# bonlime/sota_imagenet

Hardware: AMD Instinct MI355X
Metric: images/sec (whole node) ResNet-50 bs=256/GPU @224px (higher is better)
Workload: dtype bf16; 1 GPU; ResNet-50 v1.5 train step (fwd+CE+bwd+allreduce+SGD), bs=256/GPU, 224px, configs[2] bf16 activations / fp32 accumulate+master; global_batch=256, image_size=224, parallelism=dp1

## Files before the change

include/mi355rn.h:

```cpp
#ifndef MI355RN_H
#define MI355RN_H

#include <stddef.h>
#include <stdint.h>

#ifdef __cplusplus
extern "C" {
#endif

typedef enum mi355_status {
  MI355_OK = 0,
  MI355_E_ARG = -1,
  MI355_E_HIP = -2,
  MI355_E_STATE = -3,
  MI355_E_NOMEM = -4
} mi355_status;

typedef enum mi355_dtype { MI355_F32 = 0, MI355_BF16 = 1, MI355_FP8 = 2 } mi355_dtype;

const char* mi355_last_error(void);
int mi355_version(void);
int mi355_device_count(void);


size_t mi355_conv2d_workspace_bytes(int dtype, int N, int H, int W, int Cin, int Cout, int KH, int KW,
                                    int stride, int pad);

int mi355_conv2d_fwd(int dtype, const void* x, const void* w, void* y, int N, int H, int W, int Cin,
                     int Cout, int KH, int KW, int stride, int pad, void* stream);

int mi355_conv2d_fwd_stats(int dtype, const void* x, const void* w, void* y, float* partial, size_t partial_bytes, int* nblk,
                           int N, int H, int W, int Cin, int Cout, int KH, int KW, int stride, int pad, void* stream);
int mi355_conv2d_dgrad(int dtype, const void* dy, const void* w, void* dx, const void* addend, int N,
                       int H, int W, int Cin, int Cout, int KH, int KW, int stride, int pad, void* ws,
                       size_t ws_bytes, void* stream);
int mi355_conv2d_fwd_bn_in(int dtype, const void* y_in, const float* scale_shift, const void* w, void* y, void* a_out, uint8_t* a_bits,
                           float* partial, size_t partial_bytes, int* nblk, int N, int H, int W, int Cin, int Cout, int KH, int KW, int stride,
                           int pad, void* stream);
int mi355_conv2d_dgrad_bn(int dtype, const void* dy, const void* w, void* dx, const void* addend, const uint8_t* addend_bits, int addend_sub2,
                          const void* bn_y, const uint8_t* bn_bits, const float* bn_mean, const float* bn_invstd, float* partial,
                          size_t partial_bytes, int* nblk, int N, int H, int W, int Cin, int Cout, int KH, int KW, int stride, int pad,
                          void* ws, size_t ws_bytes, void* stream);
int mi355_conv2d_dgrad_bn_leaky(int dtype, const void* dy, const void* w, void* dx, const void* addend, const uint8_t* addend_bits, int addend_sub2,
                                const void* bn_y, const uint8_t* bn_bits, const float* bn_mean, const float* bn_invstd, float slope, float* partial,
                                size_t partial_bytes, int* nblk, int N, int H, int W, int Cin, int Cout, int KH, int KW, int stride, int pad,
                                void* ws, size_t ws_bytes, void* stream);

int mi355_conv2d_wgrad(int dtype, const void* dy, const void* x, float* dw, float beta, int N, int H,
                       int W, int Cin, int Cout, int KH, int KW, int stride, int pad, void* ws,
                       size_t ws_bytes, void* stream);

typedef struct mi355_crop {
  unsigned long long offset;
  int h, w, rh, rw, oy, ox, mirror, filter;
} mi355_crop;
typedef struct mi355_augment {
  float color[12];
  float blur_sigma;
  int gray, nbox, pad;
  int box[4][4];
} mi355_augment;
int mi355_ingest_u8(const unsigned char* packed, size_t packed_bytes, const mi355_crop* crops_host, const mi355_crop* crops_dev,
                    int N, int S, float mean, float std, float* out_nchw, void* stream);
int mi355_ingest_u8_aug(const unsigned char* packed, size_t packed_bytes, const mi355_crop* crops_host,
                        const mi355_crop* crops_dev, const mi355_augment* aug_host, const mi355_augment* aug_dev, int N, int S,
                        float mean, float std, float* scratch, float* out_nchw, void* stream);

int mi355_quantize_fp8(int src_dtype, const void* x, void* q, float scale, size_t n, void* stream);
int mi355_conv2d_fwd_fp8(const void* xq, const void* wq, void* y, float oscale, int N, int H, int W, int Cin, int Cout,
                         int KH, int KW, int stride, int pad, void* stream);
int mi355_conv2d_dgrad_fp8(const void* dyq, const void* wtq, void* dx, float oscale, int N, int H, int W, int Cin,
                           int Cout, int KH, int KW, int stride, int pad, void* stream);
int mi355_conv2d_wgrad_fp8(const void* dyq, const void* xq, float* dw, float beta, float oscale, int N, int H, int W, int Cin,
                           int Cout, int KH, int KW, int stride, int pad, void* ws, size_t ws_bytes, void* stream);

size_t mi355_stem_xpad_bytes(int dtype, int N, int H, int W);
int mi355_stem_ingest(int dtype, const float* x_nchw, void* xpad, int N, int H, int W, void* stream);
int mi355_stem_fwd(int dtype, const void* xpad, const float* w_krsc, void* y, int N, int H, int W,
                   void* ws, size_t ws_bytes, void* stream);
int mi355_stem_wgrad(int dtype, const void* dy, const void* xpad, float* dw, float beta, int N, int H,
                     int W, void* ws, size_t ws_bytes, void* stream);
size_t mi355_stem_workspace_bytes(int dtype, int N, int H, int W);

size_t mi355_bn_workspace_bytes(int C);
int mi355_bn_fwd_train(int dtype, const void* x, const void* residual, void* out, const float* gamma,
                       const float* beta, float* running_mean, float* running_var, float* save_mean,
                       float* save_invstd, int M, int C, float eps, float momentum, int relu, void* ws,
                       size_t ws_bytes, void* stream);
int mi355_bn_fwd_train_partial(int dtype, const void* x, const void* residual, void* out, const float* gamma,
                               const float* beta, float* running_mean, float* running_var, float* save_mean,
                               float* save_invstd, int M, int C, float eps, float momentum, int relu, const float* partial,
                               int nblk, void* ws, size_t ws_bytes, void* stream);
int mi355_bn_fwd_eval(int dtype, const void* x, const void* residual, void* out, const float* gamma,
                      const float* beta, const float* running_mean, const float* running_var, int M,
                      int C, float eps, int relu, void* ws, size_t ws_bytes, void* stream);
int mi355_bn_bwd(int dtype, const void* dout, const void* out, const void* x, const float* gamma,
                 const float* save_mean, const float* save_invstd, void* dx, void* dz_out,
                 float* dgamma, float* dbeta, float beta_acc, int M, int C, int relu, void* ws,
                 size_t ws_bytes, void* stream);

int mi355_maxpool_fwd(int dtype, const void* x, void* y, uint8_t* idx, int N, int H, int W, int C,
                      void* stream);
int mi355_maxpool_bwd(int dtype, const void* dy, const uint8_t* idx, void* dx, int N, int H, int W,
                      int C, void* stream);

int mi355_gap_fwd(int dtype, const void* x, float* pooled, int N, int HW, int C, void* stream);
int mi355_gap_bwd(int dtype, const float* dpooled, void* dx, int N, int HW, int C, void* stream);

int mi355_ce_loss(const float* logits, const float* target, float smoothing, float grad_scale,
                  float* loss, float* row_loss, float* dlogits, int N, int C, void* stream);

int mi355_sgd_step(float* p, const float* g, float* m, size_t n, float lr, float momentum,
                   float weight_decay, float grad_scale, void* stream);
int mi355_sgd_step_ema(float* p, const float* g, float* m, float* ema, size_t n, float lr, float momentum,
                       float weight_decay, float grad_scale, float ema_decay, void* stream);

int mi355_adam_step(float* p, const float* g, float* m, float* v, size_t n, double beta1, double beta2, float eps,
                    float step_size, float bc2_sqrt, double lr, double weight_decay, int decoupled, float grad_scale,
                    void* stream);
int mi355_adam_step_ema(float* p, const float* g, float* m, float* v, float* ema, size_t n, double beta1, double beta2,
                        float eps, float step_size, float bc2_sqrt, double lr, double weight_decay, int decoupled,
                        float grad_scale, float ema_decay, void* stream);

int mi355_madgrad_step(float* p, const float* g, float* grad_sum_sq, float* s, const float* x0, size_t n, double lr, double momentum,
                       double weight_decay, double eps, int k, float grad_scale, void* stream);
int mi355_madgrad_step_ema(float* p, const float* g, float* grad_sum_sq, float* s, const float* x0, float* ema, size_t n, double lr,
                           double momentum, double weight_decay, double eps, int k, float grad_scale, float ema_decay, void* stream);

size_t mi355_adais_workspace_bytes(size_t n);
int mi355_adais_moments(const float* g, float* v, size_t n, double beta2, int step, float grad_scale, void* workspace, void* stream);
int mi355_adais_mean(const void* workspace, size_t workspace_bytes, size_t param_size, float* mean, void* stream);
int mi355_adais_step(float* p, const float* g, float* m, const float* v, float* beta1_prod, const float* mean, size_t n, double lr,
                     double beta0, double beta2, double eps, double weight_decay, int step, float grad_scale, void* stream);
int mi355_adais_step_ema(float* p, const float* g, float* m, const float* v, float* beta1_prod, const float* mean, float* ema, size_t n,
                         double lr, double beta0, double beta2, double eps, double weight_decay, int step, float grad_scale,
                         float ema_decay, void* stream);

size_t mi355_lw_item_elems(void);
int mi355_lw_sumsq(const float* src, size_t n, const void* items, size_t n_items, int n_tensors, float scale, void* partial, void* stream);
int mi355_lw_coef(int rule, int flags, const void* partial, size_t n_partial, const void* tensors, size_t n_tensors, void* v, float* coef,
                  void* sums, double beta1, double beta2, double eps, double lr, double weight_decay, double mean, void* stream);
int mi355_lw_update(int rule, float* p, const float* g, float* m, size_t n, const void* items, size_t n_items, const float* coef, int n_tensors,
                    double lr, int soft_wd, double wd_eps, float grad_scale, void* stream);
int mi355_lw_update_ema(int rule, float* p, const float* g, float* m, float* ema, size_t n, const void* items, size_t n_items, const float* coef,
                        int n_tensors, double lr, int soft_wd, double wd_eps, float grad_scale, float ema_decay, void* stream);

int mi355_lw_unit_sumsq(const float* src, size_t n, const void* pieces, size_t n_pieces, int n_slots, float scale, void* partial, void* stream);
int mi355_lw_unit_coef(const void* partial, size_t n_partial, const void* slots, size_t n_slots, float* v, float* den, void* sums, double beta2,
                       double eps, void* stream);
int mi355_lw_unit_update(int rule, float* p, const float* g, float* m, size_t n, const void* items, size_t n_items, const void* tensors,
                         int n_tensors, const float* den, size_t n_slots, double beta1, double lr, double weight_decay, int soft_wd, double wd_eps,
                         float grad_scale, void* stream);
int mi355_lw_unit_update_ema(int rule, float* p, const float* g, float* m, float* ema, size_t n, const void* items, size_t n_items,
                             const void* tensors, int n_tensors, const float* den, size_t n_slots, double beta1, double lr, double weight_decay,
                             int soft_wd, double wd_eps, float grad_scale, float ema_decay, void* stream);

int mi355_adamp_unit_sums(const float* p, const float* g, const float* m, const float* v, size_t n, const void* pieces, size_t n_pieces,
                          int n_slots, double beta1, double beta2, double eps, int step, int nesterov, float grad_scale, void* partial,
                          void* stream);
int mi355_adamp_coef(const void* partial, size_t n_partial, const void* slots, size_t n_slots, const void* decide, size_t n_tensors, float* coef,
                     float* wdf, int* mode, double lr, double weight_decay, double eps, double delta, double wd_ratio, void* stream);
int mi355_adamp_update(float* p, const float* g, float* m, float* v, size_t n, const void* items, size_t n_items, const void* tensors,
                       int n_tensors, const float* coef, size_t n_slots, const float* wdf, double lr, double beta1, double beta2, double eps,
                       int step, int nesterov, float grad_scale, void* stream);
int mi355_adamp_update_ema(float* p, const float* g, float* m, float* v, float* ema, size_t n, const void* items, size_t n_items,
                           const void* tensors, int n_tensors, const float* coef, size_t n_slots, const float* wdf, double lr, double beta1,
                           double beta2, double eps, int step, int nesterov, float grad_scale, float ema_decay, void* stream);

int mi355_sam_sumsq(const float* p, const float* g, size_t n, const void* items, size_t n_items, const int* kind, int n_tensors, float eta,
                    float grad_scale, void* partial, void* stream);
int mi355_sam_scale(const void* partial, size_t n_partial, double rho, float* out, void* stream);
int mi355_sam_perturb(float* p, const float* g, float* eps, size_t n, const void* items, size_t n_items, const int* kind, int n_tensors,
                      const float* out, float eta, float grad_scale, void* stream);
int mi355_sam_restore(float* p, const float* eps, size_t n, const void* items, size_t n_items, int n_tensors, void* stream);

int mi355_sam_lw_sumsq(const float* p, const float* g, size_t n, const void* items, size_t n_items, int n_tensors, float grad_scale, void* partial,
                       void* stream);
int mi355_sam_unit_sumsq(const float* p, const float* g, size_t n, const void* pieces, size_t n_pieces, int n_slots, float grad_scale,
                         void* partial, int threads_per_piece, void* stream);
int mi355_sam_lw_coef(const void* partial, size_t n_partial, const void* slots, size_t n_slots, float* coef, float* norms, void* stream);
int mi355_sam_lw_perturb(float* p, const float* g, float* eps, size_t n, const void* items, size_t n_items, const void* tensors, int n_tensors,
                         const float* coef, size_t n_slots, double rho, float grad_scale, void* stream);
// ... 118 lines not shown
```

sota_imagenet_amd/csrc/bn.hip:

```cpp
#include <hip/hip_fp8.h>

#include <algorithm>

#include "common.h"
#include "vec.h"

namespace mi355 {
namespace {

constexpr int MAXBLK = 512;

__device__ __forceinline__ void quant8(const float (&v)[8], float scale, uint8_t* dst, float& amax) {
  float c[8];
#pragma unroll
  for (int e = 0; e < 8; ++e) {
    const float r = (float)(bf16_t)v[e];
    amax = fmaxf(amax, fabsf(r));
    c[e] = __builtin_amdgcn_fmed3f(r * scale, 448.f, -448.f);
  }
  int lo = 0, hi = 0;
  lo = __builtin_amdgcn_cvt_pk_fp8_f32(c[0], c[1], lo, false);
  lo = __builtin_amdgcn_cvt_pk_fp8_f32(c[2], c[3], lo, true);
  hi = __builtin_amdgcn_cvt_pk_fp8_f32(c[4], c[5], hi, false);
  hi = __builtin_amdgcn_cvt_pk_fp8_f32(c[6], c[7], hi, true);
// ... 326 lines not shown
      for (int e = 0; e < V; ++e) v[e] += fmaf(rv[e], sc2[e], sh2[e]);
    }
    if constexpr (RELU != 0) {
      if constexpr (RELU == 2 || RELU == 3) {
        unsigned b = 0;
#pragma unroll
        for (int e = 0; e < V; ++e) b |= (v[e] > 0.f ? 1u : 0u) << e;
        __builtin_nontemporal_store((uint8_t)b, p.bits + i);
      }
#pragma unroll
      for (int e = 0; e < V; ++e) v[e] = v[e] > 0.f ? v[e] : (RELU == 2 ? 0.f : v[e] * p.slope);
    }
    if constexpr (!QONLY) Vec16<T>::store(out + i * V, v);
    if constexpr (Q) quant8(v, qs, p.qo.q + i * V, amax);
  }
  if constexpr (Q) amax_flush(amax, p.qo.amax);
}

struct BwdApplyArgs {
  const void* g;
  const void* mask;
  const uint8_t* bits;
  const void* x;
  const float* mean;
  const float* invstd;
  const float* coef;
  void* dx;
  size_t nvec;
  int cvecs, C;
  float slope;
  EcaGrad eg;
  QuantOut qo;
};

template <typename T, int MASK, bool Q = false, bool QONLY = false>
__global__ __launch_bounds__(256) void bn_bwd_apply_kernel(const BwdApplyArgs p) {
  constexpr int V = Vec16<T>::N;
  static_assert(!Q || V == 8, "the quantised twin exists for bf16 tensors");
  float qs = 1.f, amax = 0.f;
  if constexpr (Q) qs = p.qo.scale[0];
  const T* g = reinterpret_cast<const T*>(p.g);
  const T* mk = reinterpret_cast<const T*>(p.mask);
  const T* x = reinterpret_cast<const T*>(p.x);
  T* dx = reinterpret_cast<T*>(p.dx);
  const size_t stride = (size_t)gridDim.x * 256;
  size_t i = (size_t)blockIdx.x * 256 + threadIdx.x;
  const int c0 = (int)(i % p.cvecs) * V;
  float mu[V], is[V], k0[V], k1[V], k2[V];
  load_consts<V>(p.mean, c0, mu);
  load_consts<V>(p.invstd, c0, is);
  load_consts<V>(p.coef, c0, k0);
  load_consts<V>(p.coef + p.C, c0, k1);
  load_consts<V>(p.coef + 2 * p.C, c0, k2);
#pragma unroll 2
  for (; i < p.nvec; i += stride) {
    float gv[V], xv[V];
    Vec16<T>::load_nt(g + i * V, gv);
    Vec16<T>::load_nt(x + i * V, xv);
    if constexpr (MASK == 2) {
      const unsigned b = p.bits[i];
#pragma unroll
      for (int e = 0; e < V; ++e) gv[e] = (b >> e) & 1u ? gv[e] : 0.f;
    } else if constexpr (MASK == 3) {
      const unsigned b = p.bits[i];
#pragma unroll
      for (int e = 0; e < V; ++e) gv[e] = (b >> e) & 1u ? gv[e] : gv[e] * p.slope;
    } else if constexpr (MASK == 4) {
      eca_grad<T, V>(p.eg, (int)((i / p.cvecs) / (size_t)p.eg.hw), p.C, c0, gv);
    } else if constexpr (MASK == 1) {
      float mv[V];
      Vec16<T>::load(mk + i * V, mv);
#pragma unroll
      for (int e = 0; e < V; ++e) gv[e] = mv[e] > 0.f ? gv[e] : gv[e] * p.slope;
    }
#pragma unroll
    for (int e = 0; e < V; ++e) {
      const float xh = (xv[e] - mu[e]) * is[e];
      gv[e] = k0[e] * (gv[e] - k1[e] - xh * k2[e]);
    }
    if constexpr (!QONLY) Vec16<T>::store(dx + i * V, gv);
    if constexpr (Q) quant8(gv, qs, p.qo.q + i * V, amax);
  }
  if constexpr (Q) amax_flush(amax, p.qo.amax);
}

constexpr int SC = 64;

__device__ __forceinline__ __amdgpu_buffer_rsrc_t rsrc_of(const void* p, size_t bytes) {
  return __builtin_amdgcn_make_buffer_rsrc(const_cast<void*>(p), 0, (int)(bytes > 0xfffffffcull ? 0xfffffffcull : bytes), 0x00020000);
}
__device__ __forceinline__ uint4 buf16(__amdgpu_buffer_rsrc_t r, unsigned voff, unsigned soff, bool nt = false) {
  return nt ? __builtin_bit_cast(uint4, __builtin_amdgcn_raw_buffer_load_b128(r, voff, soff, 2))
            : __builtin_bit_cast(uint4, __builtin_amdgcn_raw_buffer_load_b128(r, voff, soff, 0));
}

template <typename T>
struct PoolGather {
  static constexpr int V = Vec16<T>::N;
  uint4 g[4];
  uint32_t id[4][V / 4];
  __device__ __forceinline__ void load(__amdgpu_buffer_rsrc_t rg, __amdgpu_buffer_rsrc_t ri, unsigned t, unsigned cv, int a, int b, int Ho, int Wo) {
    const unsigned go = (t * SC + cv * V) * (unsigned)sizeof(T), io = t * SC + cv * V;
#pragma unroll
    for (int w = 0; w < 4; ++w) {
      const bool ok = a + (w >> 1) < Ho && b + (w & 1) < Wo;
      const unsigned srow = (w >> 1) ? (unsigned)Wo * SC : 0u;
      g[w] = buf16(rg, go + (w & 1) * SC * (unsigned)sizeof(T), srow * (unsigned)sizeof(T));
      if constexpr (V == 4) {
        const unsigned x = (unsigned)__builtin_amdgcn_raw_buffer_load_b32(ri, io + (w & 1) * SC, srow, 0);
        id[w][0] = ok ? x : 0xffffffffu;
      } else {
        typedef unsigned u32x2 __attribute__((ext_vector_type(2)));
        const u32x2 x = __builtin_bit_cast(u32x2, __builtin_amdgcn_raw_buffer_load_b64(ri, io + (w & 1) * SC, srow, 0));
        id[w][0] = ok ? x[0] : 0xffffffffu;
        id[w][1] = ok ? x[1] : 0xffffffffu;
      }
    }
  }
  template <int r, int c>
  __device__ __forceinline__ void pixel(unsigned bits, float (&out)[V]) const {
#pragma unroll
    for (int e = 0; e < V; ++e) out[e] = 0.f;
#pragma unroll
    for (int dr = 0; dr <= r; ++dr)
#pragma unroll
      for (int dc = 0; dc <= c; ++dc) {
        const unsigned pos = (r + 1 - 2 * dr) * 3 + (c + 1 - 2 * dc);
        float gw[V];
        Vec16<T>::unpack(g[2 * dr + dc], gw);
#pragma unroll
        for (int e = 0; e < V; ++e)
          if (((id[2 * dr + dc][e >> 2] >> (8 * (e & 3))) & 0xffu) == pos) out[e] += gw[e];
      }
#pragma unroll
    for (int e = 0; e < V; ++e) out[e] = (bits >> e) & 1u ? (float)(T)out[e] : 0.f;
  }
};

struct StemBwdArgs {
  const void* dp;
  const uint8_t* idx;
  const uint8_t* bits;
  const void* y;
  const float* mean;
  const float* invstd;
  const float* coef;
  float* partial;
  void* dx;
  int N, Ho, Wo;
};

template <typename T>
struct BlockIn {
  uint4 y[4];
  unsigned bt[4];
  unsigned pix00;
  __device__ __forceinline__ void load(__amdgpu_buffer_rsrc_t ry, __amdgpu_buffer_rsrc_t rb, int n, int a, int b, int Ho, int Wo, unsigned cv, bool nt) {
    constexpr int V = Vec16<T>::N;
    const unsigned W = 2 * Wo;
    pix00 = ((unsigned)n * 2 * Ho + 2 * a) * W + 2 * b;
#pragma unroll
    for (int k = 0; k < 4; ++k) {
      const unsigned srow = (k >> 1) ? W : 0u;
      y[k] = buf16(ry, (pix00 * SC + cv * V) * (unsigned)sizeof(T) + (k & 1) * SC * (unsigned)sizeof(T), srow * SC * (unsigned)sizeof(T), nt);
      bt[k] = (unsigned)__builtin_amdgcn_raw_buffer_load_b8(rb, pix00 * (SC / V) + cv + (k & 1) * (SC / V), srow * (SC / V), 0);
    }
// ... 329 lines not shown
  } else {
    MI355_BN_REDUCE(bf16_t)
  }
#undef MI355_BN_REDUCE
  MI355_LAUNCH_CHECK();
  return 0;
}

int launch_bn_bwd_finalize(const float* partial, int nblk, int M, int C, const float* gamma, const float* invstd,
                           float* dgamma, float* dbeta, float beta_acc, float* coef, hipStream_t s) {
  FinalizeArgs a{};
  a.partial = partial;
  a.nblk = nblk;
  a.M = M;
  a.C = C;
  a.gamma = gamma;
  a.invstd = invstd;
  a.dgamma = dgamma;
  a.dbeta = dbeta;
  a.beta_acc = beta_acc;
  a.coef = coef;
  if (fin_one_channel(C, nblk) && nblk > FIN_WIDE_ROWS) hipLaunchKernelGGL((bn_finalize_kernel<1, 1, 1024>), dim3(C), dim3(1024), 0, s, a);
  else if (fin_one_channel(C, nblk)) hipLaunchKernelGGL((bn_finalize_kernel<1, 1>), dim3(C), dim3(256), 0, s, a);
  else hipLaunchKernelGGL((bn_finalize_kernel<1, 4>), dim3(C / 4), dim3(256), 0, s, a);
  MI355_LAUNCH_CHECK();
  return 0;
}

int launch_bn_bwd_apply(int dtype, const void* g, const void* mask_src, const void* x, const float* mean,
                        const float* invstd, const float* coef, void* dx, int M, int C, hipStream_t s,
                        const uint8_t* relu_bits, float slope, QuantOut qo, const EcaGrad* eg) {
  MI355_TRY(check_c(dtype, C));
  const int V = 16 / (int)dtype_size(dtype);
  BwdApplyArgs a{};
  if (eg) a.eg = *eg;
  a.slope = slope;
  a.g = g;
  a.mask = mask_src;
  a.bits = relu_bits;
  a.x = x;
  a.mean = mean;
  a.invstd = invstd;
  a.coef = coef;
  a.dx = dx;
  a.nvec = (size_t)M * C / V;
  a.cvecs = C / V;
  a.C = C;
  const int blocks = elementwise_blocks(a.nvec, a.cvecs);
  const int mask = relu_bits ? (slope != 0.f ? 3 : 2) : mask_src ? 1 : 0;
  a.qo = qo;
  if (eg) {
    MI355_ARG(mask == 0 && !qo.q && eg->gate && eg->dpool && eg->hw > 0, "bn_bwd_apply: the ECA gradient source takes no mask / twin");
    if (dtype == MI355_F32) hipLaunchKernelGGL((bn_bwd_apply_kernel<float, 4>), dim3(blocks), dim3(256), 0, s, a);
    else hipLaunchKernelGGL((bn_bwd_apply_kernel<bf16_t, 4>), dim3(blocks), dim3(256), 0, s, a);
    MI355_LAUNCH_CHECK();
    return 0;
  }
  if (qo.q) {
    MI355_ARG(dtype == MI355_BF16 && mask != 1 && mask != 3 && qo.scale && qo.amax, "bn_bwd_apply: the e4m3 twin needs bf16 and a ReLU bit mask (or none)");
    if (mask == 2 && qo.only) hipLaunchKernelGGL((bn_bwd_apply_kernel<bf16_t, 2, true, true>), dim3(blocks), dim3(256), 0, s, a);
    else if (mask == 2) hipLaunchKernelGGL((bn_bwd_apply_kernel<bf16_t, 2, true>), dim3(blocks), dim3(256), 0, s, a);
    else if (qo.only) hipLaunchKernelGGL((bn_bwd_apply_kernel<bf16_t, 0, true, true>), dim3(blocks), dim3(256), 0, s, a);
    else hipLaunchKernelGGL((bn_bwd_apply_kernel<bf16_t, 0, true>), dim3(blocks), dim3(256), 0, s, a);
    MI355_LAUNCH_CHECK();
    return 0;
  }
#define MI355_BN_BWD_APPLY(TT)                                                                                  \
  switch (mask) {                                                                                               \
    case 0: hipLaunchKernelGGL((bn_bwd_apply_kernel<TT, 0>), dim3(blocks), dim3(256), 0, s, a); break;          \
    case 1: hipLaunchKernelGGL((bn_bwd_apply_kernel<TT, 1>), dim3(blocks), dim3(256), 0, s, a); break;          \
    case 2: hipLaunchKernelGGL((bn_bwd_apply_kernel<TT, 2>), dim3(blocks), dim3(256), 0, s, a); break;          \
    default: hipLaunchKernelGGL((bn_bwd_apply_kernel<TT, 3>), dim3(blocks), dim3(256), 0, s, a); break;         \
  }
  if (dtype == MI355_F32) {
    MI355_BN_BWD_APPLY(float)
  } else {
    MI355_BN_BWD_APPLY(bf16_t)
  }
#undef MI355_BN_BWD_APPLY
  MI355_LAUNCH_CHECK();
  return 0;
}

static int stem_bwd_args(StemBwdArgs& a, int dtype, const void* dp, const uint8_t* idx, const uint8_t* bits, const void* y, const float* mean,
                         const float* invstd, int N, int H, int W, int C) {
  MI355_TRY(check_c(dtype, C));
  const int V = 16 / (int)dtype_size(dtype);
  (void)V;
  MI355_ARG(dp && idx && bits && y && H % 2 == 0 && W % 2 == 0 && C == SC, "stem_bwd: N=%d H=%d W=%d C=%d (64 channels)", N, H, W, C);
  MI355_ARG((unsigned long long)N * H * W * C * dtype_size(dtype) < 0xfffffff0ull, "stem_bwd: tensor beyond 32-bit offsets");
  a = StemBwdArgs{};
  a.dp = dp; a.idx = idx; a.bits = bits; a.y = y; a.mean = mean; a.invstd = invstd;
  a.N = N; a.Ho = H / 2; a.Wo = W / 2;
  return 0;
}

int launch_stem_bwd_reduce(int dtype, const void* dp, const uint8_t* idx, const uint8_t* bits, const void* y, const float* mean,
                           const float* invstd, float* partial, int* nblk_out, int N, int H, int W, int C, hipStream_t s) {
  StemBwdArgs a;
  MI355_TRY(stem_bwd_args(a, dtype, dp, idx, bits, y, mean, invstd, N, H, W, C));
  a.partial = partial;
  const int V = 16 / (int)dtype_size(dtype);
  const int rpp = 256 / (C / V);
  int nblk = cdiv(N * a.Ho * a.Wo, rpp * 4);
  const int cap = std::min(2 * MAXBLK, 2 * device_cus());
  if (nblk > cap) nblk = cap;
  *nblk_out = nblk;
  if (dtype == MI355_F32) hipLaunchKernelGGL(stem_bwd_reduce_kernel<float>, dim3(nblk), dim3(256), 0, s, a);
  else hipLaunchKernelGGL(stem_bwd_reduce_kernel<bf16_t>, dim3(nblk), dim3(256), 0, s, a);
  MI355_LAUNCH_CHECK();
  return 0;
}

int launch_stem_bwd_apply(int dtype, const void* dp, const uint8_t* idx, const uint8_t* bits, const void* y, const float* mean,
                          const float* invstd, const float* coef, void* dx, int N, int H, int W, int C, hipStream_t s) {
  StemBwdArgs a;
  MI355_TRY(stem_bwd_args(a, dtype, dp, idx, bits, y, mean, invstd, N, H, W, C));
  a.coef = coef; a.dx = dx;
  const int V = 16 / (int)dtype_size(dtype);
  const int blocks = elementwise_blocks((size_t)N * a.Ho * a.Wo * (C / V), C / V);
  if (dtype == MI355_F32) hipLaunchKernelGGL(stem_bwd_apply_kernel<float>, dim3(blocks), dim3(256), 0, s, a);
  else hipLaunchKernelGGL(stem_bwd_apply_kernel<bf16_t>, dim3(blocks), dim3(256), 0, s, a);
  MI355_LAUNCH_CHECK();
  return 0;
}

}
```

sota_imagenet_amd/csrc/common.h:

```cpp
#pragma once
#include <hip/hip_runtime.h>
#include <cstdarg>
#include <cstdint>
#include <cstdio>
#include <cstring>

#include "../../include/mi355rn.h"

namespace mi355 {

typedef __bf16 bf16_t;

typedef float f32x4 __attribute__((ext_vector_type(4)));
typedef float f32x16 __attribute__((ext_vector_type(16)));
typedef __bf16 bf16x8 __attribute__((ext_vector_type(8)));
typedef __bf16 bf16x4 __attribute__((ext_vector_type(4)));
typedef short s16x4 __attribute__((ext_vector_type(4)));

void set_error(const char* fmt, ...);
int device_cus();
int probe_env(const char* name);

#define MI355_HIP(expr)                                                                         \
  do {                                                                                          \
    hipError_t e_ = (expr);                                                                     \
    if (e_ != hipSuccess) {                                                                     \
      ::mi355::set_error("%s:%d: %s -> %s", __FILE__, __LINE__, #expr, hipGetErrorString(e_));  \
      return MI355_E_HIP;                                                                       \
    }                                                                                           \
  } while (0)

#define MI355_LAUNCH_CHECK()                                                                    \
  do {                                                                                          \
    hipError_t e_ = hipGetLastError();                                                          \
    if (e_ != hipSuccess) {                                                                     \
      ::mi355::set_error("%s:%d: kernel launch -> %s", __FILE__, __LINE__, hipGetErrorString(e_)); \
      return MI355_E_HIP;                                                                       \
    }                                                                                           \
  } while (0)

#define MI355_ARG(cond, ...)                      \
  do {                                            \
    if (!(cond)) {                                \
      ::mi355::set_error(__VA_ARGS__);            \
      return MI355_E_ARG;                         \
    }                                             \
  } while (0)

#define MI355_TRY(expr)            \
  do {                             \
    int rc_ = (expr);              \
    if (rc_ != 0) return rc_;      \
  } while (0)

static inline size_t dtype_size(int dt) { return dt == MI355_BF16 ? 2 : 4; }
static inline size_t align_up(size_t x, size_t a) { return (x + a - 1) / a * a; }
static inline int cdiv(int a, int b) { return (a + b - 1) / b; }

struct Tap {
  int8_t dh, dw;
  int16_t wtap;
};
struct TapClass {
  int ph, pw, ntaps;
  Tap taps[9];
};
struct IgemmArgs {
  const void* in;
  const void* wt;
  void* out;
  const void* addend;
  const uint8_t* addend_bits = nullptr;
  int addend_sub2 = 0;
  int stat_rows_cap = 0;
  float* stat_partial;
  void* sk_ws = nullptr;
  const void* bn_y = nullptr;
  const uint8_t* bn_bits = nullptr;
  const float* bn_mean = nullptr;
  const float* bn_invstd = nullptr;
  float bn_slope = 0.f;
  const float* bn_in = nullptr;
  void* bn_in_a = nullptr;
  uint8_t* bn_in_bits = nullptr;
  const float* q_scale_in = nullptr;
  const float* q_scale_wt = nullptr;
  int N, Hin, Win, pix_stride;
  int Hsub, Wsub, IS;
  int Hout, Wout, OS;
  int Ck, Ncols, wtaps;
  int pair_delta;
  TapClass cls[4];
};

struct WgradArgs {
  const void* dy;
  const void* x;
  float* partial;
  int N, Ho, Wo, Cout;
  int Hin, Win, pix_stride, IS;
  int Ck, wtaps, ntaps;
  int chunks_per_split;
  int pair_delta;
  Tap taps[9];
};

int launch_igemm(int dtype, const IgemmArgs& a, int nclass, hipStream_t stream, int* stat_rows = nullptr);
bool igemm_leaky_sums_legal(int dtype, const IgemmArgs& a, int nclass);
bool igemm_sub2_legal(int dtype, const IgemmArgs& a, int nclass);
bool igemm_bn_in_legal(int dtype, const IgemmArgs& a, int nclass);
static constexpr size_t IGEMM_SK_FLAG_BYTES = 4096;
static constexpr int IGEMM_SK_ERR_WORD = 512;
size_t igemm_sk_ws_bytes();
bool igemm_fp8_legal(const IgemmArgs& a, int nclass);
int launch_igemm_fp8(const IgemmArgs& a, int nclass, float oscale, hipStream_t stream, int* stat_rows = nullptr);
int plan_wgrad_splits(int dtype, int M, int Cout, int ntaps, int Ck);
int plan_wgrad(int dtype, const WgradArgs& a);
int launch_wgrad(int dtype, const WgradArgs& a, int splits, hipStream_t stream);
struct Knobs {
  bool has_igemm8 = false;
  char igemm8[32] = {0};
  int igemm_big = -1;
  bool has_igemm_big = false;
  int stem_direct = 1;
  int stem_th = 0;
  bool stem_dbg = false;
  bool sk_mute = false;
  int dconv = 1;
  int wg3 = 1;
  int pw = 1;
  int pk = 1;
  int po = 1;
  int po64 = 1;
  int dconv_fp8 = 1;
  int pool_keys = 1;
  int po_bn = 1;
  int dconv_bn = 0;
  int dconv_s2 = 1;
  char error[160] = {0};
};
const Knobs& knobs();
inline int env_switch(const char* name, int def, int maxv, const char** bad) {
  const char* e = getenv(name);
  if (!e) return def;
  if (e[0] >= '0' && e[0] <= '0' + maxv && e[1] == 0) return e[0] - '0';
  if (bad && !*bad) *bad = name;
  return def;
}
void note_kernel(const char* fmt, ...);
int launch_splitk_reduce(const float* partial, int splits, size_t stride, float* dst, size_t n, float beta,
                         hipStream_t stream, const float* sa = nullptr, const float* sb = nullptr);
int launch_stem_unpack(float* partial, int splits, float* dw, float beta, hipStream_t stream);

int launch_weight_prep(int dtype, const float* w, void* w_cast, void* w_tr, int Cout, int taps, int Cin,
                       hipStream_t stream);
constexpr int PREP_TILE = 64;
struct PrepDesc {
  size_t w_off;
  void* w_cast;
  void* w_tr;
  void* w_q;
  void* w_trq;
  const float* q_scale;
  unsigned* q_amax;
  int Cout, taps, Cin;
  int tile_begin;
};
struct BPrepDesc {
  const float* w;
  float* w_hat;
  float* mean;
  float* invstd;
  void* wp;
  void* wtr;
  int Cout, taps, Cin, Coutp, Cinp;
  int row_begin;
  int tile_begin;
};
struct KeepBatch {
  float* keep[20];
  unsigned long long n[20];
  unsigned long long counter[20];
  float p[20];
  int count = 0;
};
int launch_keep_scale_batch(const KeepBatch& kb, unsigned long long seed, hipStream_t s);
int launch_bres_weight_prep(int dtype, const BPrepDesc* table, int nconv, int total_rows, int total_tiles, float eps, bool transposed, hipStream_t stream);
int launch_weight_prep_batch(int dtype, const PrepDesc* table, int nlayers, int total_tiles, const float* params,
                             hipStream_t stream);
int launch_transpose_any(int dtype, const void* w, void* wt, int Cout, int taps, int Cin, hipStream_t stream);
int launch_stem_pack(int dtype, const float* w, void* packed, hipStream_t stream);

void build_fwd_args(IgemmArgs& a, int N, int H, int W, int Cin, int Cout, int KH, int KW, int stride, int pad);
int build_dgrad_args(IgemmArgs& a, int N, int H, int W, int Cin, int Cout, int KH, int KW, int stride, int pad);
void build_wgrad_args(WgradArgs& a, int N, int H, int W, int Cin, int Cout, int KH, int KW, int stride, int pad);
void build_stem_fwd_args(IgemmArgs& a, int N, int H, int W);
void build_stem_wgrad_args(WgradArgs& a, int N, int H, int W);

static constexpr int STEM_PAD = 3, STEM_PS = 4, STEM_CK = 64, STEM_RPAD = 16;
static inline int stem_hp(int H) { return H + 2 * STEM_PAD; }
static inline int stem_wp(int W) { return W + STEM_RPAD; }

int launch_bn_stats(int dtype, const void* x, float* partial, float* pivot, int* nblk_out, int M, int C, hipStream_t s);
int launch_bn_finalize(const float* partial, const float* pivot, int nblk, int M, int C, const float* gamma, const float* beta,
                       float* running_mean, float* running_var, float* save_mean, float* save_invstd,
                       float* scale, float* shift, float eps, float momentum, hipStream_t s);
int launch_bn_eval_coeffs(const float* gamma, const float* beta, const float* rm, const float* rv, float* scale,
                          float* shift, int C, float eps, hipStream_t s);
struct QuantOut {
  uint8_t* q = nullptr;
  const float* scale = nullptr;
  unsigned* amax = nullptr;
  bool only = false;
};
int launch_bn_apply(int dtype, const void* x, const float* scale, const float* shift, const void* residual,
                    const void* x2, const float* scale2, const float* shift2, void* out, int M, int C, int relu,
                    hipStream_t s, uint8_t* relu_bits = nullptr, QuantOut qo = QuantOut());
struct EcaGrad {
  const float* keep = nullptr;
  const float* gate = nullptr;
  const float* dpool = nullptr;
  int hw = 0;
};
int launch_bn_bwd_reduce(int dtype, const void* g, const void* mask_src, const void* x, const float* mean,
                         const float* invstd, void* dz_out, float* partial, int* nblk_out, int M, int C,
                         hipStream_t s, const uint8_t* relu_bits = nullptr, float slope = 0.f, const EcaGrad* eg = nullptr);
int launch_bn_bwd_finalize(const float* partial, int nblk, int M, int C, const float* gamma, const float* invstd,
                           float* dgamma, float* dbeta, float beta_acc, float* coef , hipStream_t s);
int launch_bn_bwd_apply(int dtype, const void* g, const void* mask_src, const void* x, const float* mean,
                        const float* invstd, const float* coef, void* dx, int M, int C, hipStream_t s,
                        const uint8_t* relu_bits = nullptr, float slope = 0.f, QuantOut qo = QuantOut(), const EcaGrad* eg = nullptr);
int launch_stem_bwd_reduce(int dtype, const void* dp, const uint8_t* idx, const uint8_t* bits, const void* y, const float* mean,
                           const float* invstd, float* partial, int* nblk_out, int N, int H, int W, int C, hipStream_t s);
int launch_stem_bwd_apply(int dtype, const void* dp, const uint8_t* idx, const uint8_t* bits, const void* y, const float* mean,
                          const float* invstd, const float* coef, void* dx, int N, int H, int W, int C, hipStream_t s);
int bn_max_blocks();
int launch_nchw_pad64(int dtype, const float* x_nchw, void* h_nhwc64, int N, int HW, hipStream_t s);
int launch_weight_pad_cast(int dtype, const float* w, void* wp, int Cout, int taps, int Cin, int Coutp, int Cinp, hipStream_t s);
int launch_nchw_im2col3s2(int dtype, const float* x, void* h, int N, int H, int W, hipStream_t s);
int launch_weight_unpad(const float* dwp, float* dw, float beta, int Cout, int taps, int Cin, int Cinp, hipStream_t s);
int launch_axpby(const float* src, float* dst, float beta, size_t n, hipStream_t s);
int launch_eca_residual_fwd(int dtype, const void* x, const float* w, int k, const float* keep, const void* shortcut, void* out, float* pooled, float* gate,
                            int N, int HW, int C, int act, hipStream_t s, const float* xs = nullptr, const float* xh = nullptr, const float* ss = nullptr,
                            const float* sh2 = nullptr, uint8_t* out_bits = nullptr, float* raw_ws = nullptr );
int launch_eca_residual_bwd(int dtype, const void* dout, const void* out, const void* x, const float* keep, const float* w, int k, const float* pooled,
                            const float* gate, void* dshortcut, void* dx, float* dw, float beta, float* ws, int N, int HW, int C, int act, hipStream_t s,
                            const float* xs = nullptr, const float* xh = nullptr, float* bn_row = nullptr, const float* bn_mean = nullptr,
                            const float* bn_invstd = nullptr, const uint8_t* out_bits = nullptr, const void* ds_y = nullptr, float* ds_row = nullptr,
                            const float* ds_mean = nullptr, const float* ds_invstd = nullptr);
int launch_fp8_scale_update(float* scale, unsigned* amax, int n, float headroom, hipStream_t s);

int launch_maxpool_fwd(int dtype, const void* x, void* y, uint8_t* idx, int N, int H, int W, int C, hipStream_t s);
int launch_bn_relu_maxpool(int dtype, const void* y, const float* scale, const float* shift, void* p, uint8_t* idx,
                           uint8_t* bits, int N, int H, int W, int C, hipStream_t s);
int launch_maxpool_bwd(int dtype, const void* dy, const uint8_t* idx, void* dx, int N, int H, int W, int C,
                       hipStream_t s);
int launch_gap_fwd(int dtype, const void* x, float* pooled, int N, int HW, int C, hipStream_t s);
int launch_fc(const float* x, const float* w, float* out, int M, int N, int K, hipStream_t s);
int launch_gap_bwd(int dtype, const float* dpooled, void* dx, int N, int HW, int C, hipStream_t s);
int launch_ce(const float* logits, const float* target, float smoothing, float grad_scale, float* loss,
              float* row_loss, float* dlogits, int N, int C, hipStream_t s);
int launch_sgd(float* p, const float* g, float* m, size_t n, float lr, float mom, float wd, float gscale,
               hipStream_t s, float* ema = nullptr, float ema_decay = 0.f);
int launch_adam(float* p, const float* g, float* m, float* v, size_t n, double beta1, double beta2, float eps, float step_size,
                float bc2_sqrt, double lr, double wd, int decoupled, float gscale, hipStream_t s, float* ema = nullptr,
                float ema_decay = 0.f);
int launch_madgrad(float* p, const float* g, float* gss, float* s, const float* x0, size_t n, double lr, double momentum, double wd,
                   double eps, int k, float gscale, hipStream_t st, float* ema = nullptr, float ema_decay = 0.f);
size_t adais_partials(size_t n);
int launch_adais_moments(const float* g, float* v, size_t n, double beta2, int step, float gscale, double* partial, hipStream_t st);
int launch_adais_mean(const double* partial, size_t count, size_t param_size, float* mean, hipStream_t st);
int launch_adais_step(float* p, const float* g, float* m, const float* v, float* b1prod, const float* mean, size_t n, double lr, double beta0,
                      double beta2, double eps, double wd, int step, float gscale, hipStream_t st, float* ema = nullptr,
                      float ema_decay = 0.f);
size_t lw_item_elems();
int launch_lw_sumsq(const float* src, size_t n, const void* items, size_t n_items, int n_tensors, float scale, double* partial, hipStream_t st);
int launch_lw_coef(int rule, int flags, const double* partial, size_t n_partial, const void* tensors, size_t n_tensors, void* v, float* coef,
                   double* sums, double beta1, double beta2, double eps, double lr, double wd, double mean, hipStream_t st);
int launch_lw_update(int rule, float* p, const float* g, float* m, float* ema, size_t n, const void* items, size_t n_items, const float* coef,
                     int n_tensors, double lr, int soft_wd, double wd_eps, float gscale, float ema_decay, hipStream_t st);
int launch_lw_unit_sumsq(const float* src, size_t n, const void* pieces, size_t n_pieces, int n_slots, float scale, double* partial,
                         hipStream_t st);
int launch_lw_unit_coef(const double* partial, size_t n_partial, const void* slots, size_t n_slots, float* v, float* den, double* sums,
                        double beta2, double eps, hipStream_t st);
int launch_lw_unit_update(int rule, float* p, const float* g, float* m, float* ema, size_t n, const void* items, size_t n_items,
                          const void* tensors, int n_tensors, const float* den, size_t n_slots, double beta1, double lr, double wd, int soft_wd,
                          double wd_eps, float gscale, float ema_decay, hipStream_t st);
int launch_adamp_unit_sums(const float* p, const float* g, const float* m, const float* v, size_t n, const void* pieces, size_t n_pieces,
                           int n_slots, double beta1, double beta2, double eps, int step, int nesterov, float gscale, double* partial,
                           hipStream_t st);
int launch_adamp_coef(const double* partial, size_t n_partial, const void* slots, size_t n_slots, const void* tensors, size_t n_tensors,
                      float* coef, float* wdf, int* mode, double lr, double wd, double eps, double delta, double wd_ratio, hipStream_t st);
int launch_adamp_update(float* p, const float* g, float* m, float* v, float* ema, size_t n, const void* items, size_t n_items,
                        const void* tensors, int n_tensors, const float* coef, size_t n_slots, const float* wdf, double lr, double beta1,
                        double beta2, double eps, int step, int nesterov, float gscale, float ema_decay, hipStream_t st);
int launch_sam_sumsq(const float* p, const float* g, size_t n, const void* items, size_t n_items, const int* kind, int n_tensors, float eta,
                     float gscale, double* partial, hipStream_t st);
int launch_sam_scale(const double* partial, size_t n_partial, double rho, float* out, hipStream_t st);
int launch_sam_perturb(float* p, const float* g, float* eps, size_t n, const void* items, size_t n_items, const int* kind, int n_tensors,
                       const float* out, float eta, float gscale, hipStream_t st);
int launch_sam_restore(float* p, const float* eps, size_t n, const void* items, size_t n_items, int n_tensors, hipStream_t st);
int launch_sam_lw_sumsq(const float* p, const float* g, size_t n, const void* items, size_t n_items, int n_tensors, float gscale, double* partial,
                        hipStream_t st);
int launch_sam_unit_sumsq(const float* p, const float* g, size_t n, const void* pieces, size_t n_pieces, int n_slots, float gscale,
                          double* partial, int threads_per_piece, hipStream_t st);
int launch_sam_lw_coef(const double* partial, size_t n_partial, const void* slots, size_t n_slots, float* coef, float* norms, hipStream_t st);
int launch_sam_lw_perturb(float* p, const float* g, float* eps, size_t n, const void* items, size_t n_items, const void* tensors, int n_tensors,
                          const float* coef, size_t n_slots, double rho, float gscale, hipStream_t st);
int launch_ortho_init(float* w, size_t n, const void* mats, size_t n_mats, float gain, int* status, hipStream_t st);
int launch_stem_ingest(int dtype, const float* x, void* xpad, int N, int H, int W, hipStream_t s);
int launch_bias_slice(const float* tmp, int ld, const float* bias, float* out, int N, int O, hipStream_t s);
int launch_pad_dlogits(const float* src, float* dst, int ld, float* dbias, float beta, int N, int O, hipStream_t s);

}
// ... 1 lines not shown
```

sota_imagenet_amd/csrc/conv_api.cpp:

```cpp
#include <algorithm>
#include <atomic>
#include <cstdio>
#include <cstdlib>
#include <mutex>
#include <set>
#include <string>

#include "conv_kernels.h"

namespace mi355 {

static thread_local std::string g_err;

void set_error(const char* fmt, ...) {
  char buf[1024];
  va_list ap;
  va_start(ap, fmt);
  vsnprintf(buf, sizeof(buf), fmt, ap);
  va_end(ap);
  g_err = buf;
}
const char* get_error() { return g_err.c_str(); }

int probe_env(const char* name) {
// ... 282 lines not shown
  build_fwd_args(a, N, H, W, Cin, Cout, KH, KW, stride, pad);
  a.in = x; a.wt = w; a.out = y;
  return launch_igemm(dtype, a, 1, (hipStream_t)stream);
}

int mi355_conv2d_fwd_stats(int dtype, const void* x, const void* w, void* y, float* partial, size_t partial_bytes, int* nblk, int N,
                           int H, int W, int Cin, int Cout, int KH, int KW, int stride, int pad, void* stream) {
  MI355_TRY(check_conv(dtype, Cin, Cout, KH, KW, stride));
  MI355_ARG(partial && nblk && partial_bytes >= (size_t)768 * 2 * Cout * sizeof(float), "conv2d_fwd_stats: partial buffer needs 768 * 2 * Cout floats");
  IgemmArgs a;
  build_fwd_args(a, N, H, W, Cin, Cout, KH, KW, stride, pad);
  a.in = x; a.wt = w; a.out = y;
  a.stat_partial = partial;
  a.stat_rows_cap = (int)std::min<size_t>(partial_bytes / ((size_t)2 * Cout * sizeof(float)), 1u << 20);
  return launch_igemm(dtype, a, 1, (hipStream_t)stream, nblk);
}

int mi355_conv2d_fwd_bn_in(int dtype, const void* y_in, const float* scale_shift, const void* w, void* y, void* a_out, uint8_t* a_bits, float* partial,
                           size_t partial_bytes, int* nblk, int N, int H, int W, int Cin, int Cout, int KH, int KW, int stride, int pad, void* stream) {
  MI355_TRY(check_conv(dtype, Cin, Cout, KH, KW, stride));
  MI355_ARG(y_in && scale_shift && a_out && a_bits, "conv2d_fwd_bn_in: null pointer");
  MI355_ARG(partial && nblk && partial_bytes >= (size_t)768 * 2 * Cout * sizeof(float), "conv2d_fwd_bn_in: partial buffer needs 768 * 2 * Cout floats");
  IgemmArgs a;
  build_fwd_args(a, N, H, W, Cin, Cout, KH, KW, stride, pad);
  a.in = y_in; a.wt = w; a.out = y;
  a.bn_in = scale_shift; a.bn_in_a = a_out; a.bn_in_bits = a_bits;
  a.stat_partial = partial;
  a.stat_rows_cap = (int)std::min<size_t>(partial_bytes / ((size_t)2 * Cout * sizeof(float)), 1u << 20);
  MI355_ARG(igemm_bn_in_legal(dtype, a, 1), "conv2d_fwd_bn_in: no kernel applies the input's BatchNorm for this launch (bf16; 3x3 / stride 1 at a generated shape, or 1x1 with 64 / 128 / 256 input channels into a multiple of 256 columns over whole 64-pixel tiles)");
  return launch_igemm(dtype, a, 1, (hipStream_t)stream, nblk);
}

int mi355_conv2d_dgrad(int dtype, const void* dy, const void* w, void* dx, const void* addend, int N, int H, int W,
                       int Cin, int Cout, int KH, int KW, int stride, int pad, void* ws, size_t ws_bytes,
                       void* stream) {
  MI355_TRY(check_conv(dtype, Cin, Cout, KH, KW, stride));
  const size_t es = dtype_size(dtype);
  const size_t wbytes = (size_t)Cin * KH * KW * Cout * es;
  MI355_ARG(ws && ws_bytes >= wbytes, "dgrad: workspace too small (%zu < %zu)", ws_bytes, wbytes);
  hipStream_t s = (hipStream_t)stream;
  MI355_TRY(launch_transpose_any(dtype, w, ws, Cout, KH * KW, Cin, s));
  IgemmArgs a;
  const int nclass = build_dgrad_args(a, N, H, W, Cin, Cout, KH, KW, stride, pad);
  if (nclass < 0) return nclass;
  a.in = dy; a.wt = ws; a.out = dx; a.addend = addend;
  return launch_igemm(dtype, a, nclass, s);
}

int mi355_conv2d_dgrad_bn(int dtype, const void* dy, const void* w, void* dx, const void* addend, const uint8_t* addend_bits, int addend_sub2, const void* bn_y,
                          const uint8_t* bn_bits, const float* bn_mean, const float* bn_invstd, float* partial, size_t partial_bytes, int* nblk, int N,
                          int H, int W, int Cin, int Cout, int KH, int KW, int stride, int pad, void* ws, size_t ws_bytes, void* stream) {
  return mi355_conv2d_dgrad_bn_leaky(dtype, dy, w, dx, addend, addend_bits, addend_sub2, bn_y, bn_bits, bn_mean, bn_invstd, 0.f, partial, partial_bytes, nblk, N, H, W,
                                     Cin, Cout, KH, KW, stride, pad, ws, ws_bytes, stream);
}

int mi355_conv2d_dgrad_bn_leaky(int dtype, const void* dy, const void* w, void* dx, const void* addend, const uint8_t* addend_bits, int addend_sub2,
                                const void* bn_y, const uint8_t* bn_bits, const float* bn_mean, const float* bn_invstd, float slope, float* partial,
                                size_t partial_bytes, int* nblk, int N, int H, int W, int Cin, int Cout, int KH, int KW, int stride, int pad, void* ws,
                                size_t ws_bytes, void* stream) {
  MI355_TRY(check_conv(dtype, Cin, Cout, KH, KW, stride));
  MI355_ARG(slope == 0.f || partial, "dgrad_bn_leaky: a slope without the BN-backward sums");
  const size_t es = dtype_size(dtype);
  const size_t wbytes = (size_t)Cin * KH * KW * Cout * es;
  MI355_ARG(ws && ws_bytes >= wbytes, "dgrad_bn: workspace too small (%zu < %zu)", ws_bytes, wbytes);
  MI355_ARG(addend || !addend_bits, "dgrad_bn: addend_bits without an addend");
  MI355_ARG(!partial || (bn_y && bn_bits && bn_mean && bn_invstd && nblk), "dgrad_bn: the BN-backward sums need bn_y, bn_bits, bn_mean, bn_invstd and nblk");
  MI355_ARG(!partial || partial_bytes >= (size_t)768 * 2 * Cin * sizeof(float), "dgrad_bn: partial buffer needs 768 * 2 * Cin floats");
  hipStream_t s = (hipStream_t)stream;
  MI355_TRY(launch_transpose_any(dtype, w, ws, Cout, KH * KW, Cin, s));
  IgemmArgs a;
  const int nclass = build_dgrad_args(a, N, H, W, Cin, Cout, KH, KW, stride, pad);
  if (nclass < 0) return nclass;
  a.in = dy; a.wt = ws; a.out = dx; a.addend = addend; a.addend_bits = addend_bits; a.addend_sub2 = addend_sub2;
  MI355_ARG(!addend_sub2 || igemm_sub2_legal(dtype, a, nclass), "dgrad_bn: no kernel takes a half-resolution addend for this launch (bf16 1x1 / stride 1, even H and W)");
  if (partial) {
    a.stat_partial = partial;
    a.stat_rows_cap = (int)std::min<size_t>(partial_bytes / ((size_t)2 * Cin * sizeof(float)), 1u << 20);
    a.bn_y = bn_y; a.bn_bits = bn_bits; a.bn_mean = bn_mean; a.bn_invstd = bn_invstd; a.bn_slope = slope;
  }
  if (nblk) *nblk = 0;
  return launch_igemm(dtype, a, nclass, s, partial ? nblk : nullptr);
}

int mi355_conv2d_wgrad(int dtype, const void* dy, const void* x, float* dw, float beta, int N, int H, int W, int Cin,
                       int Cout, int KH, int KW, int stride, int pad, void* ws, size_t ws_bytes, void* stream) {
  MI355_TRY(check_conv(dtype, Cin, Cout, KH, KW, stride));
  WgradArgs a;
  build_wgrad_args(a, N, H, W, Cin, Cout, KH, KW, stride, pad);
  const int splits = plan_wgrad(dtype, a);
  const size_t n = (size_t)Cout * KH * KW * Cin;
  MI355_ARG(ws && ws_bytes >= (size_t)splits * n * 4, "wgrad: workspace too small (%zu < %zu)", ws_bytes,
            (size_t)splits * n * 4);
  a.dy = dy; a.x = x; a.partial = (float*)ws;
  hipStream_t s = (hipStream_t)stream;
  MI355_TRY(launch_wgrad(dtype, a, splits, s));
  return launch_splitk_reduce((const float*)ws, splits, n, dw, n, beta, s);
}

size_t mi355_stem_xpad_bytes(int dtype, int N, int H, int W) {
  return (size_t)N * stem_hp(H) * stem_wp(W) * STEM_PS * dtype_size(dtype);
}

size_t mi355_stem_workspace_bytes(int dtype, int N, int H, int W) {
  const int splits = plan_wgrad_splits(dtype, N * (H / 2) * (W / 2), 64, 4, STEM_CK);
  return align_up((size_t)64 * 4 * 64 * dtype_size(dtype), 256) + (size_t)splits * 64 * 4 * 64 * 4;
}

int mi355_stem_ingest(int dtype, const float* x_nchw, void* xpad, int N, int H, int W, void* stream) {
  MI355_ARG(x_nchw && xpad && H % 2 == 0 && W % 2 == 0, "stem_ingest: bad arguments");
  return launch_stem_ingest(dtype, x_nchw, xpad, N, H, W, (hipStream_t)stream);
}

int mi355_stem_fwd(int dtype, const void* xpad, const float* w_krsc, void* y, int N, int H, int W, void* ws,
                   size_t ws_bytes, void* stream) {
  const size_t pk = (size_t)64 * 4 * 64 * dtype_size(dtype);
  MI355_ARG(ws && ws_bytes >= pk, "stem_fwd: workspace too small");
  hipStream_t s = (hipStream_t)stream;
  MI355_TRY(launch_stem_pack(dtype, w_krsc, ws, s));
  IgemmArgs a;
  build_stem_fwd_args(a, N, H, W);
  a.in = xpad; a.wt = ws; a.out = y;
  return launch_igemm(dtype, a, 1, s);
}

int mi355_stem_wgrad(int dtype, const void* dy, const void* xpad, float* dw, float beta, int N, int H, int W, void* ws,
                     size_t ws_bytes, void* stream) {
  WgradArgs a;
  build_stem_wgrad_args(a, N, H, W);
  const int splits = plan_wgrad_splits(dtype, a.N * a.Ho * a.Wo, 64, 4, STEM_CK);
  MI355_ARG(ws && ws_bytes >= (size_t)splits * 64 * 4 * 64 * 4, "stem_wgrad: workspace too small");
  a.dy = dy; a.x = xpad; a.partial = (float*)ws;
  hipStream_t s = (hipStream_t)stream;
  MI355_TRY(launch_wgrad(dtype, a, splits, s));
  return launch_stem_unpack((float*)ws, splits, dw, beta, s);
}

size_t mi355_bn_workspace_bytes(int C) { return ((size_t)bn_max_blocks() * 2 * C + 8 * (size_t)C) * 4; }

int mi355_bn_fwd_train(int dtype, const void* x, const void* residual, void* out, const float* gamma,
                       const float* beta, float* running_mean, float* running_var, float* save_mean,
                       float* save_invstd, int M, int C, float eps, float momentum, int relu, void* ws,
                       size_t ws_bytes, void* stream) {
  MI355_ARG(ws && ws_bytes >= mi355_bn_workspace_bytes(C), "bn: workspace too small");
  hipStream_t s = (hipStream_t)stream;
  float* partial = (float*)ws;
  float* scale = partial + (size_t)bn_max_blocks() * 2 * C;
  float* shift = scale + C;
  float* pivot = shift + C;
  int nblk = 0;
  MI355_TRY(launch_bn_stats(dtype, x, partial, pivot, &nblk, M, C, s));
  MI355_TRY(launch_bn_finalize(partial, pivot, nblk, M, C, gamma, beta, running_mean, running_var, save_mean, save_invstd,
                               scale, shift, eps, momentum, s));
  return launch_bn_apply(dtype, x, scale, shift, residual, nullptr, nullptr, nullptr, out, M, C, relu, s);
}

int mi355_bn_fwd_train_partial(int dtype, const void* x, const void* residual, void* out, const float* gamma, const float* beta,
                               float* running_mean, float* running_var, float* save_mean, float* save_invstd, int M, int C, float eps,
                               float momentum, int relu, const float* partial, int nblk, void* ws, size_t ws_bytes, void* stream) {
  MI355_ARG(ws && ws_bytes >= (size_t)2 * C * 4 && partial && nblk >= 1, "bn_fwd_train_partial: nblk=%d, workspace of 2*C floats", nblk);
  hipStream_t s = (hipStream_t)stream;
  float* scale = (float*)ws;
  float* shift = scale + C;
  MI355_TRY(launch_bn_finalize(partial, nullptr, nblk, M, C, gamma, beta, running_mean, running_var, save_mean, save_invstd, scale,
                               shift, eps, momentum, s));
  return launch_bn_apply(dtype, x, scale, shift, residual, nullptr, nullptr, nullptr, out, M, C, relu, s);
}

int mi355_bn_fwd_eval(int dtype, const void* x, const void* residual, void* out, const float* gamma,
                      const float* beta, const float* running_mean, const float* running_var, int M, int C, float eps,
                      int relu, void* ws, size_t ws_bytes, void* stream) {
  MI355_ARG(ws && ws_bytes >= (size_t)2 * C * 4, "bn_eval: workspace too small");
  hipStream_t s = (hipStream_t)stream;
  float* scale = (float*)ws;
  float* shift = scale + C;
  MI355_TRY(launch_bn_eval_coeffs(gamma, beta, running_mean, running_var, scale, shift, C, eps, s));
  return launch_bn_apply(dtype, x, scale, shift, residual, nullptr, nullptr, nullptr, out, M, C, relu, s);
}

int mi355_bn_bwd(int dtype, const void* dout, const void* out, const void* x, const float* gamma,
                 const float* save_mean, const float* save_invstd, void* dx, void* dz_out, float* dgamma,
                 float* dbeta, float beta_acc, int M, int C, int relu, void* ws, size_t ws_bytes, void* stream) {
  MI355_ARG(ws && ws_bytes >= mi355_bn_workspace_bytes(C), "bn: workspace too small");
  hipStream_t s = (hipStream_t)stream;
  float* partial = (float*)ws;
  float* coef = partial + (size_t)bn_max_blocks() * 2 * C;
  int nblk = 0;
  const void* mask = relu ? out : nullptr;
  const float slope = relu == 2 ? 0.01f : 0.f;
  MI355_TRY(launch_bn_bwd_reduce(dtype, dout, mask, x, save_mean, save_invstd, dz_out, partial, &nblk, M, C, s, nullptr, slope));
  MI355_TRY(launch_bn_bwd_finalize(partial, nblk, M, C, gamma, save_invstd, dgamma, dbeta, beta_acc, coef, s));
  return launch_bn_bwd_apply(dtype, dout, mask, x, save_mean, save_invstd, coef, dx, M, C, s, nullptr, slope);
}

int mi355_maxpool_fwd(int dtype, const void* x, void* y, uint8_t* idx, int N, int H, int W, int C, void* stream) {
  return launch_maxpool_fwd(dtype, x, y, idx, N, H, W, C, (hipStream_t)stream);
}
int mi355_maxpool_bwd(int dtype, const void* dy, const uint8_t* idx, void* dx, int N, int H, int W, int C,
                      void* stream) {
  return launch_maxpool_bwd(dtype, dy, idx, dx, N, H, W, C, (hipStream_t)stream);
}
int mi355_gap_fwd(int dtype, const void* x, float* pooled, int N, int HW, int C, void* stream) {
  return launch_gap_fwd(dtype, x, pooled, N, HW, C, (hipStream_t)stream);
}
int mi355_gap_bwd(int dtype, const float* dpooled, void* dx, int N, int HW, int C, void* stream) {
  return launch_gap_bwd(dtype, dpooled, dx, N, HW, C, (hipStream_t)stream);
}
int mi355_ce_loss(const float* logits, const float* target, float smoothing, float grad_scale, float* loss,
                  float* row_loss, float* dlogits, int N, int C, void* stream) {
  return launch_ce(logits, target, smoothing, grad_scale, loss, row_loss, dlogits, N, C, (hipStream_t)stream);
}
int mi355_sgd_step(float* p, const float* g, float* m, size_t n, float lr, float momentum, float weight_decay,
                   float grad_scale, void* stream) {
  return launch_sgd(p, g, m, n, lr, momentum, weight_decay, grad_scale, (hipStream_t)stream);
}
int mi355_sgd_step_ema(float* p, const float* g, float* m, float* ema, size_t n, float lr, float momentum, float weight_decay,
                       float grad_scale, float ema_decay, void* stream) {
  MI355_ARG(ema, "sgd_step_ema: null ema");
  return launch_sgd(p, g, m, n, lr, momentum, weight_decay, grad_scale, (hipStream_t)stream, ema, ema_decay);
}
int mi355_adam_step(float* p, const float* g, float* m, float* v, size_t n, double beta1, double beta2, float eps,
                    float step_size, float bc2_sqrt, double lr, double weight_decay, int decoupled, float grad_scale,
                    void* stream) {
  return launch_adam(p, g, m, v, n, beta1, beta2, eps, step_size, bc2_sqrt, lr, weight_decay, decoupled, grad_scale,
                     (hipStream_t)stream);
}
int mi355_adam_step_ema(float* p, const float* g, float* m, float* v, float* ema, size_t n, double beta1, double beta2,
                        float eps, float step_size, float bc2_sqrt, double lr, double weight_decay, int decoupled,
                        float grad_scale, float ema_decay, void* stream) {
  MI355_ARG(ema, "adam_step_ema: null ema");
  return launch_adam(p, g, m, v, n, beta1, beta2, eps, step_size, bc2_sqrt, lr, weight_decay, decoupled, grad_scale,
                     (hipStream_t)stream, ema, ema_decay);
}
int mi355_madgrad_step(float* p, const float* g, float* grad_sum_sq, float* s, const float* x0, size_t n, double lr, double momentum,
                       double weight_decay, double eps, int k, float grad_scale, void* stream) {
  return launch_madgrad(p, g, grad_sum_sq, s, x0, n, lr, momentum, weight_decay, eps, k, grad_scale, (hipStream_t)stream);
}
int mi355_madgrad_step_ema(float* p, const float* g, float* grad_sum_sq, float* s, const float* x0, float* ema, size_t n, double lr,
                           double momentum, double weight_decay, double eps, int k, float grad_scale, float ema_decay, void* stream) {
  MI355_ARG(ema, "madgrad_step_ema: null ema");
  return launch_madgrad(p, g, grad_sum_sq, s, x0, n, lr, momentum, weight_decay, eps, k, grad_scale, (hipStream_t)stream, ema, ema_decay);
}
size_t mi355_adais_workspace_bytes(size_t n) { return adais_partials(n) * sizeof(double); }
int mi355_adais_moments(const float* g, float* v, size_t n, double beta2, int step, float grad_scale, void* workspace, void* stream) {
  return launch_adais_moments(g, v, n, beta2, step, grad_scale, (double*)workspace, (hipStream_t)stream);
}
int mi355_adais_mean(const void* workspace, size_t workspace_bytes, size_t param_size, float* mean, void* stream) {
  MI355_ARG(workspace_bytes % sizeof(double) == 0, "adais_mean: workspace_bytes=%zu is not a whole number of partial sums", workspace_bytes);
  return launch_adais_mean((const double*)workspace, workspace_bytes / sizeof(double), param_size, mean, (hipStream_t)stream);
}
int mi355_adais_step(float* p, const float* g, float* m, const float* v, float* beta1_prod, const float* mean, size_t n, double lr,
                     double beta0, double beta2, double eps, double weight_decay, int step, float grad_scale, void* stream) {
  return launch_adais_step(p, g, m, v, beta1_prod, mean, n, lr, beta0, beta2, eps, weight_decay, step, grad_scale, (hipStream_t)stream);
}
int mi355_adais_step_ema(float* p, const float* g, float* m, const float* v, float* beta1_prod, const float* mean, float* ema, size_t n,
                         double lr, double beta0, double beta2, double eps, double weight_decay, int step, float grad_scale,
                         float ema_decay, void* stream) {
  MI355_ARG(ema, "adais_step_ema: null ema");
  return launch_adais_step(p, g, m, v, beta1_prod, mean, n, lr, beta0, beta2, eps, weight_decay, step, grad_scale, (hipStream_t)stream, ema,
                           ema_decay);
}

size_t mi355_lw_item_elems(void) { return lw_item_elems(); }
int mi355_lw_sumsq(const float* src, size_t n, const void* items, size_t n_items, int n_tensors, float scale, void* partial, void* stream) {
  return launch_lw_sumsq(src, n, items, n_items, n_tensors, scale, (double*)partial, (hipStream_t)stream);
}
int mi355_lw_coef(int rule, int flags, const void* partial, size_t n_partial, const void* tensors, size_t n_tensors, void* v, float* coef,
                  void* sums, double beta1, double beta2, double eps, double lr, double weight_decay, double mean, void* stream) {
  return launch_lw_coef(rule, flags, (const double*)partial, n_partial, tensors, n_tensors, v, coef, (double*)sums, beta1, beta2, eps, lr,
                        weight_decay, mean, (hipStream_t)stream);
}
int mi355_lw_update(int rule, float* p, const float* g, float* m, size_t n, const void* items, size_t n_items, const float* coef, int n_tensors,
                    double lr, int soft_wd, double wd_eps, float grad_scale, void* stream) {
  return launch_lw_update(rule, p, g, m, nullptr, n, items, n_items, coef, n_tensors, lr, soft_wd, wd_eps, grad_scale, 0.f, (hipStream_t)stream);
}
int mi355_lw_update_ema(int rule, float* p, const float* g, float* m, float* ema, size_t n, const void* items, size_t n_items, const float* coef,
                        int n_tensors, double lr, int soft_wd, double wd_eps, float grad_scale, float ema_decay, void* stream) {
// ... 88 lines not shown
```

sota_imagenet_amd/csrc/conv_igemm.hip:

```cpp
#include <atomic>
#include <cstdio>
#include <cstdlib>
#include <type_traits>

#include "conv_kernels.h"
#include "lds_dma.h"
#include "vec.h"

namespace mi355 {

namespace {

constexpr int BKB = 128;

__device__ __attribute__((aligned(256))) unsigned char g_zero_page[256];
#ifdef MI355_STAMP
__device__ unsigned long long g_stamps[8 * 4096];
#define STAMP(slot)                                                                                   \
  do {                                                                                                \
    if (blockIdx.x == 0 && lane == 0 && wave < 4 && stamp_k < 1024) g_stamps[(wave * 1024 + stamp_k) * 8 + (slot)] = __builtin_readcyclecounter(); \
  } while (0)
#else
#define STAMP(slot)
#endif
__device__ __attribute__((aligned(256))) unsigned char g_trash[512 * 16];
#ifdef MI355_PROBES
#define MI355_PROBE(bit) ((kp.dbg & (bit)) != 0)
#else
#define MI355_PROBE(bit) false
#endif

struct IgemmKArgs {
  IgemmArgs a;
  int mtiles, ny, nclass, ngroups, ntpg, items;
  unsigned bytes_in, bytes_wt;
  int sk_rf, sk_tail, sk_nk, sk_gshift;
  int sk_tshift;
  unsigned sk_epoch;
  float* sk_partial;
  unsigned* sk_flags;
  unsigned sk_spin_limit;
  int sk_mute;
  int dbg;
  int xcd;
};

template <int N>
__device__ __forceinline__ void wait_vm() {
  asm volatile("s_waitcnt vmcnt(%0)" ::"n"(N) : "memory");
}

template <typename T, int BM, int BN, int WMW, int NSTG, int STATS>
__global__ __launch_bounds__(128 * WMW, (BM == 256 ? 1 : (BN == 64 && NSTG == 2 ? 3 : 2))) void igemm_kernel(const IgemmKArgs kp) {
  const IgemmArgs& p = kp.a;
  constexpr int ES = (int)sizeof(T);
  constexpr int BK = BKB / ES;
  constexpr int NW = 2 * WMW;
  constexpr int NT = 64 * NW;
  constexpr int MI = BM / (32 * WMW);
  constexpr int NI = BN / 64;
  constexpr int PA = BM / NW / 8;
  constexpr int PB = BN / NW / 8;
  constexpr int NPC = PA + PB;
  constexpr int A_BYTES = BM * BKB;
  constexpr int STAGE = (BM + BN) * BKB;
  constexpr int WN = BN / 2;
  constexpr int VEC = 16 / ES;
  constexpr int CPR = WN / VEC;
  constexpr int RPI = 64 / CPR;
  constexpr int NST = MI * (32 / RPI);
  constexpr int SCH = WN / 4;
  extern __shared__ __attribute__((aligned(16))) char smem[];
  constexpr int STG_WAVE = 32 * (BN / 2) * 4;
  constexpr int EPI_FIT = STAGE / STG_WAVE;
  constexpr int EPI_WAVES = NW <= EPI_FIT ? NW : (EPI_FIT >= 4 ? 4 : (EPI_FIT >= 2 ? 2 : 1));
  constexpr int EPI_TURNS = NW / EPI_WAVES;
  static_assert(NW % EPI_WAVES == 0, "epilogue turns");
  int* row_pix = reinterpret_cast<int*>(smem + NSTG * STAGE);
  float* stat_acc = reinterpret_cast<float*>(smem + NSTG * STAGE + BM * sizeof(int));

  const int tid = threadIdx.x;
  const int lane = tid & 63;
  const int wave = __builtin_amdgcn_readfirstlane(tid >> 6);
  const int wm = wave >> 1, wn = wave & 1;
  const int G = gridDim.x;
  const int Msub = p.N * p.Hsub * p.Wsub;
  const int kc_per_tap = p.Ck / BK;

  const int prow = lane >> 3;
  const int pch = lane & 7;
  int L_seq = 0, L_item = 0, L_nt = 0, L_kt = 0, L_kend = 0, L_cls = 0, L_grp = 0;
  bool L_valid = true;
  constexpr bool SKC = BM == 128 && BN == 128 && ES == 4;
  int sk_bg = 0, sk_n = 0, sk_item0 = 0, sk_k00 = 0, sk_k10 = 0, sk_k11 = 0;
  if constexpr (SKC) {
    if (kp.sk_tail != 0) {
      sk_bg = (int)blockIdx.x / kp.ngroups;
      const int g = (int)blockIdx.x - sk_bg * kp.ngroups;
      const unsigned TK = (unsigned)(kp.sk_tail * kp.sk_nk);
      const unsigned lo = ((unsigned)sk_bg * TK) >> kp.sk_tshift, hi = ((unsigned)(sk_bg + 1) * TK) >> kp.sk_tshift;
      if (lo < hi && sk_bg < (1 << kp.sk_tshift)) {
        const int t0 = (int)(lo / (unsigned)kp.sk_nk);
        sk_item0 = ((kp.sk_rf << kp.sk_gshift) + t0) * kp.ngroups + g;
        sk_k00 = (int)lo - t0 * kp.sk_nk;
        const int e = sk_k00 + (int)(hi - lo);
        sk_k10 = e < kp.sk_nk ? e : kp.sk_nk;
        sk_k11 = (int)hi - (t0 + 1) * kp.sk_nk;
        sk_n = sk_k11 > 0 ? 2 : 1;
      }
      sk_bg = __builtin_amdgcn_readfirstlane(sk_bg);
      sk_n = __builtin_amdgcn_readfirstlane(sk_n);
      sk_item0 = __builtin_amdgcn_readfirstlane(sk_item0);
      sk_k00 = __builtin_amdgcn_readfirstlane(sk_k00);
      sk_k10 = __builtin_amdgcn_readfirstlane(sk_k10);
      sk_k11 = __builtin_amdgcn_readfirstlane(sk_k11);
    }
  }
  const int bx = __builtin_amdgcn_readfirstlane(kp.xcd ? (int)(blockIdx.x & 7u) * (G >> 3) + (int)(blockIdx.x >> 3) : (int)blockIdx.x);
  auto unit_at = [&](int seq, int& item, int& k0, int& k1) -> bool {
    if (!SKC || kp.sk_tail == 0) {
      item = bx + seq * G;
      k0 = 0;
      k1 = -1;
      return item < kp.items;
    }
    const int u = seq - kp.sk_rf;
    if (u < 0) {
      item = (int)blockIdx.x + seq * G;
      k0 = 0;
      k1 = -1;
      return true;
    }
    if (u >= sk_n) return false;
    item = sk_item0 + u * kp.ngroups;
    k0 = u == 0 ? sk_k00 : 0;
    k1 = u == 0 ? sk_k10 : sk_k11;
    return true;
  };
  const i32x4 srdA = make_srd(p.in, kp.bytes_in);
  const i32x4 srdB = make_srd(p.wt, kp.bytes_wt);
  unsigned a_off[PA];
  int a_h[PA], a_w[PA];
  unsigned b_off[PB];
#pragma unroll
  for (int i = 0; i < PB; ++i) {
    const int r = PB * 8 * wave + 8 * i + prow;
    b_off[i] = (unsigned)r * p.wtaps * p.Ck * ES + (unsigned)((pch ^ ((r >> 1) & 7)) * 16);
  }
  auto L_setup = [&]() {
    int uk0, uk1;
    while ((L_valid = unit_at(L_seq, L_item, uk0, uk1))) {
      const int rowtile = L_item / kp.ngroups;
      L_grp = L_item - rowtile * kp.ngroups;
      L_cls = rowtile / kp.mtiles;
      const int mt = rowtile - L_cls * kp.mtiles;
      const int nk_all = p.cls[L_cls].ntaps * kc_per_tap;
      if (nk_all == 0) {
        ++L_seq;
        continue;
      }
#pragma unroll
      for (int i = 0; i < PA; ++i) {
        const int r = (BM / NW) * wave + 8 * i + prow;
        const int m = mt * BM + r;
        if (m < Msub) {
          const int j = m % p.Wsub;
          const int t = m / p.Wsub;
          const int ii = t % p.Hsub;
          const int n = t / p.Hsub;
          a_h[i] = ii * p.IS;
          a_w[i] = j * p.IS;
          const int chunk = pch ^ ((r >> 1) & 7);
          a_off[i] = (unsigned)((n * p.Hin + a_h[i]) * p.Win + a_w[i]) * (unsigned)(p.pix_stride * ES) +
                     (unsigned)(chunk * 16);
          if (ES == 2 && chunk >= 4) a_off[i] += (unsigned)(p.pair_delta * ES);
        } else {
          a_h[i] = -(1 << 20);
          a_w[i] = 0;
          a_off[i] = 0;
        }
      }
      L_nt = 0;
      L_kt = uk0;
      L_kend = uk1 < 0 ? nk_all : uk1;
      return;
    }
  };
  int S_dh = 0, S_dw = 0, S_dA = 0;
  unsigned S_dB = 0, S_As = 0;
  auto L_begin = [&](int stage) {
    const int kt_u = __builtin_amdgcn_readfirstlane(L_kt);
    const int cls_u = __builtin_amdgcn_readfirstlane(L_cls);
    const int t = kt_u / kc_per_tap;
    const int c0 = (kt_u - t * kc_per_tap) * BK;
    const Tap tp = p.cls[cls_u].taps[t];
    S_dh = tp.dh;
    S_dw = tp.dw;
    S_dA = ((tp.dh * p.Win + tp.dw) * p.pix_stride + c0 + (ES == 4 && c0 >= 32 ? p.pair_delta : 0)) * ES;
    const int n0 = __builtin_amdgcn_readfirstlane((L_grp * kp.ntpg + L_nt) * BN);
    S_dB = ((unsigned)n0 * p.wtaps + tp.wtap) * (unsigned)(p.Ck * ES) + (unsigned)(c0 * ES);
    S_As = __builtin_amdgcn_readfirstlane(lds_addr(smem) + stage * STAGE);
  };
  auto L_piece = [&](int j) {
    if (j < PA) {
      const int ih = a_h[j] + S_dh;
      const int iw = a_w[j] + S_dw;
      const bool ok = ((unsigned)ih < (unsigned)p.Hin) && ((unsigned)iw < (unsigned)p.Win);
      blds16(srdA, ok ? a_off[j] + (unsigned)S_dA : 0x80000000u, S_As + ((BM / NW) * wave + 8 * j) * BKB);
    } else {
      const int i = j - PA;
      blds16(srdB, b_off[i] + S_dB, S_As + A_BYTES + (PB * 8 * wave + 8 * i) * BKB);
    }
  };
  auto L_advance = [&]() {
    if (++L_kt < L_kend) return;
    if (++L_nt < kp.ntpg) {
      L_kt = 0;
      return;
    }
    ++L_seq;
    L_setup();
  };

  const int hh = lane >> 5;
  int a_row[MI], a_sw[MI], b_row[NI], b_sw[NI];
#pragma unroll
  for (int mi = 0; mi < MI; ++mi) {
    const int r = wm * (BM / WMW) + mi * 32 + (lane & 31);
    a_row[mi] = r * BKB;
    a_sw[mi] = (r >> 1) & 7;
  }
#pragma unroll
  for (int ni = 0; ni < NI; ++ni) {
    const int r = wn * WN + ni * 32 + (lane & 31);
    b_row[ni] = A_BYTES + r * BKB;
    b_sw[ni] = (r >> 1) & 7;
  }

  if constexpr (STATS != 0) {
    for (int i = tid; i < WMW * kp.ntpg * BN * 2; i += NT) stat_acc[i] = 0.f;
  }
  L_setup();
  int stage = 0;
  int L_stage = 0;
  int inflight = 0;
#pragma unroll
  for (int pre = 0; pre < NSTG - 1; ++pre)
    if (L_valid) {
      L_begin(L_stage);
#pragma unroll
      for (int j = 0; j < NPC; ++j) L_piece(j);
      L_advance();
      L_stage = L_stage + 1 == NSTG ? 0 : L_stage + 1;
      ++inflight;
    }
  int pending_st = 0;
#ifdef MI355_STAMP
  int stamp_k = 0;
#endif

  T* out = reinterpret_cast<T*>(p.out);
  const T* addend = reinterpret_cast<const T*>(p.addend);

  int item, uk0, uk1;
  for (int seq = 0; unit_at(seq, item, uk0, uk1); ++seq) {
    const int rowtile = item / kp.ngroups;
    const int grp = item - rowtile * kp.ngroups;
    const int ci = rowtile / kp.mtiles;
    const int mt = rowtile - ci * kp.mtiles;
    const TapClass& cls = p.cls[ci];
    const int nk = cls.ntaps * kc_per_tap;
    const int m0 = mt * BM;
    for (int nti = 0; nti < kp.ntpg; ++nti) {
      const int n0 = (grp * kp.ntpg + nti) * BN;
      f32x16 acc[MI][NI];
#pragma unroll
      for (int mi = 0; mi < MI; ++mi)
#pragma unroll
        for (int ni = 0; ni < NI; ++ni)
#pragma unroll
          for (int r = 0; r < 16; ++r) acc[mi][ni][r] = 0.f;

      const int kbeg = uk0, kend = uk1 < 0 ? nk : uk1;
      for (int kt = kbeg; kt < kend; ++kt) {
        STAMP(0);
        if constexpr (NSTG == 2) {
          if (pending_st == NST) {
            wait_vm<NST>();
          } else {
            wait_vm<0>();
          }
        } else {
          const bool younger = inflight >= 2;
          if (younger && pending_st == NST) wait_vm<NPC + NST>();
          else if (younger) wait_vm<NPC>();
          else if (pending_st == NST) wait_vm<NST>();
          else wait_vm<0>();
        }
        pending_st = 0;
        STAMP(1);
        MI355_LDS_BARRIER();
        STAMP(2);
        const bool lv = L_valid;
        if (lv) L_begin(L_stage);
        const char* base = smem + stage * STAGE;
        typedef typename std::conditional<ES == 4, f32x4, bf16x8>::type frag_t;
        frag_t av[2][MI], bv[2][NI];
        auto read_frags = [&](int g, int set) {
#pragma unroll
          for (int mi = 0; mi < MI; ++mi)
            av[set][mi] = *reinterpret_cast<const frag_t*>(base + a_row[mi] + (((2 * g + hh) ^ a_sw[mi]) << 4));
#pragma unroll
          for (int ni = 0; ni < NI; ++ni)
            bv[set][ni] = *reinterpret_cast<const frag_t*>(base + b_row[ni] + (((2 * g + hh) ^ b_sw[ni]) << 4));
        };
        read_frags(0, 0);
#pragma unroll
        for (int g = 0; g < 4; ++g) {
          if (g + 1 < 4) read_frags(g + 1, (g + 1) & 1);
          if (lv) {
#pragma unroll
            for (int j = g * NPC / 4; j < (g + 1) * NPC / 4; ++j) L_piece(j);
          }
// ... 32 lines not shown
        if (kbeg > 0) {
          const i32x4 srdP = make_srd(kp.sk_partial, (unsigned)((size_t)G * SLOT * 4));
          const unsigned base = ((unsigned)blockIdx.x * SLOT + tid * 4) * 4u;
#pragma unroll
          for (int mi = 0; mi < MI; ++mi)
#pragma unroll
            for (int ni = 0; ni < NI; ++ni)
#pragma unroll
              for (int g = 0; g < 4; ++g) {
                const f32x4 v = {acc[mi][ni][4 * g], acc[mi][ni][4 * g + 1], acc[mi][ni][4 * g + 2], acc[mi][ni][4 * g + 3]};
                const unsigned off = base + (unsigned)(((mi * NI + ni) * 4 + g) * 256 * 16);
                asm volatile("buffer_store_dwordx4 %0, %1, %2, 0 offen sc1" ::"v"(v), "v"(off), "s"(srdP) : "memory");
              }
          asm volatile("s_waitcnt vmcnt(0)" ::: "memory");
          __builtin_amdgcn_s_barrier();
          if (tid == 0 && !kp.sk_mute)
            __hip_atomic_store(kp.sk_flags + blockIdx.x, kp.sk_epoch, __ATOMIC_RELAXED, __HIP_MEMORY_SCOPE_AGENT);
          pending_st = 0;
          continue;
        }
        const unsigned TK = (unsigned)(kp.sk_tail * kp.sk_nk);
        const int tt = rowtile - (kp.sk_rf << kp.sk_gshift);
        const unsigned tile_end = (unsigned)((tt + 1) * kp.sk_nk);
        int bgj = sk_bg + 1;
        int covered = kend;
        while (covered < nk && bgj < (1 << kp.sk_tshift)) {
          const unsigned lo_j = ((unsigned)bgj * TK) >> kp.sk_tshift, hi_j = ((unsigned)(bgj + 1) * TK) >> kp.sk_tshift;
          const int cnt = (int)((hi_j < tile_end ? hi_j : tile_end) - lo_j);
          if (cnt > 0) {
            const int j = bgj * kp.ngroups + grp;
            if (tid == 0) {
              unsigned spins = 0;
              while (__hip_atomic_load(kp.sk_flags + j, __ATOMIC_RELAXED, __HIP_MEMORY_SCOPE_AGENT) != kp.sk_epoch) {
                __builtin_amdgcn_s_sleep(2);
                if (++spins > kp.sk_spin_limit) {
                  __hip_atomic_store(kp.sk_flags + IGEMM_SK_ERR_WORD, 1u, __ATOMIC_RELAXED, __HIP_MEMORY_SCOPE_AGENT);
                  break;
                }
              }
              __builtin_amdgcn_fence(__ATOMIC_ACQUIRE, "agent");
            }
            asm volatile("s_waitcnt vmcnt(0)" ::: "memory");
            __builtin_amdgcn_s_barrier();
            const float* slot = kp.sk_partial + (size_t)j * SLOT + tid * 4;
#pragma unroll
            for (int mi = 0; mi < MI; ++mi)
#pragma unroll
              for (int ni = 0; ni < NI; ++ni)
#pragma unroll
                for (int g = 0; g < 4; ++g) {
                  const f32x4 v = *reinterpret_cast<const f32x4*>(slot + ((mi * NI + ni) * 4 + g) * 256 * 4);
#pragma unroll
                  for (int e = 0; e < 4; ++e) acc[mi][ni][4 * g + e] += v[e];
                }
            covered += cnt;
            pending_st = 0;
          }
          ++bgj;
        }
      }

      const int done_stage = stage == 0 ? NSTG - 1 : stage - 1;
      char* stg = smem + done_stage * STAGE + (wave % EPI_WAVES) * STG_WAVE;
      MI355_LDS_BARRIER();
      if (MI355_PROBE(1)) continue;
      if (tid < BM) {
        const int m = m0 + tid;
        int pix = -1;
        if (m < Msub) {
          const int j = m % p.Wsub;
          const int t = m / p.Wsub;
          const int ii = t % p.Hsub;
          const int n = t / p.Hsub;
          pix = (n * p.Hout + ii * p.OS + cls.ph) * p.Wout + j * p.OS + cls.pw;
        }
        row_pix[tid] = pix;
      }
      if constexpr (EPI_TURNS > 1) MI355_LDS_BARRIER();
#pragma unroll
      for (int turn = 0; turn < EPI_TURNS; ++turn) {
        if (EPI_TURNS == 1 || wave / EPI_WAVES == turn) {
        const int prw = lane & 31;
        const int rr = lane / CPR, ch = lane % CPR;
        float s1[VEC], s2[VEC];
        float bmu[VEC], bis[VEC];
        if constexpr (STATS == 2) {
          const int c0 = n0 + wn * WN + ch * VEC;
  #pragma unroll
          for (int q = 0; q < VEC / 4; ++q) {
            const f32x4 a = *reinterpret_cast<const f32x4*>(p.bn_mean + c0 + 4 * q);
            const f32x4 b = *reinterpret_cast<const f32x4*>(p.bn_invstd + c0 + 4 * q);
  #pragma unroll
            for (int e = 0; e < 4; ++e) {
              bmu[4 * q + e] = a[e];
              bis[4 * q + e] = b[e];
            }
          }
        }
  #pragma unroll
        for (int e = 0; e < VEC; ++e) {
          s1[e] = 0.f;
          s2[e] = 0.f;
        }
  #pragma unroll
        for (int mi = 0; mi < MI; ++mi) {
  #pragma unroll
          for (int ni = 0; ni < NI; ++ni)
  #pragma unroll
            for (int g = 0; g < 4; ++g) {
              const f32x4 v = {acc[mi][ni][4 * g], acc[mi][ni][4 * g + 1], acc[mi][ni][4 * g + 2], acc[mi][ni][4 * g + 3]};
              const int sc = (ni * 8 + 2 * g + hh) ^ (prw & (SCH - 1));
              *reinterpret_cast<f32x4*>(stg + prw * (WN * 4) + sc * 16) = v;
            }
          if (mi == 0 && EPI_TURNS == 1) {
            MI355_LDS_BARRIER();
          } else {
            asm volatile("s_waitcnt lgkmcnt(0)" ::: "memory");
          }
          constexpr int NP = 32 / RPI;
          int pixs[NP];
          uint4 araw[NP];
          unsigned abits[NP];
          uint4 yraw[NP];
          unsigned ybits[NP];
  #pragma unroll
          for (int ps = 0; ps < NP; ++ps) {
            pixs[ps] = row_pix[wm * (BM / WMW) + mi * 32 + ps * RPI + rr];
            if (addend) {
              const size_t o = (size_t)(pixs[ps] < 0 ? 0 : pixs[ps]) * p.Ncols + n0 + wn * WN + ch * VEC;
              araw[ps] = *reinterpret_cast<const uint4*>((pixs[ps] < 0 || MI355_PROBE(4)) ? reinterpret_cast<const T*>(g_zero_page) : addend + o);
              abits[ps] = p.addend_bits ? (unsigned)p.addend_bits[pixs[ps] < 0 ? 0 : o / VEC] : 0xffu;
            }
            if constexpr (STATS == 2) {
              const size_t o = (size_t)(pixs[ps] < 0 ? 0 : pixs[ps]) * p.Ncols + n0 + wn * WN + ch * VEC;
              yraw[ps] = *reinterpret_cast<const uint4*>(reinterpret_cast<const T*>(p.bn_y) + o);
              ybits[ps] = (unsigned)p.bn_bits[o / VEC];
            }
          }
  #pragma unroll
          for (int ps = 0; ps < NP; ++ps) {
            const int row = ps * RPI + rr;
            const int pix = pixs[ps];
            float v[VEC];
  #pragma unroll
            for (int q = 0; q < VEC / 4; ++q) {
              const int sc = (ch * (VEC / 4) + q) ^ (row & (SCH - 1));
              const f32x4 t = *reinterpret_cast<const f32x4*>(stg + row * (WN * 4) + sc * 16);
              v[4 * q] = t[0]; v[4 * q + 1] = t[1]; v[4 * q + 2] = t[2]; v[4 * q + 3] = t[3];
            }
            const size_t o = (size_t)(pix < 0 ? 0 : pix) * p.Ncols + n0 + wn * WN + ch * VEC;
            if (addend) {
              float a[VEC];
              Vec16<T>::unpack(araw[ps], a);
  #pragma unroll
              for (int e = 0; e < VEC; ++e) v[e] += (abits[ps] >> e) & 1u ? a[e] : 0.f;
            }
            T* dst = (pix < 0 || MI355_PROBE(2)) ? reinterpret_cast<T*>(g_trash + tid * 16) : out + o;
            Vec16<T>::store(dst, v);
            if constexpr (STATS == 1) {
              if (pix >= 0) {
  #pragma unroll
                for (int e = 0; e < VEC; ++e) {
                  const float xr = (float)(T)v[e];
                  s1[e] += xr;
                  s2[e] += xr * xr;
                }
              }
            }
            if constexpr (STATS == 2) {
              if (pix >= 0) {
                float yv[VEC];
                Vec16<T>::unpack(yraw[ps], yv);
  #pragma unroll
                for (int e = 0; e < VEC; ++e) {
                  const float dz = (ybits[ps] >> e) & 1u ? (float)(T)v[e] : 0.f;
                  s1[e] += dz;
                  s2[e] += dz * ((yv[e] - bmu[e]) * bis[e]);
                }
              }
            }
          }
          asm volatile("" ::: "memory");
        }
        if constexpr (STATS != 0) {
          float* scr = reinterpret_cast<float*>(stg);
          asm volatile("s_waitcnt lgkmcnt(0)" ::: "memory");
  #pragma unroll
          for (int q = 0; q < VEC / 4; ++q) {
            const f32x4 a = {s1[4 * q], s1[4 * q + 1], s1[4 * q + 2], s1[4 * q + 3]};
            const f32x4 b = {s2[4 * q], s2[4 * q + 1], s2[4 * q + 2], s2[4 * q + 3]};
            *reinterpret_cast<f32x4*>(scr + rr * WN + ch * VEC + 4 * q) = a;
            *reinterpret_cast<f32x4*>(scr + (RPI + rr) * WN + ch * VEC + 4 * q) = b;
          }
          asm volatile("s_waitcnt lgkmcnt(0)" ::: "memory");
  #pragma unroll
          for (int cc = lane; cc < WN; cc += 64) {
            float a = 0.f, b = 0.f;
  #pragma unroll
            for (int r = 0; r < RPI; ++r) {
              a += scr[r * WN + cc];
              b += scr[(RPI + r) * WN + cc];
            }
            float* slot = stat_acc + ((wm * kp.ntpg + nti) * BN + wn * WN + cc) * 2;
            slot[0] += a;
            slot[1] += b;
          }
          asm volatile("s_waitcnt lgkmcnt(0)" ::: "memory");
        }
        }
        if constexpr (EPI_TURNS > 1) MI355_LDS_BARRIER();
      }
      pending_st += NST;
    }
  }
  if constexpr (STATS != 0) {
    MI355_LDS_BARRIER();
    const int chan = kp.ntpg * BN;
    const int grp = bx % kp.ngroups;
    float* row = p.stat_partial + (size_t)(bx / kp.ngroups) * 2 * p.Ncols + grp * chan;
    for (int c = tid; c < chan; c += NT) {
      float a = 0.f, b = 0.f;
#pragma unroll
      for (int w = 0; w < WMW; ++w) {
        a += stat_acc[(w * chan + c) * 2];
        b += stat_acc[(w * chan + c) * 2 + 1];
      }
      row[c] = a;
      row[p.Ncols + c] = b;
    }
  }
}

template <typename T, int BM, int BN, int WMW = 2, int NSTG = 2>
int launch_t(const IgemmArgs& a, int nclass, hipStream_t stream, int* stat_rows) {
  constexpr int NT = 128 * WMW;
  const int MAX_WG = device_cus() * (BM == 256 ? 1 : (BN == 64 && NSTG == 2 ? 3 : 2));
  IgemmKArgs k;
  k.a = a;
  const int Msub = a.N * a.Hsub * a.Wsub;
  k.mtiles = cdiv(Msub, BM);
  k.ny = a.Ncols / BN;
  k.nclass = nclass;
  const int R = nclass * k.mtiles;
  int ng = k.ny;
  if (sizeof(T) == 4) {
    long best_rounds = -1;
    for (int d = 1; d <= k.ny; ++d) {
      if (k.ny % d != 0) continue;
      const long rounds = (long)cdiv(R * d, MAX_WG) * (k.ny / d);
      if (best_rounds < 0 || rounds < best_rounds) {
        best_rounds = rounds;
        ng = d;
      }
    }
  } else {
    for (int d = 1; d <= k.ny; ++d)
      if (k.ny % d == 0 && R * d >= MAX_WG) {
        ng = d;
        break;
      }
  }
  k.sk_rf = k.sk_tail = k.sk_nk = k.sk_gshift = k.sk_tshift = 0;
  k.sk_epoch = 0;
  k.sk_partial = nullptr;
  k.sk_flags = nullptr;
  k.sk_mute = knobs().sk_mute ? 1 : 0;
#ifdef MI355_PROBES
  k.dbg = probe_env("MI355_IGEMM_DBG");
#else
  k.dbg = 0;
#endif
  k.sk_spin_limit = k.sk_mute ? (1u << 8) : (1u << 24);
  bool sk = false;
  if (BM == 128 && BN == 128 && sizeof(T) == 4 && a.sk_ws && nclass == 1 && MAX_WG % k.ny == 0) {
    const int Gg = MAX_WG / k.ny;
    const int rf = R / Gg, rt = R - rf * Gg;
    const int nk = a.cls[0].ntaps * (a.Ck / (BKB / (int)sizeof(T)));
    if (rt > 0 && rt * 100 <= Gg * 85 && nk >= 8 && (Gg & (Gg - 1)) == 0 && (long)rt * nk * MAX_WG < (1l << 31)) {
      sk = true;
      ng = k.ny;
      k.sk_rf = rf;
      k.sk_tail = rt;
      k.sk_nk = nk;
      k.sk_gshift = 0;
      while ((1 << k.sk_gshift) < Gg) ++k.sk_gshift;
      k.sk_tshift = 0;
      while ((2 << k.sk_tshift) <= Gg && (2 << k.sk_tshift) <= 4 * rt) ++k.sk_tshift;
      static std::atomic<unsigned> epoch{0};
      k.sk_epoch = ++epoch;
      if (k.sk_epoch == 0) k.sk_epoch = ++epoch;
      k.sk_flags = reinterpret_cast<unsigned*>(a.sk_ws);
      k.sk_partial = reinterpret_cast<float*>(reinterpret_cast<char*>(a.sk_ws) + IGEMM_SK_FLAG_BYTES);
    }
  }
  k.xcd = 0;
  if (sizeof(T) == 2 && !sk && BM == 128 && MAX_WG % 8 == 0 && (MAX_WG / 8) % k.ny == 0 && R * k.ny >= MAX_WG && k.ny >= 2 &&
      (a.addend_bits != nullptr || a.bn_bits != nullptr) && a.Ncols >= 512) {
    ng = k.ny;
    k.xcd = 1;
  }
  k.ngroups = ng;
  k.ntpg = k.ny / ng;
  k.items = R * ng;
  const size_t bytes_in = (size_t)a.N * a.Hin * a.Win * a.pix_stride * sizeof(T);
  const size_t bytes_wt = (size_t)a.Ncols * a.wtaps * a.Ck * sizeof(T);
  MI355_ARG(bytes_in < 0x80000000ull && bytes_wt < 0x80000000ull, "igemm: tensor exceeds the 2 GiB buffer-offset range");
  k.bytes_in = (unsigned)bytes_in;
  k.bytes_wt = (unsigned)bytes_wt;
  const int grid = sk ? MAX_WG : (k.items < MAX_WG ? k.items : MAX_WG);
  size_t lds = (size_t)NSTG * (BM + BN) * BKB + BM * sizeof(int);
  const int chan = k.ntpg * BN;
  const bool stats = a.stat_partial != nullptr && chan <= 512 && grid % ng == 0 &&
                     lds + (size_t)WMW * chan * 2 * sizeof(float) <= 160 * 1024;
  if (stat_rows) *stat_rows = stats ? grid / ng : 0;
  if (stats) {
    lds += (size_t)WMW * chan * 2 * sizeof(float);
    lds_opt_in((const void*)igemm_kernel<T, BM, BN, WMW, NSTG, 1>, lds);
    lds_opt_in((const void*)igemm_kernel<T, BM, BN, WMW, NSTG, 2>, lds);
    if (a.bn_y)
      hipLaunchKernelGGL((igemm_kernel<T, BM, BN, WMW, NSTG, 2>), dim3(grid), dim3(NT), lds, stream, k);
    else
      hipLaunchKernelGGL((igemm_kernel<T, BM, BN, WMW, NSTG, 1>), dim3(grid), dim3(NT), lds, stream, k);
  } else {
    lds_opt_in((const void*)igemm_kernel<T, BM, BN, WMW, NSTG, 0>, lds);
    hipLaunchKernelGGL((igemm_kernel<T, BM, BN, WMW, NSTG, 0>), dim3(grid), dim3(NT), lds, stream, k);
  }
  MI355_LAUNCH_CHECK();
  note_kernel("igemm<%s,%d,%d,%d>", sizeof(T) == 2 ? "bf16" : "f32", BM, BN, NSTG);
  return 0;
}

}

size_t igemm_sk_ws_bytes() { return IGEMM_SK_FLAG_BYTES + (size_t)512 * 128 * 128 * sizeof(float); }

int launch_igemm_tile(int dtype, const IgemmArgs& a, int nclass, int bm, int bn, hipStream_t stream, int* stat_rows) {
  if (dtype == MI355_F32 && bm == 128 && bn == 128) return launch_t<float, 128, 128>(a, nclass, stream, stat_rows);
  if (dtype == MI355_F32 && bm == 128 && bn == 64) return launch_t<float, 128, 64>(a, nclass, stream, stat_rows);
  if (dtype == MI355_BF16 && bm == 256 && bn == 256) return launch_t<bf16_t, 256, 256>(a, nclass, stream, stat_rows);
  if (dtype == MI355_BF16 && bm == 256 && bn == 128) return launch_t<bf16_t, 256, 128, 4, 3>(a, nclass, stream, stat_rows);
  if (dtype == MI355_BF16 && bm == 128 && bn == 128) return launch_t<bf16_t, 128, 128>(a, nclass, stream, stat_rows);
  if (dtype == MI355_BF16 && bm == 128 && bn == 64) return launch_t<bf16_t, 128, 64>(a, nclass, stream, stat_rows);
  set_error("igemm: no %dx%d tile for dtype %d", bm, bn, dtype);
  return MI355_E_ARG;
}

}

#ifdef MI355_STAMP
extern "C" int mi355_debug_stamps(unsigned long long* host_out, int n) {
  return (int)hipMemcpyFromSymbol(host_out, HIP_SYMBOL(mi355::g_stamps), (size_t)n * sizeof(unsigned long long), 0,
                                  hipMemcpyDeviceToHost);
}
extern "C" int mi355_debug_stamps_clear(void) {
  static unsigned long long z[8 * 4096];
  return (int)hipMemcpyToSymbol(HIP_SYMBOL(mi355::g_stamps), z, sizeof(z), 0, hipMemcpyHostToDevice);
}
#endif
```

sota_imagenet_amd/csrc/conv_select.cpp:

```cpp
#include <cstdio>

#include "conv_kernels.h"

namespace mi355 {

namespace {

constexpr int BKB = 128;

int max_taps(const IgemmArgs& a, int nclass) {
  int m = 0;
  for (int ci = 0; ci < nclass; ++ci) m = a.cls[ci].ntaps > m ? a.cls[ci].ntaps : m;
  return m;
}

bool choose_igemm8(const IgemmArgs& a, int nclass, ConvPick* p) {
  const char* env = knobs().has_igemm8 ? knobs().igemm8 : nullptr;
  if (env && env[0] == '0') return false;
  if (env && env[0]) {
    int m = 0, n = 0;
    char k1 = 0, k2 = 0;
    if (sscanf(env, "%dx%d%c%c", &m, &n, &k1, &k2) >= 2 && (m == 256 || m == 224) && (n == 256 || n == 128) && igemm8_legal(a, nclass, n)) {
      p->bm = m; p->bn = n; p->korder = k1 == 'k' || k2 == 'k'; p->fat = k1 == 'f' || k2 == 'f';
      return true;
    }
    return false;
  }
  const int mt = max_taps(a, nclass);
  const long K = (long)mt * a.Ck;
  const long M = (long)a.N * a.Hsub * a.Wsub;
  const bool heavy_epilogue = (a.addend != nullptr && K < 1024);
  const int ko = (mt > 1 && a.Ck > 64) ? 1 : 0;
  if (a.Ncols % 256 == 0 && K >= 256 && !heavy_epilogue && igemm8_legal(a, nclass, 256)) {
    const long tiles = ((M + 223) / 224) * nclass * (a.Ncols / 256);
    const int cus = device_cus();
    if (tiles * 10 >= 7L * cus && !(nclass > 1 && tiles > 2L * cus && mt > 1)) {
      p->bm = 224; p->bn = 256; p->korder = ko; p->fat = 0;
      return true;
    }
  }
  if (a.Ncols % 128 == 0 && K >= 4096 && igemm8_legal(a, nclass, 128)) {
    const long tiles = ((M + 255) / 256) * nclass * (a.Ncols / 128);
    if (tiles * 10 >= 7L * device_cus() && tiles <= device_cus()) {
      p->bm = 256; p->bn = 128; p->korder = ko; p->fat = 1;
      return true;
    }
  }
  return false;
}

bool select_generated(const IgemmArgs& a, int nclass, ConvPick* p) {
  return dconv_pick(a, nclass, 0, p) || po_pick(a, nclass, p) || pw_pick(a, nclass, p) || pk_pick(a, nclass, p);
}

ConvPick select_bf16(const IgemmArgs& a, int nclass, bool wide) {
  ConvPick p;
  if (select_generated(a, nclass, &p)) return p;
  if (knobs().stem_direct && stem_direct_legal(a, nclass)) {
    p.family = CONV_STEM;
    return p;
  }
  if (choose_igemm8(a, nclass, &p)) {
    p.family = CONV_IGEMM8;
    return p;
  }
  const int big_mode = knobs().has_igemm_big ? knobs().igemm_big : -1;
  const long items256 = (long)cdiv(a.N * a.Hsub * a.Wsub, 256) * nclass * (a.Ncols / 256);
  const int mt = max_taps(a, nclass);
  const int cus = device_cus();
  const bool big = a.Ncols % 256 == 0 && (big_mode < 0 ? (items256 * 4 >= 3L * cus && mt * a.Ck >= 256 && !a.bn_y) : big_mode == 1);
  const long items3 = (long)cdiv(a.N * a.Hsub * a.Wsub, 256) * nclass * (a.Ncols / 128);
  const bool tall = a.Ncols % 128 == 0 &&
                    (big_mode < 0 ? ((items3 <= cus && items3 * 2 >= cus && mt * a.Ck >= 512) || (items3 <= 2L * cus && mt == 1 && a.Ck >= 1024)) : big_mode == 3);
  p.bm = big || tall ? 256 : 128;
  p.bn = big ? 256 : (tall || wide ? 128 : 64);
  return p;
}

bool leaky_sums_args(int dtype, const IgemmArgs& a) { return dtype == MI355_BF16 && a.bn_y && a.stat_partial && a.bn_slope == 0.01f && !knobs().error[0]; }
bool takes_leaky_sums(const ConvPick& p) { return p.family == CONV_DCONV || p.family == CONV_PO || p.family == CONV_PK; }
bool takes_bn_in(const ConvPick& p) { return p.family == CONV_DCONV || p.family == CONV_PO; }
bool takes_sub2(const ConvPick& p) { return p.family == CONV_PO; }

}

bool igemm_leaky_sums_legal(int dtype, const IgemmArgs& a, int nclass) {
  ConvPick p;
  return leaky_sums_args(dtype, a) && select_generated(a, nclass, &p) && takes_leaky_sums(p);
}

bool igemm_sub2_legal(int dtype, const IgemmArgs& a, int nclass) {
  ConvPick p;
  return dtype == MI355_BF16 && a.addend_sub2 && select_generated(a, nclass, &p) && takes_sub2(p);
}

bool igemm_bn_in_legal(int dtype, const IgemmArgs& a, int nclass) {
  ConvPick p;
  return dtype == MI355_BF16 && a.bn_in != nullptr && select_generated(a, nclass, &p) && takes_bn_in(p);
}

int launch_igemm(int dtype, const IgemmArgs& a, int nclass, hipStream_t stream, int* stat_rows) {
  const int bk = BKB / (int)dtype_size(dtype);
  MI355_ARG(a.in && a.wt && a.out, "igemm: null pointer");
  MI355_ARG(a.Ck % bk == 0, "igemm: Ck=%d not a multiple of %d", a.Ck, bk);
  MI355_ARG(a.Ncols % 64 == 0, "igemm: Ncols=%d not a multiple of 64", a.Ncols);
  MI355_ARG(nclass >= 1 && nclass <= 4, "igemm: nclass=%d", nclass);
  MI355_ARG(((size_t)a.pix_stride * dtype_size(dtype)) % 8 == 0, "igemm: pixel stride not 8-byte aligned");
  MI355_ARG(a.N > 0 && a.Hsub > 0 && a.Wsub > 0, "igemm: empty problem");
  MI355_ARG(!knobs().error[0], "%s", knobs().error);
  const long tiles128 = (long)cdiv(a.N * a.Hsub * a.Wsub, 128) * nclass * (a.Ncols / 128);
  const bool wide = (a.Ncols % 128 == 0) && tiles128 * 2 >= device_cus();
  MI355_ARG(dtype == MI355_BF16 || !a.addend_sub2, "igemm: a half-resolution addend needs the generated pointwise kernel (igemm_sub2_legal)");
  ConvPick p;
  p.bm = 128;
  p.bn = wide ? 128 : 64;
  if (dtype == MI355_BF16) p = select_bf16(a, nclass, wide);
  MI355_ARG(a.bn_slope == 0.f || (leaky_sums_args(dtype, a) && takes_leaky_sums(p)), "igemm: BN-backward sums under a leaky mask need a generated kernel with that epilogue and slope 0.01 (igemm_leaky_sums_legal)");
  MI355_ARG(a.bn_in == nullptr || takes_bn_in(p), "igemm: the input's BatchNorm in the operand path needs a generated kernel with that form (igemm_bn_in_legal)");
  if (dtype != MI355_F32 && dtype != MI355_BF16) {
    set_error("igemm: bad dtype %d", dtype);
    return MI355_E_ARG;
  }
  MI355_ARG(!a.addend_sub2 || p.family == CONV_DCONV || p.family == CONV_PO, "igemm: a half-resolution addend needs the generated pointwise kernel (igemm_sub2_legal)");
  switch (p.family) {
    case CONV_STEM: return launch_stem_direct(a, stream, stat_rows);
    case CONV_IGEMM8: return launch_igemm8(a, nclass, p.bm, p.bn, p.korder, p.fat, stream, stat_rows);
    case CONV_TILE: return launch_igemm_tile(dtype, a, nclass, p.bm, p.bn, stream, stat_rows);
    default: return launch_gen(p, a, nclass, 1.f, stream, stat_rows);
  }
}

bool igemm_fp8_legal(const IgemmArgs& a, int nclass) { return igemm8_fp8_legal(a, nclass, 128); }

int launch_igemm_fp8(const IgemmArgs& a, int nclass, float oscale, hipStream_t stream, int* stat_rows) {
  ConvPick p;
  if (dconv_pick(a, nclass, 1, &p)) return launch_gen(p, a, nclass, oscale, stream, stat_rows);
  const long long M = (long long)a.N * a.Hsub * a.Wsub;
  const bool wide8 = a.Ncols % 256 == 0 && ((M + 223) / 224) * nclass * (a.Ncols / 256) * 10 >= 7LL * device_cus();
  MI355_ARG(wide8 || a.Ncols % 128 == 0, "conv fp8: %d output columns (a multiple of 128 is needed)", a.Ncols);
  const int bm = wide8 ? 224 : 256, bn = wide8 ? 256 : 128;
  return launch_igemm8_fp8(a, nclass, bm, bn, max_taps(a, nclass) > 1 ? 1 : 0, oscale, stream, stat_rows);
}

}
```

sota_imagenet_amd/csrc/resnet_exec.cpp:

```cpp
#include <cstdlib>
#include <string>
#include <vector>

#include "flat_model.h"

namespace mi355 {

namespace {

constexpr float BN_EPS = 1e-5f;
constexpr float FP8_HEADROOM = 2.f;
constexpr size_t PARAM_ALIGN = 64;
constexpr int MAX_EVENTS = 8192;

struct ConvBN {
  std::string conv_name, bn_name;
  int Cin, Cout, K, stride, pad;
  int Hin, Win, Hout, Wout;
  size_t w_off = 0, gamma_off = 0, beta_off = 0;
  size_t rm_off = 0, rv_off = 0;
  void* y = nullptr;
  void* w_cast = nullptr;
  void* w_tr = nullptr;
  float* stat = nullptr;
  int splits = 1;
  int splits8 = 1;
  int stat_rows = 0;
  int bwd_rows = 0;
  bool is_stem = false;
  bool fp8_fwd = false, fp8_dgrad = false, fp8_wgrad = false;
  void* w_q = nullptr;
  void* w_trq = nullptr;
  const void* in_q = nullptr;
  int qid_w = -1, qid_in = -1, qid_dy = -1;
  char k_fwd[48] = "", k_dgrad[48] = "", k_wgrad[48] = "";
};

struct Block {
  ConvBN c1, c2, c3, ds;
  bool has_ds = false;
  const void* in = nullptr;
  void* a1 = nullptr;
  void* a2 = nullptr;
  void* out = nullptr;
  uint8_t *a1_bits = nullptr, *a2_bits = nullptr, *out_bits = nullptr;
  uint8_t *a1_q = nullptr, *a2_q = nullptr, *out_q = nullptr;
  int qid_a1 = -1, qid_a2 = -1, qid_out = -1;
  int Hin, Win, Hout, Wout, Cin, Cout;
};

}
}

using namespace mi355;

constexpr int MAX_GSETS = 4;

struct mi355_ctx : FlatModel {
  int fc_pad = 0;
  size_t es = 4;
  ConvBN stem;
  std::vector<Block> blocks;
  size_t fc_w_off = 0, fc_b_off = 0;

  void *xpad = nullptr, *stem_pack = nullptr, *p0 = nullptr;
  uint8_t* pool_idx = nullptr;
  uint8_t* a0_bits = nullptr;
  float *pooled = nullptr, *fc_tmp = nullptr, *dlogits_pad = nullptr, *dpooled = nullptr, *fc_wtr = nullptr;
  float *bn_partial = nullptr, *bn_coef = nullptr, *wg_partial = nullptr;
  float *bn_partial2 = nullptr, *bn_coef2 = nullptr;
  void* sk_ws[2] = {nullptr, nullptr};
  bool stream_k = true;
  bool fp8 = false;
  int q_n = 0;
  float* q_scale = nullptr;
  unsigned* q_amax = nullptr;
  void* gq[MAX_GSETS][4] = {};
  bool fp8_fwd_cal = false, fp8_bwd_cal = false;
  bool fp8_fwd_on = false, fp8_bwd_on = false;
  bool fp8_use_fwd = true, fp8_use_bwd = true;
  bool fp8_use_wgrad = true;
  bool fp8_keep_bf16 = false;
  bool fp8_lean = false;
  unsigned* sk_err_host = nullptr;
  PrepDesc* prep_table[2] = {nullptr, nullptr};
  int prep_layers = 0, prep_tiles = 0;
  void* gG[2] = {nullptr, nullptr};
  void* gsub = nullptr;
  bool ds_compact = true;
  void* gset[MAX_GSETS][4] = {};
  size_t max_c = 64;
  int nsets = 2;
  bool fuse_bn_bwd = false;
  bool fuse_bn_in = true;
  bool stem_fused_bwd = true;
  hipEvent_t w_done[MAX_GSETS] = {};
  hipEvent_t ds_done = nullptr;
  bool w_pending[MAX_GSETS] = {};
  int bwd_parity = 0;
  bool fwd_training_done = false;
  int next_seg = 0;
  void* cur_dout = nullptr;
  double fwd_flops = 0, train_flops = 0;

  unsigned prof_mask = 0;
  std::vector<hipEvent_t> ev;
  struct Rec {
    int cls;
    int tag;
    double flops, bytes;
  };
  std::vector<Rec> recs;
};

namespace {

size_t act_bytes(const mi355_ctx* c, int H, int W, int C) { return (size_t)c->N * H * W * C * c->es; }

void add_param(mi355_ctx* c, std::vector<TensorInfo>& rev, const std::string& name, size_t* off, int ndim, int s0,
               int s1 = 0, int s2 = 0, int s3 = 0, size_t extra_pad = 0) {
  size_t n = (size_t)s0 * (ndim > 1 ? s1 : 1) * (ndim > 2 ? s2 : 1) * (ndim > 3 ? s3 : 1);
  *off = c->param_elems;
  c->param_elems += align_up(n + extra_pad, PARAM_ALIGN);
  TensorInfo t{name, 0, *off, ndim, {s0, s1, s2, s3}};
  rev.push_back(t);
}
void add_buffer(mi355_ctx* c, std::vector<TensorInfo>& rev, const std::string& name, size_t* off, int n) {
  *off = c->buffer_elems;
  c->buffer_elems += align_up((size_t)n, PARAM_ALIGN);
  TensorInfo t{name, 1, *off, 1, {n, 0, 0, 0}};
  rev.push_back(t);
}

void init_conv(ConvBN& l, const std::string& conv_name, const std::string& bn_name, int Cin, int Cout, int K,
               int stride, int Hin, int Win) {
  l.conv_name = conv_name;
  l.bn_name = bn_name;
  l.Cin = Cin; l.Cout = Cout; l.K = K; l.stride = stride; l.pad = K / 2;
  l.Hin = Hin; l.Win = Win;
  l.Hout = (Hin + 2 * l.pad - K) / stride + 1;
  l.Wout = (Win + 2 * l.pad - K) / stride + 1;
}

void register_convbn(mi355_ctx* c, std::vector<TensorInfo>& rev, ConvBN& l) {
  add_param(c, rev, l.bn_name + ".bias", &l.beta_off, 1, l.Cout);
  add_param(c, rev, l.bn_name + ".weight", &l.gamma_off, 1, l.Cout);
  add_param(c, rev, l.conv_name + ".weight", &l.w_off, 4, l.Cout, l.Cin, l.K, l.K);
  add_buffer(c, rev, l.bn_name + ".running_var", &l.rv_off, l.Cout);
  add_buffer(c, rev, l.bn_name + ".running_mean", &l.rm_off, l.Cout);
}

struct Prof {
  mi355_ctx* c;
  hipStream_t stream;
  int idx = -1;
  Prof(mi355_ctx* ctx, int cls, double flops, double bytes, hipStream_t s, int tag = 0) : c(ctx), stream(s) {
    if (!(c->prof_mask & (1u << cls))) return;
    if ((c->recs.size() + 1) * 2 > c->ev.size()) return;
    idx = (int)c->recs.size();
    c->recs.push_back({cls, tag, flops, bytes});
    (void)hipEventRecord(c->ev[2 * idx], stream);
  }
  ~Prof() {
    if (idx >= 0) (void)hipEventRecord(c->ev[2 * idx + 1], stream);
  }
};

enum { PC_IGEMM128 = 0, PC_IGEMM64 = 1, PC_WGRAD128 = 2, PC_WGRAD64 = 3, PC_BN_REDUCE = 4, PC_BN_APPLY = 5, PC_OTHER = 6,
       PC_BN_BWD_APPLY = 7 };
inline int igemm_class(int ncols) { return ncols % 128 == 0 ? PC_IGEMM128 : PC_IGEMM64; }
inline int wgrad_class(int cout) { return cout % 128 == 0 ? PC_WGRAD128 : PC_WGRAD64; }

inline float* bn_partial_of(mi355_ctx* c, hipStream_t s) { return (c->wstream && s == c->wstream) ? c->bn_partial2 : c->bn_partial; }
inline void* sk_ws_of(mi355_ctx* c, hipStream_t s) {
  return c->stream_k ? c->sk_ws[(c->wstream && s == c->wstream) ? 1 : 0] : nullptr;
}
inline float* bn_coef_of(mi355_ctx* c, hipStream_t s) { return (c->wstream && s == c->wstream) ? c->bn_coef2 : c->bn_coef; }
double conv_flops(const mi355_ctx* c, const ConvBN& l) {
  return 2.0 * c->N * l.Hout * l.Wout * (double)l.Cout * l.Cin * l.K * l.K;
}

int conv_forward(mi355_ctx* c, ConvBN& l, const void* in, int training, float momentum, hipStream_t s, const ConvBN* bn_in = nullptr,
                 void* a_out = nullptr, uint8_t* a_bits = nullptr) {
  IgemmArgs a;
  build_fwd_args(a, c->N, l.Hin, l.Win, l.Cin, l.Cout, l.K, l.K, l.stride, l.pad);
  a.in = in;
  if (bn_in) {
    a.bn_in = bn_in->stat + 2 * bn_in->Cout;
    a.bn_in_a = a_out;
    a.bn_in_bits = a_bits;
  }
  a.stat_partial = training ? bn_partial_of(c, s) : nullptr;
  a.stat_rows_cap = (int)((size_t)bn_max_blocks() * c->max_c / l.Cout);
  a.sk_ws = sk_ws_of(c, s);
  a.wt = c->dtype == MI355_F32 ? (const void*)(c->params + l.w_off) : (const void*)l.w_cast;
  a.out = l.y;
  const double fl = conv_flops(c, l);
  const bool q = training && c->fp8_fwd_on && l.fp8_fwd;
  const double by = (double)c->N * l.Hin * l.Win * l.Cin * (q ? 1 : c->es) * (bn_in ? 2.0 + 1.0 / 16 : 1.0) + (double)c->N * l.Hout * l.Wout * l.Cout * c->es;
  Prof p(c, igemm_class(l.Cout), fl, by, s, (l.K == 3 ? 1 : 0) | (q ? 2 : 0));
  if (q) {
    a.in = l.in_q; a.wt = l.w_q;
    a.q_scale_in = c->q_scale + l.qid_in; a.q_scale_wt = c->q_scale + l.qid_w;
    MI355_TRY(launch_igemm_fp8(a, 1, 1.f, s, &l.stat_rows));
  } else {
    MI355_TRY(launch_igemm(c->dtype, a, 1, s, &l.stat_rows));
  }
  snprintf(l.k_fwd, sizeof(l.k_fwd), "%s", mi355_last_conv_kernel());
  return 0;
}

bool conv_bn_in_legal(mi355_ctx* c, const ConvBN& prev, const ConvBN& l, int training) {
  if (!training || c->dtype != MI355_BF16 || c->fp8 || !c->fuse_bn_in) return false;
  IgemmArgs a;
  build_fwd_args(a, c->N, l.Hin, l.Win, l.Cin, l.Cout, l.K, l.K, l.stride, l.pad);
  a.in = prev.y; a.wt = l.w_cast; a.out = l.y;
  a.stat_partial = c->bn_partial;
  a.stat_rows_cap = (int)((size_t)bn_max_blocks() * c->max_c / l.Cout);
  a.bn_in = prev.stat; a.bn_in_a = prev.y; a.bn_in_bits = (uint8_t*)prev.y;
  return igemm_bn_in_legal(c->dtype, a, 1);
}

int bn_prepare(mi355_ctx* c, ConvBN& l, int training, float momentum, hipStream_t s) {
  const int M = c->N * l.Hout * l.Wout, C = l.Cout;
  float* save_mean = l.stat;
  float* save_invstd = l.stat + C;
  float* scale = l.stat + 2 * C;
  float* shift = l.stat + 3 * C;
  const float* gamma = c->params + l.gamma_off;
  const float* beta = c->params + l.beta_off;
  if (training) {
    int nblk = l.stat_rows;
    const float* pivot = nullptr;
    if (nblk == 0) {
      Prof p(c, PC_BN_REDUCE, 0, (double)M * C * c->es, s);
      MI355_TRY(launch_bn_stats(c->dtype, l.y, bn_partial_of(c, s), bn_coef_of(c, s), &nblk, M, C, s));
      pivot = bn_coef_of(c, s);
    }
    return launch_bn_finalize(bn_partial_of(c, s), pivot, nblk, M, C, gamma, beta, c->buffers + l.rm_off, c->buffers + l.rv_off,
                              save_mean, save_invstd, scale, shift, BN_EPS, momentum, s);
  }
  return launch_bn_eval_coeffs(gamma, beta, c->buffers + l.rm_off, c->buffers + l.rv_off, scale, shift, C, BN_EPS, s);
}

int bn_apply(mi355_ctx* c, ConvBN& l, const void* residual, ConvBN* l2, void* out, int relu, hipStream_t s,
             uint8_t* bits, uint8_t* q = nullptr, int qid = -1, bool q_only = false) {
  const int M = c->N * l.Hout * l.Wout, C = l.Cout;
  const int nin = 1 + (residual ? 1 : 0) + (l2 ? 1 : 0);
  QuantOut qo;
  if (q && bits && qid >= 0) {
    qo.q = q; qo.scale = c->q_scale + qid; qo.amax = c->q_amax + qid;
    qo.only = q_only && !residual && !l2;
  }
  Prof p(c, PC_BN_APPLY, 0, (double)M * C * (c->es * (nin + (qo.only ? 0 : 1)) + (qo.q ? 1 : 0)), s);
  return launch_bn_apply(c->dtype, l.y, l.stat + 2 * C, l.stat + 3 * C, residual, l2 ? l2->y : nullptr,
                         l2 ? l2->stat + 2 * C : nullptr, l2 ? l2->stat + 3 * C : nullptr, out, M, C, relu, s, bits, qo);
}

void* grad_twin(const mi355_ctx* c, const void* g) {
  for (int p = 0; p < c->nsets; ++p)
    for (int i = 0; i < 4; ++i)
      if (c->gset[p][i] == g) return c->gq[p][i];
  return nullptr;
}

int bn_backward(mi355_ctx* c, ConvBN& l, const void* g, const uint8_t* bits, void* dz_out, void* dx, float beta_acc,
                hipStream_t s) {
  const int M = c->N * l.Hout * l.Wout, C = l.Cout;
  int nblk = l.bwd_rows;
  l.bwd_rows = 0;
  const double mask_bytes = bits ? (double)M * C * c->es / 16 : 0.0;
  if (nblk == 0 || dz_out) {
    Prof p(c, PC_BN_REDUCE, 0, (double)M * C * c->es * (2 + (dz_out ? 1 : 0)) + mask_bytes, s);
    MI355_TRY(launch_bn_bwd_reduce(c->dtype, g, nullptr, l.y, l.stat, l.stat + C, dz_out, bn_partial_of(c, s), &nblk, M, C, s,
                                   bits, 0.f));
  }
  MI355_TRY(launch_bn_bwd_finalize(bn_partial_of(c, s), nblk, M, C, c->params + l.gamma_off, l.stat + C,
                                     c->grads + l.gamma_off, c->grads + l.beta_off, beta_acc, bn_coef_of(c, s), s));
  const uint8_t* bits2 = dz_out ? nullptr : bits;
  const void* g2 = dz_out ? dz_out : g;
  QuantOut qo;
  if (c->fp8 && l.qid_dy >= 0) {
    qo.q = (uint8_t*)grad_twin(c, dx); qo.scale = c->q_scale + l.qid_dy; qo.amax = c->q_amax + l.qid_dy;
    qo.only = c->fp8_lean && c->fp8_bwd_on && l.fp8_dgrad && l.fp8_wgrad && qo.q;
  }
  Prof p(c, PC_BN_BWD_APPLY, 0, (double)M * C * (c->es * (qo.only ? 2 : 3) + (qo.q ? 1 : 0)) + (bits2 ? mask_bytes : 0.0), s);
  return launch_bn_bwd_apply(c->dtype, g2, nullptr, l.y, l.stat, l.stat + C, bn_coef_of(c, s), dx, M, C, s, bits2, 0.f, qo);
}

int conv_wgrad(mi355_ctx* c, ConvBN& l, const void* dy, const void* x, float beta_acc, hipStream_t s) {
  WgradArgs a;
  build_wgrad_args(a, c->N, l.Hin, l.Win, l.Cin, l.Cout, l.K, l.K, l.stride, l.pad);
  a.dy = dy; a.x = x; a.partial = c->wg_partial;
  const size_t n = (size_t)l.Cout * l.K * l.K * l.Cin;
  void* dyq = c->fp8_bwd_on && l.fp8_wgrad ? grad_twin(c, dy) : nullptr;
  const double by = ((double)c->N * l.Hin * l.Win * l.Cin + (double)c->N * l.Hout * l.Wout * l.Cout) * (dyq ? 1 : c->es);
  if (dyq) {
    a.dy = dyq; a.x = l.in_q;
    {
      Prof p(c, wgrad_class(l.Cout), conv_flops(c, l), by, s, 2);
      MI355_TRY(launch_wgrad(MI355_FP8, a, l.splits8, s));
    }
    snprintf(l.k_wgrad, sizeof(l.k_wgrad), "%s", mi355_last_conv_kernel());
    return launch_splitk_reduce(c->wg_partial, l.splits8, n, c->grads + l.w_off, n, beta_acc, s, c->q_scale + l.qid_dy, c->q_scale + l.qid_in);
  }
  {
    Prof p(c, wgrad_class(l.Cout), conv_flops(c, l), by, s);
    MI355_TRY(launch_wgrad(c->dtype, a, l.splits, s));
  }
  snprintf(l.k_wgrad, sizeof(l.k_wgrad), "%s", mi355_last_conv_kernel());
  return launch_splitk_reduce(c->wg_partial, l.splits, n, c->grads + l.w_off, n, beta_acc, s);
}

int conv_dgrad(mi355_ctx* c, ConvBN& l, const void* dy, void* dx, const void* addend, hipStream_t s,
               const uint8_t* addend_bits = nullptr, ConvBN* bn = nullptr, const uint8_t* bn_bits = nullptr, float beta_acc = 0.f, bool sub2 = false) {
  IgemmArgs a;
  const int nclass = build_dgrad_args(a, c->N, l.Hin, l.Win, l.Cin, l.Cout, l.K, l.K, l.stride, l.pad);
  if (nclass < 0) return nclass;
  a.in = dy; a.wt = l.w_tr; a.out = dx; a.addend = addend; a.addend_bits = addend_bits; a.addend_sub2 = sub2 ? 1 : 0;
  a.sk_ws = sk_ws_of(c, s);
  if (bn && c->fuse_bn_bwd) {
    a.stat_partial = bn_partial_of(c, s);
    a.stat_rows_cap = (int)((size_t)bn_max_blocks() * c->max_c / bn->Cout);
    a.bn_y = bn->y; a.bn_bits = bn_bits; a.bn_mean = bn->stat; a.bn_invstd = bn->stat + bn->Cout;
  }
  const double dx_elems = (double)c->N * l.Hin * l.Win * l.Cin;
  void* dyq = c->fp8_bwd_on && l.fp8_dgrad ? grad_twin(c, dy) : nullptr;
  const double by = dx_elems * (1 + (addend ? (sub2 ? 0.25 : 1) : 0) + (a.bn_y ? 1 : 0)) * c->es + (double)c->N * l.Hout * l.Wout * l.Cout * (dyq ? 1 : c->es) +
                    dx_elems * c->es / 16 * ((addend_bits ? 1 : 0) + (a.bn_y ? 1 : 0));
  Prof p(c, igemm_class(l.Cin), conv_flops(c, l), by, s, (l.K == 3 ? 1 : 0) | (dyq ? 2 : 0));
  int* rows = bn && c->fuse_bn_bwd ? &bn->bwd_rows : nullptr;
  if (dyq) {
    a.in = dyq; a.wt = l.w_trq;
    a.q_scale_in = c->q_scale + l.qid_dy; a.q_scale_wt = c->q_scale + l.qid_w;
    MI355_TRY(launch_igemm_fp8(a, nclass, 1.f, s, rows));
  } else {
    MI355_TRY(launch_igemm(c->dtype, a, nclass, s, rows));
  }
  snprintf(l.k_dgrad, sizeof(l.k_dgrad), "%s", mi355_last_conv_kernel());
  return 0;
}

int conv_dgrad_compact(mi355_ctx* c, ConvBN& l, const void* dy, void* dxs, hipStream_t s) {
  IgemmArgs a;
  const int nclass = build_dgrad_args(a, c->N, l.Hout, l.Wout, l.Cin, l.Cout, 1, 1, 1, 0);
  if (nclass < 0) return nclass;
  a.in = dy; a.wt = l.w_tr; a.out = dxs;
  const double px = (double)c->N * l.Hout * l.Wout;
  Prof p(c, igemm_class(l.Cin), 2.0 * px * l.Cin * l.Cout, px * (l.Cin + l.Cout) * c->es, s, 0);
  MI355_TRY(launch_igemm(c->dtype, a, nclass, s, nullptr));
  snprintf(l.k_dgrad, sizeof(l.k_dgrad), "%s", mi355_last_conv_kernel());
  return 0;
}

bool sub2_ok(mi355_ctx* c, Block& b, Block* prev) {
  if (!c->ds_compact || c->dtype != MI355_BF16 || !b.has_ds || b.ds.stride != 2 || b.ds.K != 1) return false;
  if (c->fp8 && b.ds.fp8_dgrad) return false;
  IgemmArgs a;
  ConvBN& l = b.c1;
  const int nclass = build_dgrad_args(a, c->N, l.Hin, l.Win, l.Cin, l.Cout, l.K, l.K, l.stride, l.pad);
  if (nclass < 0) return false;
  a.in = a.wt = a.addend = (const void*)1;
  a.out = (void*)1;
  a.addend_sub2 = 1;
  if (prev && c->fuse_bn_bwd) {
    a.stat_partial = (float*)1; a.bn_y = (const void*)1; a.bn_bits = (const uint8_t*)1; a.bn_mean = a.bn_invstd = (const float*)1;
    a.stat_rows_cap = (int)((size_t)bn_max_blocks() * c->max_c / prev->c3.Cout);
  }
  return igemm_sub2_legal(c->dtype, a, nclass);
}

int plan_arena(mi355_ctx* c, Arena& ar) {
  const int N = c->N;
  size_t max_act = 0, max_wg = 0, max_c = 64;
  auto conv_ws = [&](ConvBN& l) {
    ar.add(&l.y, act_bytes(c, l.Hout, l.Wout, l.Cout));
    ar.add((void**)&l.stat, (size_t)4 * l.Cout * 4);
    max_act = std::max(max_act, act_bytes(c, l.Hout, l.Wout, l.Cout));
    max_act = std::max(max_act, act_bytes(c, l.Hin, l.Win, l.Cin));
    max_c = std::max<size_t>(max_c, l.Cout);
    if (!l.is_stem) {
      const size_t wn = (size_t)l.Cout * l.K * l.K * l.Cin;
      if (c->dtype != MI355_F32) ar.add(&l.w_cast, wn * c->es);
      ar.add(&l.w_tr, wn * c->es);
      if (l.qid_w >= 0) {
        ar.add(&l.w_q, wn);
        ar.add(&l.w_trq, wn);
      }
      WgradArgs wa;
      build_wgrad_args(wa, N, l.Hin, l.Win, l.Cin, l.Cout, l.K, l.K, l.stride, l.pad);
      l.splits = plan_wgrad(c->dtype, wa);
      l.splits8 = c->fp8 ? plan_wgrad_splits(c->dtype, N * l.Hout * l.Wout, l.Cout, l.K * l.K, l.Cin) : l.splits;
      max_wg = std::max(max_wg, (size_t)std::max(l.splits, l.splits8) * wn * 4);
    } else {
      l.splits = plan_wgrad_splits(c->dtype, N * l.Hout * l.Wout, 64, 4, STEM_CK);
      max_wg = std::max(max_wg, (size_t)l.splits * 64 * 4 * 64 * 4);
    }
  };
  ar.add(&c->xpad, mi355_stem_xpad_bytes(c->dtype, N, c->H, c->W));
  ar.add(&c->stem_pack, (size_t)64 * 4 * 64 * c->es);
  conv_ws(c->stem);
  ar.add((void**)&c->a0_bits, act_bytes(c, c->stem.Hout, c->stem.Wout, 64) / 16);
  ar.add(&c->p0, act_bytes(c, c->stem.Hout / 2, c->stem.Wout / 2, 64));
  ar.add((void**)&c->pool_idx, (size_t)N * (c->stem.Hout / 2) * (c->stem.Wout / 2) * 64);
  for (auto& b : c->blocks) {
    conv_ws(b.c1);
    ar.add(&b.a1, act_bytes(c, b.c1.Hout, b.c1.Wout, b.c1.Cout));
    ar.add((void**)&b.a1_bits, act_bytes(c, b.c1.Hout, b.c1.Wout, b.c1.Cout) / 16);
    conv_ws(b.c2);
    ar.add(&b.a2, act_bytes(c, b.c2.Hout, b.c2.Wout, b.c2.Cout));
    ar.add((void**)&b.a2_bits, act_bytes(c, b.c2.Hout, b.c2.Wout, b.c2.Cout) / 16);
    conv_ws(b.c3);
    if (b.has_ds) conv_ws(b.ds);
    ar.add(&b.out, act_bytes(c, b.Hout, b.Wout, b.Cout));
    ar.add((void**)&b.out_bits, act_bytes(c, b.Hout, b.Wout, b.Cout) / 16);
    if (b.qid_a1 >= 0) ar.add((void**)&b.a1_q, act_bytes(c, b.c1.Hout, b.c1.Wout, b.c1.Cout) / c->es);
    if (b.qid_a2 >= 0) ar.add((void**)&b.a2_q, act_bytes(c, b.c2.Hout, b.c2.Wout, b.c2.Cout) / c->es);
    if (b.qid_out >= 0) ar.add((void**)&b.out_q, act_bytes(c, b.Hout, b.Wout, b.Cout) / c->es);
  }
  const int fcp = c->fc_pad;
  ar.add((void**)&c->pooled, (size_t)N * 2048 * 4);
// ... 67 lines not shown
      l.fp8_wgrad = c->fp8_use_wgrad && l.fp8_fwd && l.qid_in >= 0 && l.Cin % 128 == 0 && l.Cout % 128 == 0;
      if (!plan_all) {
        if (l.K == 3 && l.stride == 1) l.fp8_wgrad = false;
        if (l.K == 1 && l.stride == 1 && l.Cin * l.Cout == 2048 * 512) l.fp8_wgrad = false;
      }
      if (l.fp8_wgrad && l.qid_dy < 0) l.qid_dy = n++;
    };
    wg_plan(b.c1); wg_plan(b.c2); wg_plan(b.c3);
    if (b.has_ds) wg_plan(b.ds);
  }
  c->q_n = (int)align_up((size_t)n, 64);
}

int weight_prep_all(mi355_ctx* c, bool need_tr, hipStream_t s) {
  Prof p(c, PC_OTHER, 0, 0, s);
  MI355_TRY(launch_stem_pack(c->dtype, c->params + c->stem.w_off, c->stem_pack, s));
  if (need_tr || c->dtype != MI355_F32)
    MI355_TRY(launch_weight_prep_batch(c->dtype, c->prep_table[need_tr ? 1 : 0], c->prep_layers, c->prep_tiles, c->params, s));
  if (need_tr)
    MI355_TRY(launch_weight_prep(MI355_F32, c->params + c->fc_w_off, nullptr, c->fc_wtr, c->fc_pad, 1, 2048, s));
  return 0;
}

int acquire_set(mi355_ctx* c, int p, hipStream_t s) {
  if (c->overlap && c->w_pending[p]) {
    MI355_HIP(hipStreamWaitEvent(s, c->w_done[p], 0));
    c->w_pending[p] = false;
  }
  return 0;
}
int release_set(mi355_ctx* c, int p) {
  if (c->overlap) {
    MI355_HIP(hipEventRecord(c->w_done[p], c->wstream));
    c->w_pending[p] = true;
  }
  return 0;
}
int sk_check(mi355_ctx* c) {
  if (c->sk_err_host && (c->sk_err_host[0] | c->sk_err_host[1])) {
    set_error("a stream-K hand-off of an earlier convolution launch timed out (partial tile lost): the results of that "
              "step are invalid; recreate the context (MI355_STREAM_K=0 disables the tile cutting)");
    return MI355_E_STATE;
  }
  return 0;
}
int sk_snapshot(mi355_ctx* c, hipStream_t s) {
  if (!c->sk_err_host || !c->stream_k) return 0;
  for (int i = 0; i < 2; ++i)
    if (c->sk_ws[i])
      MI355_HIP(hipMemcpyAsync(c->sk_err_host + i, reinterpret_cast<unsigned*>(c->sk_ws[i]) + IGEMM_SK_ERR_WORD, sizeof(unsigned),
                               hipMemcpyDeviceToHost, s));
  return 0;
}

int backward_fc(mi355_ctx* c, const float* dlogits, float beta_acc, hipStream_t s) {
  const int N = c->N, O = c->num_classes, P = c->fc_pad;
  MI355_TRY(launch_pad_dlogits(dlogits, c->dlogits_pad, P, c->grads + c->fc_b_off, beta_acc, N, O, s));
  WgradArgs w;
  build_wgrad_args(w, N, 1, 1, 2048, P, 1, 1, 1, 0);
  w.dy = c->dlogits_pad; w.x = c->pooled; w.partial = c->wg_partial;
  const int splits = plan_wgrad_splits(MI355_F32, N, P, 1, 2048);
  hipStream_t ws;
  MI355_TRY(c->fork(s, &ws));
  MI355_TRY(launch_wgrad(MI355_F32, w, splits, ws));
  MI355_TRY(launch_splitk_reduce(c->wg_partial, splits, (size_t)P * 2048, c->grads + c->fc_w_off, (size_t)O * 2048,
                                 beta_acc, ws));
  MI355_TRY(launch_fc(c->dlogits_pad, c->fc_wtr, c->dpooled, N, 2048, P, s));
  const Block& last = c->blocks.back();
  c->cur_dout = c->gG[0];
  c->bwd_parity = 0;
  return launch_gap_bwd(c->dtype, c->dpooled, c->cur_dout, N, last.Hout * last.Wout, last.Cout, s);
}

int backward_block(mi355_ctx* c, Block& b, Block* prev, float beta_acc, hipStream_t s) {
  void* G = c->cur_dout;
  void* Gn = G == c->gG[0] ? c->gG[1] : c->gG[0];
  const int par = c->bwd_parity;
  c->bwd_parity = (par + 1) % c->nsets;
  void** S = c->gset[par];
  void *B1 = S[0], *B2 = S[1], *B3 = S[2], *B4 = S[3];
  hipStream_t ws;
  const bool sub2 = sub2_ok(c, b, prev);
  MI355_TRY(acquire_set(c, par, s));
  MI355_TRY(bn_backward(c, b.c3, G, b.out_bits, nullptr, B1, beta_acc, s));
  MI355_TRY(c->fork(s, &ws));
  MI355_TRY(conv_wgrad(c, b.c3, B1, b.a2, beta_acc, ws));
  if (b.has_ds) {
    MI355_TRY(bn_backward(c, b.ds, G, b.out_bits, nullptr, B2, beta_acc, ws));
    if (sub2) MI355_TRY(conv_dgrad_compact(c, b.ds, B2, c->gsub, ws));
    else MI355_TRY(conv_dgrad(c, b.ds, B2, Gn, nullptr, ws));
    if (c->overlap) MI355_HIP(hipEventRecord(c->ds_done, ws));
    MI355_TRY(conv_wgrad(c, b.ds, B2, b.in, beta_acc, ws));
  }
  MI355_TRY(conv_dgrad(c, b.c3, B1, B3, nullptr, s, nullptr, &b.c2, b.a2_bits, beta_acc));
  MI355_TRY(bn_backward(c, b.c2, B3, b.a2_bits, nullptr, B3, beta_acc, s));
  MI355_TRY(c->fork(s, &ws));
  MI355_TRY(conv_wgrad(c, b.c2, B3, b.a1, beta_acc, ws));
  MI355_TRY(conv_dgrad(c, b.c2, B3, B4, nullptr, s, nullptr, &b.c1, b.a1_bits, beta_acc));
  MI355_TRY(bn_backward(c, b.c1, B4, b.a1_bits, nullptr, B4, beta_acc, s));
  MI355_TRY(c->fork(s, &ws));
  MI355_TRY(conv_wgrad(c, b.c1, B4, b.in, beta_acc, ws));
  if (b.has_ds) {
    if (c->overlap) MI355_HIP(hipStreamWaitEvent(s, c->ds_done, 0));
    MI355_TRY(conv_dgrad(c, b.c1, B4, Gn, sub2 ? c->gsub : Gn, s, nullptr, prev ? &prev->c3 : nullptr, prev ? prev->out_bits : nullptr, beta_acc, sub2));
    c->cur_dout = Gn;
  } else {
    MI355_TRY(conv_dgrad(c, b.c1, B4, G, G, s, b.out_bits, prev ? &prev->c3 : nullptr, prev ? prev->out_bits : nullptr, beta_acc));
    c->cur_dout = G;
  }
  return release_set(c, par);
}

int backward_stem(mi355_ctx* c, float beta_acc, hipStream_t s) {
  void* G = c->cur_dout;
  const int par = c->bwd_parity;
  c->bwd_parity = (par + 1) % c->nsets;
  void* B1 = c->gset[par][0];
  ConvBN& l = c->stem;
  MI355_TRY(acquire_set(c, par, s));
  if (c->stem_fused_bwd) {
    const int M = c->N * l.Hout * l.Wout, C = l.Cout;
    const double full = (double)M * C * c->es, pooled = full / 4 + (double)M * C / 4, mask = full / 16;
    int nblk = 0;
    {
      Prof p(c, PC_BN_REDUCE, 0, full + pooled + mask, s);
      MI355_TRY(launch_stem_bwd_reduce(c->dtype, G, c->pool_idx, c->a0_bits, l.y, l.stat, l.stat + C, bn_partial_of(c, s), &nblk, c->N, l.Hout,
                                       l.Wout, C, s));
    }
    MI355_TRY(launch_bn_bwd_finalize(bn_partial_of(c, s), nblk, M, C, c->params + l.gamma_off, l.stat + C, c->grads + l.gamma_off,
                                     c->grads + l.beta_off, beta_acc, bn_coef_of(c, s), s));
    Prof p(c, PC_BN_BWD_APPLY, 0, 2 * full + pooled + mask, s);
    MI355_TRY(launch_stem_bwd_apply(c->dtype, G, c->pool_idx, c->a0_bits, l.y, l.stat, l.stat + C, bn_coef_of(c, s), B1, c->N, l.Hout, l.Wout, C, s));
  } else {
    {
      Prof p(c, PC_OTHER, 0, 0, s);
      MI355_TRY(launch_maxpool_bwd(c->dtype, G, c->pool_idx, B1, c->N, l.Hout, l.Wout, 64, s));
    }
    MI355_TRY(bn_backward(c, l, B1, c->a0_bits, nullptr, B1, beta_acc, s));
  }
  WgradArgs a;
  build_stem_wgrad_args(a, c->N, c->H, c->W);
  a.dy = B1; a.x = c->xpad; a.partial = c->wg_partial;
  hipStream_t ws;
  MI355_TRY(c->fork(s, &ws));
  {
    Prof p(c, PC_WGRAD64, conv_flops(c, l), 0, ws);
    MI355_TRY(launch_wgrad(c->dtype, a, l.splits, ws));
    snprintf(l.k_wgrad, sizeof(l.k_wgrad), "%s", mi355_last_conv_kernel());
  }
  MI355_TRY(launch_stem_unpack(c->wg_partial, l.splits, c->grads + l.w_off, beta_acc, ws));
  return release_set(c, par);
}

}

extern "C" {

int mi355_resnet50_create(mi355_ctx** out, int device, int dtype, int N, int H, int W, int num_classes) {
  MI355_ARG(out, "create: null out");
  MI355_ARG(dtype == MI355_F32 || dtype == MI355_BF16 || dtype == MI355_FP8, "create: bad dtype %d", dtype);
  const bool fp8 = dtype == MI355_FP8;
  if (fp8) dtype = MI355_BF16;
  MI355_ARG(N >= 1 && H >= 32 && W >= 32 && H % 32 == 0 && W % 32 == 0, "create: N=%d H=%d W=%d (H,W multiples of 32)",
            N, H, W);
  MI355_ARG(num_classes >= 1 && num_classes <= 65536, "create: num_classes=%d", num_classes);
  if (device >= 0) MI355_HIP(hipSetDevice(device));
  mi355_ctx* c = new mi355_ctx();
  c->device = device; c->dtype = dtype; c->N = N; c->H = H; c->W = W; c->num_classes = num_classes;
  c->fc_pad = (int)align_up((size_t)num_classes, 128);
  c->es = dtype_size(dtype);
  c->fp8 = fp8;

  init_conv(c->stem, "conv1", "bn1", 3, 64, 7, 2, H, W);
  c->stem.is_stem = true;
  int h = c->stem.Hout / 2, w = c->stem.Wout / 2, cin = 64;
  const int nblk[4] = {3, 4, 6, 3};
  const int planes[4] = {64, 128, 256, 512};
  for (int st = 0; st < 4; ++st) {
    for (int i = 0; i < nblk[st]; ++i) {
      Block b;
      const int p = planes[st];
      const int stride = (i == 0 && st > 0) ? 2 : 1;
      const std::string pre = "layer" + std::to_string(st + 1) + "." + std::to_string(i) + ".";
      b.Hin = h; b.Win = w; b.Cin = cin; b.Cout = 4 * p;
      init_conv(b.c1, pre + "conv1", pre + "bn1", cin, p, 1, 1, h, w);
      init_conv(b.c2, pre + "conv2", pre + "bn2", p, p, 3, stride, h, w);
      init_conv(b.c3, pre + "conv3", pre + "bn3", p, 4 * p, 1, 1, b.c2.Hout, b.c2.Wout);
      b.has_ds = (i == 0);
      if (b.has_ds) init_conv(b.ds, pre + "downsample.0", pre + "downsample.1", cin, 4 * p, 1, stride, h, w);
      b.Hout = b.c2.Hout; b.Wout = b.c2.Wout;
      h = b.Hout; w = b.Wout; cin = 4 * p;
      c->blocks.push_back(b);
    }
  }
  std::vector<TensorInfo> rev;
  size_t seg_begin = c->param_elems;
  auto end_segment = [&] {
    c->segs.push_back({seg_begin, c->param_elems});
    seg_begin = c->param_elems;
  };
  add_param(c, rev, "fc.bias", &c->fc_b_off, 1, num_classes);
  add_param(c, rev, "fc.weight", &c->fc_w_off, 2, num_classes, 2048, 0, 0,
            (size_t)(c->fc_pad - num_classes) * 2048);
  end_segment();
  for (int i = (int)c->blocks.size() - 1; i >= 0; --i) {
    Block& b = c->blocks[i];
    if (b.has_ds) register_convbn(c, rev, b.ds);
    register_convbn(c, rev, b.c3);
    register_convbn(c, rev, b.c2);
    register_convbn(c, rev, b.c1);
    end_segment();
  }
  register_convbn(c, rev, c->stem);
  end_segment();
  c->tensors.assign(rev.rbegin(), rev.rend());

  double f = conv_flops(c, c->stem), bw = 2 * conv_flops(c, c->stem) - conv_flops(c, c->stem);
  double tr = 2 * conv_flops(c, c->stem);
  (void)bw;
  for (auto& b : c->blocks) {
    const double fb = conv_flops(c, b.c1) + conv_flops(c, b.c2) + conv_flops(c, b.c3) + (b.has_ds ? conv_flops(c, b.ds) : 0);
    f += fb;
    tr += 3 * fb;
  }
  const double ffc = 2.0 * N * 2048 * num_classes;
  c->fwd_flops = f + ffc;
  c->train_flops = tr + 3 * ffc;

  const char* bad = nullptr;
  if (c->fp8) {
    plan_fp8(c, &bad);
    c->fp8_use_fwd = env_switch("MI355_FP8_FWD", 1, 1, &bad) != 0;
    c->fp8_use_bwd = env_switch("MI355_FP8_BWD", 1, 1, &bad) != 0;
  }
  c->stream_k = env_switch("MI355_STREAM_K", 1, 1, &bad) != 0;
  c->fuse_bn_bwd = env_switch("MI355_FUSE_BN_BWD", dtype == MI355_BF16 ? 1 : 0, 1, &bad) != 0;
  c->stem_fused_bwd = env_switch("MI355_STEM_FUSED", 1, 1, &bad) != 0;
  c->overlap = env_switch("MI355_WGRAD_STREAM", 1, 1, &bad) != 0;
  c->ds_compact = env_switch("MI355_DS_COMPACT", 1, 1, &bad) != 0;
  if (bad) {
    set_error("create: %s=%s is outside the switch's domain", bad, getenv(bad));
    mi355_resnet50_destroy(c);
    return MI355_E_ARG;
  }
  Arena ar;
  plan_arena(c, ar);
  c->arena_bytes = ar.size;
  if (device < 0) {
    *out = c;
    return 0;
  }
  hipError_t e = hipMalloc((void**)&c->arena, ar.size);
  if (e != hipSuccess) {
    set_error("create: hipMalloc(%zu bytes) -> %s", ar.size, hipGetErrorString(e));
    delete c;
    return MI355_E_NOMEM;
  }
  for (auto& sl : ar.slots) *sl.first = c->arena + sl.second;
  e = hipMemset(c->arena, 0, ar.size);
  if (e != hipSuccess) {
    set_error("create: hipMemset -> %s", hipGetErrorString(e));
    delete c;
    return MI355_E_HIP;
  }
  if (c->fp8) {
    for (size_t i = 0; i < c->blocks.size(); ++i) {
      Block& b = c->blocks[i];
      if (i > 0) b.c1.in_q = b.ds.in_q = c->blocks[i - 1].out_q;
      b.c2.in_q = b.a1_q;
      b.c3.in_q = b.a2_q;
    }
    std::vector<float> ones(c->q_n, 1.f);
    if (hipMemcpy(c->q_scale, ones.data(), ones.size() * 4, hipMemcpyHostToDevice) != hipSuccess) {
      set_error("create: fp8 scale table upload failed");
      mi355_resnet50_destroy(c);
      return MI355_E_HIP;
    }
  }
  {
    std::vector<PrepDesc> tab[2];
    int tiles = 0;
    auto add = [&](ConvBN& l) {
      PrepDesc d;
      d.w_off = l.w_off; d.w_cast = l.w_cast; d.w_tr = nullptr;
      d.w_q = d.w_trq = nullptr; d.q_scale = nullptr; d.q_amax = nullptr;
      d.Cout = l.Cout; d.taps = l.K * l.K; d.Cin = l.Cin; d.tile_begin = tiles;
      tab[0].push_back(d);
      d.w_tr = l.w_tr;
      if (l.qid_w >= 0) {
        d.w_q = l.w_q; d.w_trq = l.w_trq;
        d.q_scale = c->q_scale + l.qid_w; d.q_amax = c->q_amax + l.qid_w;
      }
      tab[1].push_back(d);
      tiles += (l.Cout / PREP_TILE) * (l.Cin / PREP_TILE) * l.K * l.K;
    };
    for (auto& b : c->blocks) {
      add(b.c1); add(b.c2); add(b.c3);
      if (b.has_ds) add(b.ds);
    }
    c->prep_layers = (int)tab[0].size();
    c->prep_tiles = tiles;
    bool ok = c->prep_layers <= 64;
    for (int i = 0; i < 2 && ok; ++i)
      ok = hipMemcpy(c->prep_table[i], tab[i].data(), tab[i].size() * sizeof(PrepDesc), hipMemcpyHostToDevice) == hipSuccess;
    if (!ok) {
      set_error("create: weight-prep table upload failed");
      mi355_resnet50_destroy(c);
      return MI355_E_HIP;
    }
  }
  if (c->stream_k && dtype == MI355_F32) {
    if (hipHostMalloc((void**)&c->sk_err_host, 2 * sizeof(unsigned), hipHostMallocDefault) != hipSuccess) {
      set_error("create: hipHostMalloc -> %s", hipGetErrorString(hipGetLastError()));
      mi355_resnet50_destroy(c);
      return MI355_E_HIP;
    }
    c->sk_err_host[0] = c->sk_err_host[1] = 0;
  }
  if (c->overlap) {
    bool ok = c->create_side_stream(true, 16);
    for (auto& ev : c->w_done) ok = ok && hipEventCreateWithFlags(&ev, hipEventDisableTiming) == hipSuccess;
    ok = ok && hipEventCreateWithFlags(&c->ds_done, hipEventDisableTiming) == hipSuccess;
// ... 166 lines not shown
  }
  return sk_snapshot(c, s);
}

int mi355_resnet50_debug_tensor(const mi355_ctx* c, const char* name, void** ptr, int* dtype, int* ndim,
                                int shape[4]) {
  MI355_ARG(c && name && ptr && dtype && ndim && shape, "debug_tensor: null argument");
  const std::string n(name);
  auto set4 = [&](void* p, int dt, int h, int w, int ch) {
    *ptr = p; *dtype = dt; *ndim = 4;
    shape[0] = c->N; shape[1] = h; shape[2] = w; shape[3] = ch;
    return 0;
  };
  auto set1 = [&](void* p, int len) {
    *ptr = p; *dtype = MI355_F32; *ndim = 1;
    shape[0] = len; shape[1] = shape[2] = shape[3] = 0;
    return 0;
  };
  auto setq = [&](const void* p, int d0, int d1, int d2, int d3) {
    if (!p) return 1;
    *ptr = const_cast<void*>(p); *dtype = MI355_FP8; *ndim = 4;
    shape[0] = d0; shape[1] = d1; shape[2] = d2; shape[3] = d3;
    return 0;
  };
  auto conv_match = [&](const ConvBN& l) -> int {
    if (c->fp8 && l.qid_w >= 0) {
      if (n == l.conv_name + ".xq" && l.fp8_fwd) return setq(l.in_q, c->N, l.Hin, l.Win, l.Cin);
      if (n == l.conv_name + ".wq") return setq(l.w_q, l.Cout, l.K, l.K, l.Cin);
      if (n == l.conv_name + ".wtq") return setq(l.w_trq, l.Cin, l.K, l.K, l.Cout);
      if (n == l.conv_name + ".sx" && l.fp8_fwd) return set1(c->q_scale + l.qid_in, 1);
      if (n == l.conv_name + ".sw") return set1(c->q_scale + l.qid_w, 1);
      if (n == l.conv_name + ".sdy" && l.fp8_dgrad) return set1(c->q_scale + l.qid_dy, 1);
      if (n == l.conv_name + ".amax_w") return set1(reinterpret_cast<float*>(c->q_amax + l.qid_w), 1);
    }
    if (n == l.conv_name + ".y") return set4(l.y, c->dtype, l.Hout, l.Wout, l.Cout);
    if (n == l.bn_name + ".save_mean") return set1(l.stat, l.Cout);
    if (n == l.bn_name + ".save_invstd") return set1(l.stat + l.Cout, l.Cout);
    return 1;
  };
  if (conv_match(c->stem) == 0) return 0;
  if (n == "stem.p0") return set4(c->p0, c->dtype, c->stem.Hout / 2, c->stem.Wout / 2, 64);
  for (const auto& b : c->blocks) {
    if (conv_match(b.c1) == 0 || conv_match(b.c2) == 0 || conv_match(b.c3) == 0) return 0;
    if (b.has_ds && conv_match(b.ds) == 0) return 0;
    const std::string pre = b.c1.conv_name.substr(0, b.c1.conv_name.size() - 5);
    if (n == pre + "a1") return set4(b.a1, c->dtype, b.c1.Hout, b.c1.Wout, b.c1.Cout);
    if (n == pre + "a2") return set4(b.a2, c->dtype, b.c2.Hout, b.c2.Wout, b.c2.Cout);
    if (n == pre + "out") return set4(b.out, c->dtype, b.Hout, b.Wout, b.Cout);
  }
  const Block& last = c->blocks.back();
  if (n == "pooled" || n == "dpooled") {
    *ptr = n == "pooled" ? c->pooled : c->dpooled; *dtype = MI355_F32; *ndim = 2;
    shape[0] = c->N; shape[1] = 2048; shape[2] = shape[3] = 0;
    return 0;
  }
  for (int i = 0; i < 2; ++i)
    if (n == "gG" + std::to_string(i)) return set4(c->gG[i], c->dtype, last.Hout, last.Wout, last.Cout);
  if (n == "grad.cur") {
    const int nb = (int)c->blocks.size();
    if (c->next_seg >= 1 && c->next_seg <= nb) {
      const Block& b = c->blocks[nb - c->next_seg];
      return set4(c->cur_dout, c->dtype, b.Hout, b.Wout, b.Cout);
    }
    if (c->next_seg == nb + 1) return set4(c->cur_dout, c->dtype, c->stem.Hout / 2, c->stem.Wout / 2, 64);
    set_error("debug_tensor: 'grad.cur' exists between backward segments only (next segment %d)", c->next_seg);
    return MI355_E_STATE;
  }
  set_error("debug_tensor: unknown tensor '%s'", name);
  return MI355_E_ARG;
}

int mi355_resnet50_force_grad(mi355_ctx* c, const void* g, size_t bytes, void* stream) {
  MI355_ARG(c && g, "force_grad: null argument");
  const int nb = (int)c->blocks.size();
  if (!c->fwd_training_done || c->next_seg < 1 || c->next_seg > nb + 1) {
    set_error("force_grad: only between two backward segments (next segment %d)", c->next_seg);
    return MI355_E_STATE;
  }
  size_t want;
  if (c->next_seg <= nb) {
    Block& b = c->blocks[nb - c->next_seg];
    want = (size_t)c->N * b.Hout * b.Wout * b.Cout * c->es;
    b.c3.bwd_rows = 0;
  } else {
    want = (size_t)c->N * (c->stem.Hout / 2) * (c->stem.Wout / 2) * 64 * c->es;
  }
  MI355_ARG(bytes == want, "force_grad: %zu bytes given, the pending gradient has %zu", bytes, want);
  MI355_HIP(hipMemcpyAsync(c->cur_dout, g, bytes, hipMemcpyDeviceToDevice, (hipStream_t)stream));
  return 0;
}

int mi355_resnet50_fp8_state(const mi355_ctx* c, int* fwd_on, int* bwd_on, int* n_fwd_layers, int* n_dgrad_layers) {
  MI355_ARG(c, "fp8_state: null ctx");
  int nf = 0, nd = 0;
  auto count = [&](const ConvBN& l) {
    nf += l.fp8_fwd ? 1 : 0;
    nd += l.fp8_dgrad ? 1 : 0;
  };
  for (const auto& b : c->blocks) {
    count(b.c1); count(b.c2); count(b.c3);
    if (b.has_ds) count(b.ds);
  }
  if (fwd_on) *fwd_on = c->fp8 && c->fp8_fwd_on;
  if (bwd_on) *bwd_on = c->fp8 && c->fp8_bwd_on;
  if (n_fwd_layers) *n_fwd_layers = nf;
  if (n_dgrad_layers) *n_dgrad_layers = nd;
  return 0;
}

int mi355_resnet50_flops(const mi355_ctx* c, double* fwd, double* train) {
  MI355_ARG(c, "flops: null ctx");
  if (fwd) *fwd = c->fwd_flops;
  if (train) *train = c->train_flops;
  return 0;
}

int mi355_resnet50_kernel_table(const mi355_ctx* c, char* out, size_t cap, size_t* needed) {
  MI355_ARG(c && (out || cap == 0), "kernel_table: bad arguments");
  std::string t;
  auto line = [&](const ConvBN& l) {
    t += l.conv_name + " fwd=" + (l.k_fwd[0] ? l.k_fwd : "-") + " dgrad=" + (l.k_dgrad[0] ? l.k_dgrad : "-") + " wgrad=" + (l.k_wgrad[0] ? l.k_wgrad : "-") + "\n";
  };
  line(c->stem);
  for (const Block& b : c->blocks) {
    line(b.c1); line(b.c2); line(b.c3);
    if (b.has_ds) line(b.ds);
  }
  if (needed) *needed = t.size() + 1;
  if (cap > 0) {
    const size_t n = std::min(cap - 1, t.size());
    memcpy(out, t.data(), n);
    out[n] = 0;
  }
  return 0;
}

int mi355_resnet50_profile(mi355_ctx* c, int class_mask) {
  MI355_ARG(c, "profile: null ctx");
  MI355_HIP(hipSetDevice(c->device));
  if (class_mask && c->ev.empty()) {
    c->ev.resize(MAX_EVENTS);
    for (auto& e : c->ev) MI355_HIP(hipEventCreate(&e));
  }
  c->prof_mask = (unsigned)class_mask;
  c->recs.clear();
  return 0;
}

int mi355_resnet50_profile_read(mi355_ctx* c, int kind, double* total_ms, int* launches, double* alg_flops,
                                double* alg_bytes) {
  MI355_ARG(c && kind >= 0 && kind < 32, "profile_read: bad arguments");
  double ms = 0, fl = 0, by = 0;
  int n = 0;
  for (size_t i = 0; i < c->recs.size(); ++i) {
    const bool match = kind == 8 ? ((c->recs[i].tag & 1) && c->recs[i].cls <= 1) : kind == 9 ? (c->recs[i].tag & 2) != 0 : c->recs[i].cls == kind;
    if (!match) continue;
    float t = 0;
    MI355_HIP(hipEventSynchronize(c->ev[2 * i + 1]));
    MI355_HIP(hipEventElapsedTime(&t, c->ev[2 * i], c->ev[2 * i + 1]));
    ms += t; fl += c->recs[i].flops; by += c->recs[i].bytes;
    ++n;
  }
  MI355_TRY(sk_check(c));
  if (total_ms) *total_ms = ms;
  if (launches) *launches = n;
  if (alg_flops) *alg_flops = fl;
// ... 6 lines not shown
```

sota_imagenet_amd/ops.py:

```python
import ctypes

import torch

from . import native
from .native import check, cur_stream, dtype_code, ptr


def _L():
    return native.lib()


def _need_cuda(*ts):
    for t in ts:
        if t is not None and not (t.is_cuda and t.is_contiguous()):
            raise ValueError("tensors must be contiguous CUDA (ROCm) tensors")


def _out_dim(h, k, s, p):
    return (h + 2 * p - k) // s + 1


def conv2d_fwd(x, w, stride=1, pad=0, stats=False):
    _need_cuda(x, w)
    N, H, W, Cin = x.shape
# ... 42 lines not shown
    return y


def conv2d_dgrad_fp8(dyq, wq, x_shape, stride=1, pad=0, oscale=1.0, wt=None):
    _need_cuda(dyq, wq)
    N, H, W, Cin = x_shape
    Cout, KH, KW, _ = wq.shape
    if wt is None:
        wt = wq.view(torch.uint8).permute(3, 1, 2, 0).contiguous()
    dx = torch.empty((N, H, W, Cin), dtype=torch.bfloat16, device=dyq.device)
    check(_L().mi355_conv2d_dgrad_fp8(ptr(dyq), ptr(wt), ptr(dx), float(oscale), N, H, W, Cin, Cout, KH, KW, stride, pad, cur_stream()))
    return dx


_WGRAD_WS = {}


def conv2d_wgrad_fp8(dyq, xq, KH, KW, stride=1, pad=0, oscale=1.0):
    _need_cuda(dyq, xq)
    N, H, W, Cin = xq.shape
    Cout = dyq.shape[-1]
    n = _L().mi355_conv2d_workspace_bytes(native.BF16, N, H, W, Cin, Cout, KH, KW, stride, pad)
    key = (dyq.device, torch.cuda.current_stream(dyq.device).cuda_stream, n)
    ws = _WGRAD_WS.get(key)
    if ws is None:
        while len(_WGRAD_WS) >= 8:
            _WGRAD_WS.pop(next(iter(_WGRAD_WS)))
        ws = _WGRAD_WS[key] = torch.empty(n + 256, dtype=torch.uint8, device=dyq.device)
    dw = torch.empty((Cout, KH, KW, Cin), dtype=torch.float32, device=dyq.device)
    check(_L().mi355_conv2d_wgrad_fp8(ptr(dyq), ptr(xq), ptr(dw), 0.0, float(oscale), N, H, W, Cin, Cout, KH, KW, stride, pad, ptr(ws), n + 256, cur_stream()))
    return dw


def ingest_u8(packed, table_host, table_dev, S, mean=127.5, std=51.0, aug_host=None, aug_dev=None):
    _need_cuda(packed, table_dev, aug_dev)
    N = int(table_host.shape[0])
    if table_host.dtype.itemsize != 40 or table_dev.numel() * table_dev.element_size() != 40 * N or not table_host.flags["C_CONTIGUOUS"]:
        raise ValueError("ingest_u8: the descriptor table must be N contiguous 40-byte mi355_crop records on both sides")
    out = torch.empty((N, 3, S, S), dtype=torch.float32, device=packed.device)
    if aug_host is None:
        check(_L().mi355_ingest_u8(ptr(packed), packed.numel(), table_host.ctypes.data, ptr(table_dev), N, int(S), float(mean), float(std), ptr(out), cur_stream()))
        return out
    if aug_host.dtype.itemsize != 128 or aug_host.shape[0] != N or aug_dev is None or aug_dev.numel() * aug_dev.element_size() != 128 * N or not aug_host.flags["C_CONTIGUOUS"]:
        raise ValueError("ingest_u8: the augment table must be N contiguous 128-byte mi355_augment records on both sides")
    scratch = torch.empty((N, 3, S, S), dtype=torch.float32, device=packed.device) if bool((aug_host["blur_sigma"] > 0).any()) else None
    check(_L().mi355_ingest_u8_aug(ptr(packed), packed.numel(), table_host.ctypes.data, ptr(table_dev), aug_host.ctypes.data, ptr(aug_dev), N, int(S),
                                   float(mean), float(std), ptr(scratch), ptr(out), cur_stream()))
    return out


def _conv_ws(dt, N, H, W, Cin, Cout, KH, KW, stride, pad, device):
    n = _L().mi355_conv2d_workspace_bytes(dt, N, H, W, Cin, Cout, KH, KW, stride, pad)
    return torch.empty(n, dtype=torch.uint8, device=device), n


def conv2d_dgrad(dy, w, x_shape, stride=1, pad=0, addend=None):
    _need_cuda(dy, w, addend)
    N, H, W, Cin = x_shape
    Cout, KH, KW, _ = w.shape
    dt = dtype_code(dy.dtype)
    ws, n = _conv_ws(dt, N, H, W, Cin, Cout, KH, KW, stride, pad, dy.device)
    dx = torch.empty((N, H, W, Cin), dtype=dy.dtype, device=dy.device)
    check(_L().mi355_conv2d_dgrad(dt, ptr(dy), ptr(w), ptr(dx), ptr(addend), N, H, W, Cin, Cout, KH, KW, stride, pad, ptr(ws), n, cur_stream()))
    return dx


def conv2d_dgrad_bn(dy, w, x_shape, stride=1, pad=0, addend=None, addend_bits=None, bn_y=None, bn_bits=None, bn_mean=None, bn_invstd=None, addend_sub2=False, slope=0.0):
    _need_cuda(dy, w, addend, addend_bits, bn_y, bn_bits, bn_mean, bn_invstd)
    N, H, W, Cin = x_shape
    Cout, KH, KW, _ = w.shape
    dt = dtype_code(dy.dtype)
    ws, n = _conv_ws(dt, N, H, W, Cin, Cout, KH, KW, stride, pad, dy.device)
    dx = torch.empty((N, H, W, Cin), dtype=dy.dtype, device=dy.device)
    part = None
    nblk = ctypes.c_int(0)
    if bn_y is not None:
        part = torch.empty((4096, 2, Cin), dtype=torch.float32, device=dy.device)
    check(_L().mi355_conv2d_dgrad_bn_leaky(dt, ptr(dy), ptr(w), ptr(dx), ptr(addend), ptr(addend_bits), int(addend_sub2), ptr(bn_y), ptr(bn_bits), ptr(bn_mean),
                                           ptr(bn_invstd), float(slope), ptr(part), 0 if part is None else part.numel() * 4, ctypes.byref(nblk), N, H, W, Cin, Cout,
                                           KH, KW, stride, pad, ptr(ws), n, cur_stream()))
    if part is not None:
        part = part[:nblk.value] if nblk.value > 0 else None
    return dx, part


def last_conv_kernel():
    return _L().mi355_last_conv_kernel().decode()


def conv2d_wgrad(dy, x, KH, KW, stride=1, pad=0, dw=None, beta=0.0):
    _need_cuda(dy, x, dw)
    N, H, W, Cin = x.shape
    Cout = dy.shape[-1]
    dt = dtype_code(dy.dtype)
    ws, n = _conv_ws(dt, N, H, W, Cin, Cout, KH, KW, stride, pad, dy.device)
    if dw is None:
        dw = torch.empty((Cout, KH, KW, Cin), dtype=torch.float32, device=dy.device)
    check(_L().mi355_conv2d_wgrad(dt, ptr(dy), ptr(x), ptr(dw), beta, N, H, W, Cin, Cout, KH, KW, stride, pad, ptr(ws), n, cur_stream()))
    return dw


def stem_ingest(x_nchw, dtype):
    _need_cuda(x_nchw)
    N, _, H, W = x_nchw.shape
    dt = dtype_code(dtype)
    nbytes = _L().mi355_stem_xpad_bytes(dt, N, H, W)
    xpad = torch.zeros(nbytes, dtype=torch.uint8, device=x_nchw.device)
    check(_L().mi355_stem_ingest(dt, ptr(x_nchw), ptr(xpad), N, H, W, cur_stream()))
    return xpad


def stem_fwd(xpad, w, N, H, W, dtype):
    _need_cuda(xpad, w)
    dt = dtype_code(dtype)
    n = _L().mi355_stem_workspace_bytes(dt, N, H, W)
    ws = torch.empty(n, dtype=torch.uint8, device=w.device)
    y = torch.empty((N, H // 2, W // 2, 64), dtype=dtype, device=w.device)
    check(_L().mi355_stem_fwd(dt, ptr(xpad), ptr(w), ptr(y), N, H, W, ptr(ws), n, cur_stream()))
    return y


def stem_wgrad(dy, xpad, N, H, W):
    _need_cuda(dy, xpad)
    dt = dtype_code(dy.dtype)
    n = _L().mi355_stem_workspace_bytes(dt, N, H, W)
    ws = torch.empty(n, dtype=torch.uint8, device=dy.device)
    dw = torch.empty((64, 7, 7, 3), dtype=torch.float32, device=dy.device)
    check(_L().mi355_stem_wgrad(dt, ptr(dy), ptr(xpad), ptr(dw), 0.0, N, H, W, ptr(ws), n, cur_stream()))
    return dw


def _bn_ws(C, device):
    n = _L().mi355_bn_workspace_bytes(C)
    return torch.empty(n, dtype=torch.uint8, device=device), n


def bn_fwd_train(x, gamma, beta, running_mean, running_var, residual=None, relu=True, eps=1e-5, momentum=0.1, stats=None):
    _need_cuda(x, gamma, beta, running_mean, running_var, residual)
    C = x.shape[-1]
    M = x.numel() // C
    out = torch.empty_like(x)
    sm = torch.empty(C, dtype=torch.float32, device=x.device)
    si = torch.empty(C, dtype=torch.float32, device=x.device)
    if stats is not None:
        _need_cuda(stats)
        if stats.dim() != 3 or stats.shape[1:] != (2, C) or stats.dtype != torch.float32:
            raise ValueError(f"bn_fwd_train: stats must be the fp32 [nblk, 2, {C}] rows conv2d_fwd(stats=True) returned for this tensor")
        ws = torch.empty(2 * C, dtype=torch.float32, device=x.device)
        check(_L().mi355_bn_fwd_train_partial(dtype_code(x.dtype), ptr(x), ptr(residual), ptr(out), ptr(gamma), ptr(beta), ptr(running_mean),
                                              ptr(running_var), ptr(sm), ptr(si), M, C, eps, momentum, int(relu), ptr(stats), stats.shape[0], ptr(ws),
                                              ws.numel() * 4, cur_stream()))
        return out, sm, si
    ws, n = _bn_ws(C, x.device)
    check(_L().mi355_bn_fwd_train(dtype_code(x.dtype), ptr(x), ptr(residual), ptr(out), ptr(gamma), ptr(beta), ptr(running_mean),
                                  ptr(running_var), ptr(sm), ptr(si), M, C, eps, momentum, int(relu), ptr(ws), n, cur_stream()))
    return out, sm, si


def bn_fwd_eval(x, gamma, beta, running_mean, running_var, residual=None, relu=True, eps=1e-5):
    _need_cuda(x, gamma, beta, running_mean, running_var, residual)
    C = x.shape[-1]
    M = x.numel() // C
    out = torch.empty_like(x)
    ws, n = _bn_ws(C, x.device)
    check(_L().mi355_bn_fwd_eval(dtype_code(x.dtype), ptr(x), ptr(residual), ptr(out), ptr(gamma), ptr(beta), ptr(running_mean),
                                 ptr(running_var), M, C, eps, int(relu), ptr(ws), n, cur_stream()))
# ... 517 lines not shown
```

Before: 14490 images/sec.

## Fuse downsample BN backward stats into dgrad epilogue and joint apply kernel

At blocks with a downsample branch, the BN backward reductions for the main c3 BN and the downsample BN share one incoming gradient. The dgrad epilogue of the next block's c1 now also accumulates the second BN's dz·xhat sum. A new kernel then applies both BN backward transforms in one pass, reading the gradient and bit mask once. This removes a separate reduce pass and a duplicate gradient read. In exchange it uses more LDS and registers in the STATS==3 igemm variant (occupancy is lowered to 2) and puts both BN applies on the main stream instead of splitting them across streams.

```diff
diff --git a/include/mi355rn.h b/include/mi355rn.h
--- a/include/mi355rn.h
+++ b/include/mi355rn.h
@@ -45,6 +45,10 @@
                                 const void* bn_y, const uint8_t* bn_bits, const float* bn_mean, const float* bn_invstd, float slope, float* partial,
                                 size_t partial_bytes, int* nblk, int N, int H, int W, int Cin, int Cout, int KH, int KW, int stride, int pad,
                                 void* ws, size_t ws_bytes, void* stream);
+int mi355_conv2d_dgrad_bn2(int dtype, const void* dy, const void* w, void* dx, const void* addend, const uint8_t* addend_bits, const void* bn_y,
+                           const uint8_t* bn_bits, const float* bn_mean, const float* bn_invstd, float* partial, const void* bn2_y,
+                           const float* bn2_mean, const float* bn2_invstd, float* partial2, size_t partial_bytes, int* nblk, int N, int H, int W,
+                           int Cin, int Cout, int KH, int KW, int stride, int pad, void* ws, size_t ws_bytes, void* stream);
 
 int mi355_conv2d_wgrad(int dtype, const void* dy, const void* x, float* dw, float beta, int N, int H,
                        int W, int Cin, int Cout, int KH, int KW, int stride, int pad, void* ws,
@@ -98,6 +102,11 @@
                  const float* save_mean, const float* save_invstd, void* dx, void* dz_out,
                  float* dgamma, float* dbeta, float beta_acc, int M, int C, int relu, void* ws,
                  size_t ws_bytes, void* stream);
+int mi355_bn_bwd_apply_bits(int dtype, const void* dout, const uint8_t* bits, const void* x, const float* save_mean, const float* save_invstd,
+                            const float* coef, void* dx, int M, int C, void* stream);
+int mi355_bn_bwd_apply2(int dtype, const void* dout, const uint8_t* bits, const void* xa, const float* mean_a, const float* invstd_a,
+                        const float* coef_a, void* dxa, const void* xb, const float* mean_b, const float* invstd_b, const float* coef_b, void* dxb,
+                        int M, int C, void* stream);
 
 int mi355_maxpool_fwd(int dtype, const void* x, void* y, uint8_t* idx, int N, int H, int W, int C,
                       void* stream);
diff --git a/sota_imagenet_amd/csrc/bn.hip b/sota_imagenet_amd/csrc/bn.hip
--- a/sota_imagenet_amd/csrc/bn.hip
+++ b/sota_imagenet_amd/csrc/bn.hip
@@ -432,6 +432,63 @@
     if constexpr (Q) quant8(gv, qs, p.qo.q + i * V, amax);
   }
   if constexpr (Q) amax_flush(amax, p.qo.amax);
+}
+
+struct BwdApply2Args {
+  const void* g;
+  const uint8_t* bits;
+  const void *xa, *xb;
+  const float *mean_a, *invstd_a, *coef_a;
+  const float *mean_b, *invstd_b, *coef_b;
+  void *dxa, *dxb;
+  size_t nvec;
+  int cvecs, C;
+};
+
+template <typename T, int MASK>
+__global__ __launch_bounds__(256) void bn_bwd_apply2_kernel(const BwdApply2Args p) {
+  static_assert(MASK == 0 || MASK == 2, "no mask or the ReLU bit mask");
+  constexpr int V = Vec16<T>::N;
+  const T* g = reinterpret_cast<const T*>(p.g);
+  const T* xa = reinterpret_cast<const T*>(p.xa);
+  const T* xb = reinterpret_cast<const T*>(p.xb);
+  T* dxa = reinterpret_cast<T*>(p.dxa);
+  T* dxb = reinterpret_cast<T*>(p.dxb);
+  const size_t stride = (size_t)gridDim.x * 256;
+  size_t i = (size_t)blockIdx.x * 256 + threadIdx.x;
+  const int c0 = (int)(i % p.cvecs) * V;
+  float mua[V], isa[V], a0[V], a1[V], a2[V];
+  float mub[V], isb[V], b0[V], b1[V], b2[V];
+  load_consts<V>(p.mean_a, c0, mua);
+  load_consts<V>(p.invstd_a, c0, isa);
+  load_consts<V>(p.coef_a, c0, a0);
+  load_consts<V>(p.coef_a + p.C, c0, a1);
+  load_consts<V>(p.coef_a + 2 * p.C, c0, a2);
+  load_consts<V>(p.mean_b, c0, mub);
+  load_consts<V>(p.invstd_b, c0, isb);
+  load_consts<V>(p.coef_b, c0, b0);
+  load_consts<V>(p.coef_b + p.C, c0, b1);
+  load_consts<V>(p.coef_b + 2 * p.C, c0, b2);
+  for (; i < p.nvec; i += stride) {
+    float gv[V], xv[V], yv[V], ra[V], rb[V];
+    Vec16<T>::load_nt(g + i * V, gv);
+    Vec16<T>::load_nt(xa + i * V, xv);
+    Vec16<T>::load_nt(xb + i * V, yv);
+    if constexpr (MASK == 2) {
+      const unsigned b = p.bits[i];
+#pragma unroll
+      for (int e = 0; e < V; ++e) gv[e] = (b >> e) & 1u ? gv[e] : 0.f;
+    }
+#pragma unroll
+    for (int e = 0; e < V; ++e) {
+      const float xh = (xv[e] - mua[e]) * isa[e];
+      ra[e] = a0[e] * (gv[e] - a1[e] - xh * a2[e]);
+      const float yh = (yv[e] - mub[e]) * isb[e];
+      rb[e] = b0[e] * (gv[e] - b1[e] - yh * b2[e]);
+    }
+    Vec16<T>::store(dxa + i * V, ra);
+    Vec16<T>::store(dxb + i * V, rb);
+  }
 }
 
 constexpr int SC = 64;
@@ -927,6 +984,31 @@
   return 0;
 }
 
+int launch_bn_bwd_apply2(int dtype, const void* g, const uint8_t* relu_bits, const void* xa, const float* mean_a, const float* invstd_a,
+                         const float* coef_a, void* dxa, const void* xb, const float* mean_b, const float* invstd_b, const float* coef_b,
+                         void* dxb, int M, int C, hipStream_t s) {
+  MI355_TRY(check_c(dtype, C));
+  const int V = 16 / (int)dtype_size(dtype);
+  BwdApply2Args a{};
+  a.g = g;
+  a.bits = relu_bits;
+  a.xa = xa; a.mean_a = mean_a; a.invstd_a = invstd_a; a.coef_a = coef_a; a.dxa = dxa;
+  a.xb = xb; a.mean_b = mean_b; a.invstd_b = invstd_b; a.coef_b = coef_b; a.dxb = dxb;
+  a.nvec = (size_t)M * C / V;
+  a.cvecs = C / V;
+  a.C = C;
+  const int blocks = elementwise_blocks(a.nvec, a.cvecs);
+  if (dtype == MI355_F32) {
+    if (relu_bits) hipLaunchKernelGGL((bn_bwd_apply2_kernel<float, 2>), dim3(blocks), dim3(256), 0, s, a);
+    else hipLaunchKernelGGL((bn_bwd_apply2_kernel<float, 0>), dim3(blocks), dim3(256), 0, s, a);
+  } else {
+    if (relu_bits) hipLaunchKernelGGL((bn_bwd_apply2_kernel<bf16_t, 2>), dim3(blocks), dim3(256), 0, s, a);
+    else hipLaunchKernelGGL((bn_bwd_apply2_kernel<bf16_t, 0>), dim3(blocks), dim3(256), 0, s, a);
+  }
+  MI355_LAUNCH_CHECK();
+  return 0;
+}
+
 static int stem_bwd_args(StemBwdArgs& a, int dtype, const void* dp, const uint8_t* idx, const uint8_t* bits, const void* y, const float* mean,
                          const float* invstd, int N, int H, int W, int C) {
   MI355_TRY(check_c(dtype, C));
diff --git a/sota_imagenet_amd/csrc/common.h b/sota_imagenet_amd/csrc/common.h
--- a/sota_imagenet_amd/csrc/common.h
+++ b/sota_imagenet_amd/csrc/common.h
@@ -79,6 +79,10 @@
   const uint8_t* bn_bits = nullptr;
   const float* bn_mean = nullptr;
   const float* bn_invstd = nullptr;
+  const void* bn2_y = nullptr;
+  const float* bn2_mean = nullptr;
+  const float* bn2_invstd = nullptr;
+  float* stat2_partial = nullptr;
   float bn_slope = 0.f;
   const float* bn_in = nullptr;
   void* bn_in_a = nullptr;
@@ -230,6 +234,9 @@
 int launch_bn_bwd_apply(int dtype, const void* g, const void* mask_src, const void* x, const float* mean,
                         const float* invstd, const float* coef, void* dx, int M, int C, hipStream_t s,
                         const uint8_t* relu_bits = nullptr, float slope = 0.f, QuantOut qo = QuantOut(), const EcaGrad* eg = nullptr);
+int launch_bn_bwd_apply2(int dtype, const void* g, const uint8_t* relu_bits, const void* xa, const float* mean_a, const float* invstd_a,
+                         const float* coef_a, void* dxa, const void* xb, const float* mean_b, const float* invstd_b, const float* coef_b,
+                         void* dxb, int M, int C, hipStream_t s);
 int launch_stem_bwd_reduce(int dtype, const void* dp, const uint8_t* idx, const uint8_t* bits, const void* y, const float* mean,
                            const float* invstd, float* partial, int* nblk_out, int N, int H, int W, int C, hipStream_t s);
 int launch_stem_bwd_apply(int dtype, const void* dp, const uint8_t* idx, const uint8_t* bits, const void* y, const float* mean,
diff --git a/sota_imagenet_amd/csrc/conv_api.cpp b/sota_imagenet_amd/csrc/conv_api.cpp
--- a/sota_imagenet_amd/csrc/conv_api.cpp
+++ b/sota_imagenet_amd/csrc/conv_api.cpp
@@ -388,6 +388,31 @@
   return launch_igemm(dtype, a, nclass, s, partial ? nblk : nullptr);
 }
 
+int mi355_conv2d_dgrad_bn2(int dtype, const void* dy, const void* w, void* dx, const void* addend, const uint8_t* addend_bits, const void* bn_y,
+                           const uint8_t* bn_bits, const float* bn_mean, const float* bn_invstd, float* partial, const void* bn2_y, const float* bn2_mean,
+                           const float* bn2_invstd, float* partial2, size_t partial_bytes, int* nblk, int N, int H, int W, int Cin, int Cout, int KH, int KW,
+                           int stride, int pad, void* ws, size_t ws_bytes, void* stream) {
+  MI355_TRY(check_conv(dtype, Cin, Cout, KH, KW, stride));
+  const size_t es = dtype_size(dtype);
+  const size_t wbytes = (size_t)Cin * KH * KW * Cout * es;
+  MI355_ARG(ws && ws_bytes >= wbytes, "dgrad_bn2: workspace too small (%zu < %zu)", ws_bytes, wbytes);
+  MI355_ARG(addend || !addend_bits, "dgrad_bn2: addend_bits without an addend");
+  MI355_ARG(partial && partial2 && bn_y && bn_bits && bn_mean && bn_invstd && bn2_y && bn2_mean && bn2_invstd && nblk, "dgrad_bn2: null pointer");
+  MI355_ARG(partial_bytes >= (size_t)768 * 2 * Cin * sizeof(float), "dgrad_bn2: each partial buffer needs 768 * 2 * Cin floats");
+  hipStream_t s = (hipStream_t)stream;
+  MI355_TRY(launch_transpose_any(dtype, w, ws, Cout, KH * KW, Cin, s));
+  IgemmArgs a;
+  const int nclass = build_dgrad_args(a, N, H, W, Cin, Cout, KH, KW, stride, pad);
+  if (nclass < 0) return nclass;
+  a.in = dy; a.wt = ws; a.out = dx; a.addend = addend; a.addend_bits = addend_bits;
+  a.stat_partial = partial;
+  a.stat_rows_cap = (int)std::min<size_t>(partial_bytes / ((size_t)2 * Cin * sizeof(float)), 1u << 20);
+  a.bn_y = bn_y; a.bn_bits = bn_bits; a.bn_mean = bn_mean; a.bn_invstd = bn_invstd;
+  a.bn2_y = bn2_y; a.bn2_mean = bn2_mean; a.bn2_invstd = bn2_invstd; a.stat2_partial = partial2;
+  *nblk = 0;
+  return launch_igemm(dtype, a, nclass, s, nblk);
+}
+
 int mi355_conv2d_wgrad(int dtype, const void* dy, const void* x, float* dw, float beta, int N, int H, int W, int Cin,
                        int Cout, int KH, int KW, int stride, int pad, void* ws, size_t ws_bytes, void* stream) {
   MI355_TRY(check_conv(dtype, Cin, Cout, KH, KW, stride));
@@ -498,6 +523,18 @@
   return launch_bn_bwd_apply(dtype, dout, mask, x, save_mean, save_invstd, coef, dx, M, C, s, nullptr, slope);
 }
 
+int mi355_bn_bwd_apply_bits(int dtype, const void* dout, const uint8_t* bits, const void* x, const float* save_mean, const float* save_invstd,
+                            const float* coef, void* dx, int M, int C, void* stream) {
+  MI355_ARG(dout && x && save_mean && save_invstd && coef && dx && M >= 1, "bn_bwd_apply_bits: null pointer");
+  return launch_bn_bwd_apply(dtype, dout, nullptr, x, save_mean, save_invstd, coef, dx, M, C, (hipStream_t)stream, bits, 0.f);
+}
+
+int mi355_bn_bwd_apply2(int dtype, const void* dout, const uint8_t* bits, const void* xa, const float* mean_a, const float* invstd_a, const float* coef_a,
+                        void* dxa, const void* xb, const float* mean_b, const float* invstd_b, const float* coef_b, void* dxb, int M, int C, void* stream) {
+  MI355_ARG(dout && xa && mean_a && invstd_a && coef_a && dxa && xb && mean_b && invstd_b && coef_b && dxb && M >= 1, "bn_bwd_apply2: null pointer");
+  return launch_bn_bwd_apply2(dtype, dout, bits, xa, mean_a, invstd_a, coef_a, dxa, xb, mean_b, invstd_b, coef_b, dxb, M, C, (hipStream_t)stream);
+}
+
 int mi355_maxpool_fwd(int dtype, const void* x, void* y, uint8_t* idx, int N, int H, int W, int C, void* stream) {
   return launch_maxpool_fwd(dtype, x, y, idx, N, H, W, C, (hipStream_t)stream);
 }
diff --git a/sota_imagenet_amd/csrc/conv_igemm.hip b/sota_imagenet_amd/csrc/conv_igemm.hip
--- a/sota_imagenet_amd/csrc/conv_igemm.hip
+++ b/sota_imagenet_amd/csrc/conv_igemm.hip
@@ -51,7 +51,7 @@
 }
 
 template <typename T, int BM, int BN, int WMW, int NSTG, int STATS>
-__global__ __launch_bounds__(128 * WMW, (BM == 256 ? 1 : (BN == 64 && NSTG == 2 ? 3 : 2))) void igemm_kernel(const IgemmKArgs kp) {
+__global__ __launch_bounds__(128 * WMW, (BM == 256 ? 1 : (BN == 64 && NSTG == 2 && STATS != 3 ? 3 : 2))) void igemm_kernel(const IgemmKArgs kp) {
   const IgemmArgs& p = kp.a;
   constexpr int ES = (int)sizeof(T);
   constexpr int BK = BKB / ES;
@@ -78,6 +78,7 @@
   static_assert(NW % EPI_WAVES == 0, "epilogue turns");
   int* row_pix = reinterpret_cast<int*>(smem + NSTG * STAGE);
   float* stat_acc = reinterpret_cast<float*>(smem + NSTG * STAGE + BM * sizeof(int));
+  float* stat_acc2 = stat_acc + WMW * kp.ntpg * BN * 2;
 
   const int tid = threadIdx.x;
   const int lane = tid & 63;
@@ -238,7 +239,7 @@
   }
 
   if constexpr (STATS != 0) {
-    for (int i = tid; i < WMW * kp.ntpg * BN * 2; i += NT) stat_acc[i] = 0.f;
+    for (int i = tid; i < WMW * kp.ntpg * BN * (STATS == 3 ? 3 : 2); i += NT) stat_acc[i] = 0.f;
   }
   L_setup();
   int stage = 0;
@@ -437,9 +438,9 @@
         if (EPI_TURNS == 1 || wave / EPI_WAVES == turn) {
         const int prw = lane & 31;
         const int rr = lane / CPR, ch = lane % CPR;
-        float s1[VEC], s2[VEC];
-        float bmu[VEC], bis[VEC];
-        if constexpr (STATS == 2) {
+        float s1[VEC], s2[VEC], s3[VEC];
+        float bmu[VEC], bis[VEC], bmu2[VEC], bis2[VEC];
+        if constexpr (STATS >= 2) {
           const int c0 = n0 + wn * WN + ch * VEC;
   #pragma unroll
           for (int q = 0; q < VEC / 4; ++q) {
@@ -450,12 +451,22 @@
               bmu[4 * q + e] = a[e];
               bis[4 * q + e] = b[e];
             }
+            if constexpr (STATS == 3) {
+              const f32x4 a2 = *reinterpret_cast<const f32x4*>(p.bn2_mean + c0 + 4 * q);
+              const f32x4 b2 = *reinterpret_cast<const f32x4*>(p.bn2_invstd + c0 + 4 * q);
+  #pragma unroll
+              for (int e = 0; e < 4; ++e) {
+                bmu2[4 * q + e] = a2[e];
+                bis2[4 * q + e] = b2[e];
+              }
+            }
           }
         }
   #pragma unroll
         for (int e = 0; e < VEC; ++e) {
           s1[e] = 0.f;
           s2[e] = 0.f;
+          s3[e] = 0.f;
         }
   #pragma unroll
         for (int mi = 0; mi < MI; ++mi) {
@@ -477,6 +488,7 @@
           uint4 araw[NP];
           unsigned abits[NP];
           uint4 yraw[NP];
+          uint4 y2raw[NP];
           unsigned ybits[NP];
   #pragma unroll
           for (int ps = 0; ps < NP; ++ps) {
@@ -486,9 +498,10 @@
               araw[ps] = *reinterpret_cast<const uint4*>((pixs[ps] < 0 || MI355_PROBE(4)) ? reinterpret_cast<const T*>(g_zero_page) : addend + o);
               abits[ps] = p.addend_bits ? (unsigned)p.addend_bits[pixs[ps] < 0 ? 0 : o / VEC] : 0xffu;
             }
-            if constexpr (STATS == 2) {
+            if constexpr (STATS >= 2) {
               const size_t o = (size_t)(pixs[ps] < 0 ? 0 : pixs[ps]) * p.Ncols + n0 + wn * WN + ch * VEC;
               yraw[ps] = *reinterpret_cast<const uint4*>(reinterpret_cast<const T*>(p.bn_y) + o);
+              if constexpr (STATS == 3) y2raw[ps] = *reinterpret_cast<const uint4*>(reinterpret_cast<const T*>(p.bn2_y) + o);
               ybits[ps] = (unsigned)p.bn_bits[o / VEC];
             }
           }
@@ -522,15 +535,17 @@
                 }
               }
             }
-            if constexpr (STATS == 2) {
+            if constexpr (STATS >= 2) {
               if (pix >= 0) {
-                float yv[VEC];
+                float yv[VEC], y2v[VEC];
                 Vec16<T>::unpack(yraw[ps], yv);
+                if constexpr (STATS == 3) Vec16<T>::unpack(y2raw[ps], y2v);
   #pragma unroll
                 for (int e = 0; e < VEC; ++e) {
                   const float dz = (ybits[ps] >> e) & 1u ? (float)(T)v[e] : 0.f;
                   s1[e] += dz;
                   s2[e] += dz * ((yv[e] - bmu[e]) * bis[e]);
+                  if constexpr (STATS == 3) s3[e] += dz * ((y2v[e] - bmu2[e]) * bis2[e]);
                 }
               }
             }
@@ -561,6 +576,22 @@
             slot[1] += b;
           }
           asm volatile("s_waitcnt lgkmcnt(0)" ::: "memory");
+          if constexpr (STATS == 3) {
+  #pragma unroll
+            for (int q = 0; q < VEC / 4; ++q) {
+              const f32x4 a = {s3[4 * q], s3[4 * q + 1], s3[4 * q + 2], s3[4 * q + 3]};
+              *reinterpret_cast<f32x4*>(scr + rr * WN + ch * VEC + 4 * q) = a;
+            }
+            asm volatile("s_waitcnt lgkmcnt(0)" ::: "memory");
+  #pragma unroll
+            for (int cc = lane; cc < WN; cc += 64) {
+              float a = 0.f;
+  #pragma unroll
+              for (int r = 0; r < RPI; ++r) a += scr[r * WN + cc];
+              stat_acc2[(wm * kp.ntpg + nti) * BN + wn * WN + cc] += a;
+            }
+            asm volatile("s_waitcnt lgkmcnt(0)" ::: "memory");
+          }
         }
         }
         if constexpr (EPI_TURNS > 1) MI355_LDS_BARRIER();
@@ -582,6 +613,14 @@
       }
       row[c] = a;
       row[p.Ncols + c] = b;
+      if constexpr (STATS == 3) {
+        float b2 = 0.f;
+#pragma unroll
+        for (int w = 0; w < WMW; ++w) b2 += stat_acc2[w * chan + c];
+        float* row2 = p.stat2_partial + (size_t)(bx / kp.ngroups) * 2 * p.Ncols + grp * chan;
+        row2[c] = a;
+        row2[p.Ncols + c] = b2;
+      }
     }
   }
 }
@@ -665,14 +704,23 @@
   const int grid = sk ? MAX_WG : (k.items < MAX_WG ? k.items : MAX_WG);
   size_t lds = (size_t)NSTG * (BM + BN) * BKB + BM * sizeof(int);
   const int chan = k.ntpg * BN;
-  const bool stats = a.stat_partial != nullptr && chan <= 512 && grid % ng == 0 &&
-                     lds + (size_t)WMW * chan * 2 * sizeof(float) <= 160 * 1024;
+  const size_t stat_lds = (size_t)WMW * chan * (a.bn2_y ? 3 : 2) * sizeof(float);
+  const bool stats = a.stat_partial != nullptr && chan <= 512 && grid % ng == 0 && lds + stat_lds <= 160 * 1024 &&
+                     (a.bn2_y == nullptr || a.stat_rows_cap == 0 || grid / ng <= a.stat_rows_cap);
   if (stat_rows) *stat_rows = stats ? grid / ng : 0;
   if (stats) {
-    lds += (size_t)WMW * chan * 2 * sizeof(float);
+    lds += stat_lds;
     lds_opt_in((const void*)igemm_kernel<T, BM, BN, WMW, NSTG, 1>, lds);
     lds_opt_in((const void*)igemm_kernel<T, BM, BN, WMW, NSTG, 2>, lds);
-    if (a.bn_y)
+    if (a.bn2_y) {
+      if constexpr (sizeof(T) == 2 && BM == 128) {
+        lds_opt_in((const void*)igemm_kernel<T, BM, BN, WMW, NSTG, 3>, lds);
+        hipLaunchKernelGGL((igemm_kernel<T, BM, BN, WMW, NSTG, 3>), dim3(grid), dim3(NT), lds, stream, k);
+      } else {
+        set_error("igemm: the sums of a second BatchNorm exist on the bf16 128-row tiles only");
+        return MI355_E_ARG;
+      }
+    } else if (a.bn_y)
       hipLaunchKernelGGL((igemm_kernel<T, BM, BN, WMW, NSTG, 2>), dim3(grid), dim3(NT), lds, stream, k);
     else
       hipLaunchKernelGGL((igemm_kernel<T, BM, BN, WMW, NSTG, 1>), dim3(grid), dim3(NT), lds, stream, k);
diff --git a/sota_imagenet_amd/csrc/conv_select.cpp b/sota_imagenet_amd/csrc/conv_select.cpp
--- a/sota_imagenet_amd/csrc/conv_select.cpp
+++ b/sota_imagenet_amd/csrc/conv_select.cpp
@@ -50,6 +50,7 @@
 }
 
 bool select_generated(const IgemmArgs& a, int nclass, ConvPick* p) {
+  if (a.bn2_y) return false;
   return dconv_pick(a, nclass, 0, p) || po_pick(a, nclass, p) || pw_pick(a, nclass, p) || pk_pick(a, nclass, p);
 }
 
@@ -60,7 +61,7 @@
     p.family = CONV_STEM;
     return p;
   }
-  if (choose_igemm8(a, nclass, &p)) {
+  if (!a.bn2_y && choose_igemm8(a, nclass, &p)) {
     p.family = CONV_IGEMM8;
     return p;
   }
@@ -74,6 +75,7 @@
                     (big_mode < 0 ? ((items3 <= cus && items3 * 2 >= cus && mt * a.Ck >= 512) || (items3 <= 2L * cus && mt == 1 && a.Ck >= 1024)) : big_mode == 3);
   p.bm = big || tall ? 256 : 128;
   p.bn = big ? 256 : (tall || wide ? 128 : 64);
+  if (a.bn2_y && p.bm == 256) p.bm = p.bn = 128;
   return p;
 }
 
@@ -116,6 +118,9 @@
   p.bn = wide ? 128 : 64;
   if (dtype == MI355_BF16) p = select_bf16(a, nclass, wide);
   MI355_ARG(a.bn_slope == 0.f || (leaky_sums_args(dtype, a) && takes_leaky_sums(p)), "igemm: BN-backward sums under a leaky mask need a generated kernel with that epilogue and slope 0.01 (igemm_leaky_sums_legal)");
+  MI355_ARG(a.bn2_y == nullptr || (a.bn_y && a.bn_bits && a.stat_partial && a.stat2_partial && a.bn2_mean && a.bn2_invstd && a.bn_slope == 0.f && p.family == CONV_TILE &&
+                                   dtype == MI355_BF16),
+            "igemm: the sums of a second BatchNorm ride with the first one's (bn_y, ReLU bit mask, both partial buffers) on the bf16 128-row implicit-GEMM tiles");
   MI355_ARG(a.bn_in == nullptr || takes_bn_in(p), "igemm: the input's BatchNorm in the operand path needs a generated kernel with that form (igemm_bn_in_legal)");
   if (dtype != MI355_F32 && dtype != MI355_BF16) {
     set_error("igemm: bad dtype %d", dtype);
diff --git a/sota_imagenet_amd/csrc/resnet_exec.cpp b/sota_imagenet_amd/csrc/resnet_exec.cpp
--- a/sota_imagenet_amd/csrc/resnet_exec.cpp
+++ b/sota_imagenet_amd/csrc/resnet_exec.cpp
@@ -47,6 +47,7 @@
   uint8_t *a1_q = nullptr, *a2_q = nullptr, *out_q = nullptr;
   int qid_a1 = -1, qid_a2 = -1, qid_out = -1;
   int Hin, Win, Hout, Wout, Cin, Cout;
+  int entry_form = 0;
 };
 
 }
@@ -96,6 +97,7 @@
   bool stem_fused_bwd = true;
   hipEvent_t w_done[MAX_GSETS] = {};
   hipEvent_t ds_done = nullptr;
+  int entry_joint = 1;
   bool w_pending[MAX_GSETS] = {};
   int bwd_parity = 0;
   bool fwd_training_done = false;
@@ -176,6 +178,10 @@
   return c->stream_k ? c->sk_ws[(c->wstream && s == c->wstream) ? 1 : 0] : nullptr;
 }
 inline float* bn_coef_of(mi355_ctx* c, hipStream_t s) { return (c->wstream && s == c->wstream) ? c->bn_coef2 : c->bn_coef; }
+inline size_t bn_partial_half(const mi355_ctx* c) { return (size_t)bn_max_blocks() * c->max_c; }
+inline float* ds_partial_of(mi355_ctx* c) { return c->bn_partial + bn_partial_half(c); }
+inline float* ds_coef_of(mi355_ctx* c) { return c->bn_partial + 2 * bn_partial_half(c) - 3 * c->max_c; }
+inline int ds_rows_cap(const mi355_ctx* c, int C) { return (int)((bn_partial_half(c) - 3 * c->max_c) / ((size_t)2 * C)); }
 double conv_flops(const mi355_ctx* c, const ConvBN& l) {
   return 2.0 * c->N * l.Hout * l.Wout * (double)l.Cout * l.Cin * l.K * l.K;
 }
@@ -288,6 +294,24 @@
   return launch_bn_bwd_apply(c->dtype, g2, nullptr, l.y, l.stat, l.stat + C, bn_coef_of(c, s), dx, M, C, s, bits2, 0.f, qo);
 }
 
+int bn_backward_entry(mi355_ctx* c, Block& b, const void* g, void* dx3, void* dxd, float beta_acc, hipStream_t s) {
+  ConvBN &l = b.c3, &d = b.ds;
+  const int M = c->N * l.Hout * l.Wout, C = l.Cout;
+  const double full = (double)M * C * c->es, mask_bytes = full / 16;
+  int nblk = l.bwd_rows, nblk_d = d.bwd_rows;
+  l.bwd_rows = d.bwd_rows = 0;
+  if (nblk == 0) {
+    Prof p(c, PC_BN_REDUCE, 0, 2 * full + mask_bytes, s);
+    MI355_TRY(launch_bn_bwd_reduce(c->dtype, g, nullptr, l.y, l.stat, l.stat + C, nullptr, c->bn_partial, &nblk, M, C, s, b.out_bits, 0.f));
+  }
+  MI355_TRY(launch_bn_bwd_finalize(c->bn_partial, nblk, M, C, c->params + l.gamma_off, l.stat + C, c->grads + l.gamma_off, c->grads + l.beta_off,
+                                   beta_acc, c->bn_coef, s));
+  MI355_TRY(launch_bn_bwd_finalize(ds_partial_of(c), nblk_d, M, C, c->params + d.gamma_off, d.stat + C, c->grads + d.gamma_off, c->grads + d.beta_off,
+                                   beta_acc, ds_coef_of(c), s));
+  Prof p(c, PC_BN_BWD_APPLY, 0, 5 * full + mask_bytes, s);
+  return launch_bn_bwd_apply2(c->dtype, g, b.out_bits, l.y, l.stat, l.stat + C, c->bn_coef, dx3, d.y, d.stat, d.stat + C, ds_coef_of(c), dxd, M, C, s);
+}
+
 int conv_wgrad(mi355_ctx* c, ConvBN& l, const void* dy, const void* x, float beta_acc, hipStream_t s) {
   WgradArgs a;
   build_wgrad_args(a, c->N, l.Hin, l.Win, l.Cin, l.Cout, l.K, l.K, l.stride, l.pad);
@@ -313,20 +337,25 @@
 }
 
 int conv_dgrad(mi355_ctx* c, ConvBN& l, const void* dy, void* dx, const void* addend, hipStream_t s,
-               const uint8_t* addend_bits = nullptr, ConvBN* bn = nullptr, const uint8_t* bn_bits = nullptr, float beta_acc = 0.f, bool sub2 = false) {
+               const uint8_t* addend_bits = nullptr, ConvBN* bn = nullptr, const uint8_t* bn_bits = nullptr, float beta_acc = 0.f, bool sub2 = false,
+               ConvBN* bn2 = nullptr) {
   IgemmArgs a;
   const int nclass = build_dgrad_args(a, c->N, l.Hin, l.Win, l.Cin, l.Cout, l.K, l.K, l.stride, l.pad);
   if (nclass < 0) return nclass;
   a.in = dy; a.wt = l.w_tr; a.out = dx; a.addend = addend; a.addend_bits = addend_bits; a.addend_sub2 = sub2 ? 1 : 0;
   a.sk_ws = sk_ws_of(c, s);
+  void* dyq = c->fp8_bwd_on && l.fp8_dgrad ? grad_twin(c, dy) : nullptr;
   if (bn && c->fuse_bn_bwd) {
     a.stat_partial = bn_partial_of(c, s);
     a.stat_rows_cap = (int)((size_t)bn_max_blocks() * c->max_c / bn->Cout);
     a.bn_y = bn->y; a.bn_bits = bn_bits; a.bn_mean = bn->stat; a.bn_invstd = bn->stat + bn->Cout;
+    if (bn2 && !dyq && a.stat_partial == c->bn_partial) {
+      a.bn2_y = bn2->y; a.bn2_mean = bn2->stat; a.bn2_invstd = bn2->stat + bn2->Cout; a.stat2_partial = ds_partial_of(c);
+      a.stat_rows_cap = ds_rows_cap(c, bn->Cout);
+    }
   }
   const double dx_elems = (double)c->N * l.Hin * l.Win * l.Cin;
-  void* dyq = c->fp8_bwd_on && l.fp8_dgrad ? grad_twin(c, dy) : nullptr;
-  const double by = dx_elems * (1 + (addend ? (sub2 ? 0.25 : 1) : 0) + (a.bn_y ? 1 : 0)) * c->es + (double)c->N * l.Hout * l.Wout * l.Cout * (dyq ? 1 : c->es) +
+  const double by = dx_elems * (1 + (addend ? (sub2 ? 0.25 : 1) : 0) + (a.bn_y ? 1 : 0) + (a.bn2_y ? 1 : 0)) * c->es + (double)c->N * l.Hout * l.Wout * l.Cout * (dyq ? 1 : c->es) +
                     dx_elems * c->es / 16 * ((addend_bits ? 1 : 0) + (a.bn_y ? 1 : 0));
   Prof p(c, igemm_class(l.Cin), conv_flops(c, l), by, s, (l.K == 3 ? 1 : 0) | (dyq ? 2 : 0));
   int* rows = bn && c->fuse_bn_bwd ? &bn->bwd_rows : nullptr;
@@ -337,6 +366,7 @@
   } else {
     MI355_TRY(launch_igemm(c->dtype, a, nclass, s, rows));
   }
+  if (a.bn2_y) bn2->bwd_rows = bn->bwd_rows;
   snprintf(l.k_dgrad, sizeof(l.k_dgrad), "%s", mi355_last_conv_kernel());
   return 0;
 }
@@ -570,11 +600,13 @@
   hipStream_t ws;
   const bool sub2 = sub2_ok(c, b, prev);
   MI355_TRY(acquire_set(c, par, s));
-  MI355_TRY(bn_backward(c, b.c3, G, b.out_bits, nullptr, B1, beta_acc, s));
+  const bool joint = b.has_ds && b.ds.bwd_rows > 0;
+  if (joint) MI355_TRY(bn_backward_entry(c, b, G, B1, B2, beta_acc, s));
+  else MI355_TRY(bn_backward(c, b.c3, G, b.out_bits, nullptr, B1, beta_acc, s));
   MI355_TRY(c->fork(s, &ws));
   MI355_TRY(conv_wgrad(c, b.c3, B1, b.a2, beta_acc, ws));
   if (b.has_ds) {
-    MI355_TRY(bn_backward(c, b.ds, G, b.out_bits, nullptr, B2, beta_acc, ws));
+    if (!joint) MI355_TRY(bn_backward(c, b.ds, G, b.out_bits, nullptr, B2, beta_acc, ws));
     if (sub2) MI355_TRY(conv_dgrad_compact(c, b.ds, B2, c->gsub, ws));
     else MI355_TRY(conv_dgrad(c, b.ds, B2, Gn, nullptr, ws));
     if (c->overlap) MI355_HIP(hipEventRecord(c->ds_done, ws));
@@ -593,7 +625,8 @@
     MI355_TRY(conv_dgrad(c, b.c1, B4, Gn, sub2 ? c->gsub : Gn, s, nullptr, prev ? &prev->c3 : nullptr, prev ? prev->out_bits : nullptr, beta_acc, sub2));
     c->cur_dout = Gn;
   } else {
-    MI355_TRY(conv_dgrad(c, b.c1, B4, G, G, s, b.out_bits, prev ? &prev->c3 : nullptr, prev ? prev->out_bits : nullptr, beta_acc));
+    MI355_TRY(conv_dgrad(c, b.c1, B4, G, G, s, b.out_bits, prev ? &prev->c3 : nullptr, prev ? prev->out_bits : nullptr, beta_acc, false,
+                         prev && prev->has_ds && prev->entry_form == 1 ? &prev->ds : nullptr));
     c->cur_dout = G;
   }
   return release_set(c, par);
@@ -726,6 +759,17 @@
   c->stem_fused_bwd = env_switch("MI355_STEM_FUSED", 1, 1, &bad) != 0;
   c->overlap = env_switch("MI355_WGRAD_STREAM", 1, 1, &bad) != 0;
   c->ds_compact = env_switch("MI355_DS_COMPACT", 1, 1, &bad) != 0;
+  c->entry_joint = env_switch("MI355_ENTRY_JOINT_BN", 1, 2, &bad);
+  if (dtype == MI355_BF16 && c->entry_joint != 0) {
+    static const int forms[3][4] = {{0, 0, 0, 0}, {1, 0, 0, 0}, {1, 1, 1, 1}};
+    int st = 0;
+    for (auto& b : c->blocks)
+      if (b.has_ds) {
+        b.entry_form = forms[c->entry_joint][st++];
+        if (!c->fuse_bn_bwd) b.entry_form = 0;
+        if (b.c3.qid_dy >= 0 || b.ds.qid_dy >= 0) b.entry_form = 0;
+      }
+  }
   if (bad) {
     set_error("create: %s=%s is outside the switch's domain", bad, getenv(bad));
     mi355_resnet50_destroy(c);
@@ -1058,6 +1102,7 @@
     Block& b = c->blocks[nb - c->next_seg];
     want = (size_t)c->N * b.Hout * b.Wout * b.Cout * c->es;
     b.c3.bwd_rows = 0;
+    b.ds.bwd_rows = 0;
   } else {
     want = (size_t)c->N * (c->stem.Hout / 2) * (c->stem.Wout / 2) * 64 * c->es;
   }
diff --git a/sota_imagenet_amd/ops.py b/sota_imagenet_amd/ops.py
--- a/sota_imagenet_amd/ops.py
+++ b/sota_imagenet_amd/ops.py
@@ -148,6 +148,45 @@
     if part is not None:
         part = part[:nblk.value] if nblk.value > 0 else None
     return dx, part
+
+
+def conv2d_dgrad_bn2(dy, w, x_shape, stride=1, pad=0, addend=None, addend_bits=None, bn_y=None, bn_bits=None, bn_mean=None, bn_invstd=None, bn2_y=None,
+                     bn2_mean=None, bn2_invstd=None):
+    _need_cuda(dy, w, addend, addend_bits, bn_y, bn_bits, bn_mean, bn_invstd, bn2_y, bn2_mean, bn2_invstd)
+    N, H, W, Cin = x_shape
+    Cout, KH, KW, _ = w.shape
+    dt = dtype_code(dy.dtype)
+    ws, n = _conv_ws(dt, N, H, W, Cin, Cout, KH, KW, stride, pad, dy.device)
+    dx = torch.empty((N, H, W, Cin), dtype=dy.dtype, device=dy.device)
+    part = torch.empty((768, 2, Cin), dtype=torch.float32, device=dy.device)
+    part2 = torch.empty((768, 2, Cin), dtype=torch.float32, device=dy.device)
+    nblk = ctypes.c_int(0)
+    check(_L().mi355_conv2d_dgrad_bn2(dt, ptr(dy), ptr(w), ptr(dx), ptr(addend), ptr(addend_bits), ptr(bn_y), ptr(bn_bits), ptr(bn_mean), ptr(bn_invstd),
+                                      ptr(part), ptr(bn2_y), ptr(bn2_mean), ptr(bn2_invstd), ptr(part2), part.numel() * 4, ctypes.byref(nblk), N, H, W,
+                                      Cin, Cout, KH, KW, stride, pad, ptr(ws), n, cur_stream()))
+    if nblk.value == 0:
+        return dx, None, None
+    return dx, part[:nblk.value], part2[:nblk.value]
+
+
+def bn_bwd_apply_bits(dout, bits, x, save_mean, save_invstd, coef):
+    _need_cuda(dout, bits, x, save_mean, save_invstd, coef)
+    C = x.shape[-1]
+    dx = torch.empty_like(x)
+    check(_L().mi355_bn_bwd_apply_bits(dtype_code(x.dtype), ptr(dout), ptr(bits), ptr(x), ptr(save_mean), ptr(save_invstd), ptr(coef), ptr(dx),
+                                       x.numel() // C, C, cur_stream()))
+    return dx
+
+
+def bn_bwd_apply2(dout, bits, xa, mean_a, invstd_a, coef_a, xb, mean_b, invstd_b, coef_b):
+    _need_cuda(dout, bits, xa, mean_a, invstd_a, coef_a, xb, mean_b, invstd_b, coef_b)
+    C = xa.shape[-1]
+    if xb.shape != xa.shape or xb.dtype != xa.dtype:
+        raise ValueError("bn_bwd_apply2: both BatchNorm inputs must have one shape and dtype")
+    dxa, dxb = torch.empty_like(xa), torch.empty_like(xb)
+    check(_L().mi355_bn_bwd_apply2(dtype_code(xa.dtype), ptr(dout), ptr(bits), ptr(xa), ptr(mean_a), ptr(invstd_a), ptr(coef_a), ptr(dxa), ptr(xb),
+                                   ptr(mean_b), ptr(invstd_b), ptr(coef_b), ptr(dxb), xa.numel() // C, C, cur_stream()))
+    return dxa, dxb
 
 
 def last_conv_kernel():
```

Result: no change. 14560 images/sec, median of 6 (+0.5%).
